# bluecube/minipath

Measured on AMD Instinct MI355X. Metric: Mrays/s, higher is better.
Workload: dtype f32

## Files before the change

minipath_amd/csrc/group_walk.h:

```cpp
#pragma once

#include "wave_common.h"

namespace mp {
namespace {

constexpr int kFcmpOGT = 2, kFcmpOGE = 3, kFcmpOLT = 4, kFcmpOLE = 5;
__device__ __forceinline__ uint64_t mask_gt(float a, float b) { return __builtin_amdgcn_fcmpf(a, b, kFcmpOGT); }
__device__ __forceinline__ uint64_t mask_lt(float a, float b) { return __builtin_amdgcn_fcmpf(a, b, kFcmpOLT); }
__device__ __forceinline__ uint64_t mask_le(float a, float b) { return __builtin_amdgcn_fcmpf(a, b, kFcmpOLE); }
__device__ __forceinline__ uint64_t mask_ge(float a, float b) { return __builtin_amdgcn_fcmpf(a, b, kFcmpOGE); }

enum { kClosest = 0, kBounded = 1, kAnyHit = 2 };
template <bool PATCH_NAN, bool BFE, int QS = 64, int MODE = kClosest>
__device__ __forceinline__ void trace_wave_impl(const DevScene& sc, float* __restrict__ q, uint2* __restrict__ stack_base,
                                                int nrays, float pb = FLT_MAX) {
    static_assert(MODE == kClosest || QS == 64, "ray queries run on the wave's LDS queue");
    constexpr int HB = QS == 64 ? 0 : 9;
    const int lane = static_cast<int>(threadIdx.x) & 63;
    const int g = lane >> 3, li = lane & 7;
    uint2* stack = stack_base + g * sc.stack_cap;
    const uint32_t lanes_below = (1u << li) - 1u;

    int slot = -1, sp = 0, head = 0;
    uint32_t pk = 0, pk_end = 0, seq = 0;
    float ox = 0, oy = 0, oz = 0, dx = 0, dy = 0, dz = 0, ix = 0, iy = 0, iz = 0;
    const float4* __restrict__ nodes4 = reinterpret_cast<const float4*>(PATCH_NAN ? sc.nodes_lit : sc.nodes_aos);
    const uint32_t root = PATCH_NAN ? sc.root_lit : sc.root;
    const float* __restrict__ tris = sc.tris_aos;
    float best_t = FLT_MAX;
    float tl = FLT_MAX, ul = 0, vl = 0;
    uint32_t pkl = kNoPrim, seql = 0;
    float pix = 0.0f, piy = 0.0f, piz = 0.0f;
    if (QS == 64) {
        const float qx = q[3 * 64 + lane], qy = q[4 * 64 + lane], qz = q[5 * 64 + lane];
        pix = (qx == 0.0f) ? INFINITY : 1.0f / qx; piy = (qy == 0.0f) ? INFINITY : 1.0f / qy; piz = (qz == 0.0f) ? INFINITY : 1.0f / qz;
    }

    for (;;) {
        if (MODE == kAnyHit && slot >= 0 && sp == 0 && pk == pk_end) {
            if (li == 0) q[1 * 64 + slot] = as_f(pkl);
            slot = -1;
        }
        if (MODE != kAnyHit && slot >= 0 && sp == 0 && pk == pk_end) {
            float tmin = group_min_t(tl);
            uint32_t key = (pkl != kNoPrim && tl == tmin) ? ((seql << 3) | static_cast<uint32_t>(li)) : 0xFFFFFFFFu;
            uint32_t kmin = group_min_u(key);
            const int wl4 = (((static_cast<int>(threadIdx.x) & 56) | static_cast<int>(kmin & 7u))) << 2;
            const float wu = __int_as_float(__builtin_amdgcn_ds_bpermute(wl4, __float_as_int(ul)));
            const float wv = __int_as_float(__builtin_amdgcn_ds_bpermute(wl4, __float_as_int(vl)));
            const uint32_t wp = static_cast<uint32_t>(__builtin_amdgcn_ds_bpermute(wl4, static_cast<int>(pkl)));
            if (li == 0) {
                bool hit = kmin != 0xFFFFFFFFu;
                q[(HB + 0) * QS + slot] = hit ? tmin : FLT_MAX;
                q[(HB + 1) * QS + slot] = as_f(hit ? (wp * 8u + (kmin & 7u)) : kNoPrim);
                q[(HB + 2) * QS + slot] = wu;
                q[(HB + 3) * QS + slot] = wv;
            }
            slot = -1;
        }
        uint64_t idle = __ballot(slot < 0);
        if (idle != 0) {
            int g_ = g;
            asm volatile("" : "+v"(g_));
            const uint64_t groups_below = (1ull << (g_ * 8)) - 1ull;
            uint64_t gm = idle & 0x0101010101010101ull;
            int mine = head + __popcll(gm & groups_below);
            head += __popcll(gm);
            float fix = 0.0f, fiy = 0.0f, fiz = 0.0f, fb = FLT_MAX;
            if (QS == 64) { fix = __shfl(pix, mine & 63); fiy = __shfl(piy, mine & 63); fiz = __shfl(piz, mine & 63); }
            if (MODE != kClosest) fb = __shfl(pb, mine & 63);
            if (slot < 0 && mine < nrays) {
                slot = mine;
                ox = q[0 * QS + mine]; oy = q[1 * QS + mine]; oz = q[2 * QS + mine];
                dx = q[3 * QS + mine]; dy = q[4 * QS + mine]; dz = q[5 * QS + mine];
                if (QS != 64) { fix = q[6 * QS + mine]; fiy = q[7 * QS + mine]; fiz = q[8 * QS + mine]; }
                ix = fix; iy = fiy; iz = fiz;
                best_t = fb; tl = fb; ul = 0; vl = 0; pkl = kNoPrim; seql = 0; seq = 0;
                pk = pk_end = 0;
                sp = 1;
                if (li == 0) stack[0] = make_uint2(root, as_u(-INFINITY));
            }
            if (__ballot(slot >= 0) == 0) break;
        }
        wave_lds_sync();
        if (slot >= 0 && pk == pk_end) {
            sp--;
            uint2 e = stack[sp];
            float node_t1 = as_f(e.y);
            if (!(node_t1 > best_t)) {
                uint32_t link = e.x;
                if ((link & 63u) == 0u) {
                    const float4* cp = reinterpret_cast<const float4*>(reinterpret_cast<const char*>(nodes4) + ((link << 2) | (static_cast<uint32_t>(li) << 5)));
                    const float4 c0 = cp[0], c1 = cp[1];
                    const uint32_t child = as_u(c1.z);
                    float ax = (c0.x - ox) * ix, ay = (c0.y - oy) * iy, az = (c0.z - oz) * iz;
                    float cx = (c0.w - ox) * ix, cy = (c1.x - oy) * iy, cz = (c1.y - oz) * iz;
                    if (PATCH_NAN) {
                        ax = fmaxf(ax, -INFINITY); ay = fmaxf(ay, -INFINITY); az = fmaxf(az, -INFINITY);
                        cx = fminf(cx, INFINITY); cy = fminf(cy, INFINITY); cz = fminf(cz, INFINITY);
                    }
                    const float t1 = fmaxf(fmaxf(fminf(ax, cx), 0.0f), fmaxf(fminf(ay, cy), fminf(az, cz)));
                    const float t2 = fminf(fminf(fmaxf(ax, cx), best_t), fminf(fmaxf(ay, cy), fmaxf(az, cz)));
                    const uint64_t okm = mask_le(t1, t2) & __builtin_amdgcn_uicmp(child, MP_LINK_NULL, 33);
                    const bool ok = __builtin_amdgcn_inverse_ballot_w64(okm);
                    uint32_t m = static_cast<uint32_t>(okm >> (g * 8)) & 0xFFu;
                    const uint32_t below = BFE ? __builtin_amdgcn_ubfe(m, 0u, static_cast<uint32_t>(li)) : (m & lanes_below);
                    if (ok) stack[sp + __popc(below)] = make_uint2(child, as_u(t1));
                    sp += __popc(m);
                } else {
                    pk = link >> 6;
                    pk_end = pk + (((link & 63u) + 7u) >> 3);
                }
            }
        }
        if (slot >= 0 && pk < pk_end) {
            const uint32_t toff = ((pk * 9u) << 5) + static_cast<uint32_t>(li) * 36u;
            const float* tp = reinterpret_cast<const float*>(reinterpret_cast<const char*>(tris) + toff);
            const float v0x = tp[0], v0y = tp[1], v0z = tp[2], e1x = tp[3], e1y = tp[4], e1z = tp[5], e2x = tp[6], e2y = tp[7], e2z = tp[8];
            float hx = fms(dy, e2z, dz * e2y), hy = fms(dz, e2x, dx * e2z), hz = fms(dx, e2y, dy * e2x);
            float det = fma_dot(e1x, e1y, e1z, hx, hy, hz);
            float inv_det = 1.0f / det;
            float sx = ox - v0x, sy = oy - v0y, sz = oz - v0z;
            float u = inv_det * fma_dot(sx, sy, sz, hx, hy, hz);
            float qx = fms(sy, e1z, sz * e1y), qy = fms(sz, e1x, sx * e1z), qz = fms(sx, e1y, sy * e1x);
            float v = inv_det * fma_dot(dx, dy, dz, qx, qy, qz);
            float t = inv_det * fma_dot(e2x, e2y, e2z, qx, qy, qz);
            bool valid = (u >= 0.0f) & (v >= 0.0f) & ((u + v) <= 1.0f) & (t >= 0.0f) & (t <= best_t);
            if (MODE == kAnyHit) {
                if ((__ballot(valid && t < tl) >> (g * 8)) & 0xFFull) { sp = 0; pk = pk_end; pkl = 0u; }
                else pk++;
                continue;
            }
            if (valid && t < tl) { tl = t; ul = u; vl = v; pkl = pk; seql = seq; }
            seq++;
            pk++;
            if (pk == pk_end) best_t = group_min_t(tl);
        }
    }
    wave_lds_sync();
}

template <bool BFE = false, int MODE = kClosest>
__device__ __forceinline__ void trace_wave(const DevScene& sc, float* __restrict__ q, uint2* __restrict__ stack_base, int nrays,
                                           float pb = FLT_MAX) {
    const int lane = static_cast<int>(threadIdx.x) & 63;
    const float qx = q[3 * 64 + lane], qy = q[4 * 64 + lane], qz = q[5 * 64 + lane];
    const float ix = (qx == 0.0f) ? INFINITY : 1.0f / qx, iy = (qy == 0.0f) ? INFINITY : 1.0f / qy, iz = (qz == 0.0f) ? INFINITY : 1.0f / qz;
    const bool inf = lane < nrays && (fabsf(ix) == INFINITY || fabsf(iy) == INFINITY || fabsf(iz) == INFINITY);
    if (__ballot(inf) != 0) trace_wave_impl<true, BFE, 64, MODE>(sc, q, stack_base, nrays, pb);
    else trace_wave_impl<false, BFE, 64, MODE>(sc, q, stack_base, nrays, pb);
}

template <int QS>
__device__ __forceinline__ void trace_wave_pool(const DevScene& sc, float* __restrict__ q, uint2* __restrict__ stack_base, int nrays) {
    int lane = static_cast<int>(threadIdx.x) & 63;
    asm volatile("" : "+v"(lane));
    bool inf = false;
#pragma unroll
    for (int k = 0; k < QS / 64; k++) {
        const int slot = lane + 64 * k;
        if (slot < nrays)
            inf = inf || fabsf(q[6 * QS + slot]) == INFINITY || fabsf(q[7 * QS + slot]) == INFINITY || fabsf(q[8 * QS + slot]) == INFINITY;
    }
    if (__ballot(inf) != 0) trace_wave_impl<true, true, QS>(sc, q, stack_base, nrays);
    else trace_wave_impl<false, true, QS>(sc, q, stack_base, nrays);
}

__device__ __forceinline__ bool may_hit_scene(const DevScene& sc, const Ray& r) {
    if (!sc.has_pre) return true;
    float ax = (sc.pre_min[0] - r.ox) * r.ix, ay = (sc.pre_min[1] - r.oy) * r.iy, az = (sc.pre_min[2] - r.oz) * r.iz;
    float cx = (sc.pre_max[0] - r.ox) * r.ix, cy = (sc.pre_max[1] - r.oy) * r.iy, cz = (sc.pre_max[2] - r.oz) * r.iz;
    ax = (ax != ax) ? -INFINITY : ax; ay = (ay != ay) ? -INFINITY : ay; az = (az != az) ? -INFINITY : az;
    cx = (cx != cx) ? INFINITY : cx; cy = (cy != cy) ? INFINITY : cy; cz = (cz != cz) ? INFINITY : cz;
    float lox = fminf(ax, cx), loy = fminf(ay, cy), loz = fminf(az, cz);
    float hix = fmaxf(ax, cx), hiy = fmaxf(ay, cy), hiz = fmaxf(az, cz);
    float t1 = fmaxf(fmaxf(lox, 0.0f), fmaxf(loy, loz));
    float t2 = fminf(fminf(hix, FLT_MAX), fminf(hiy, hiz));
    return t1 <= t2;
}

__device__ __forceinline__ uint32_t resolve_normal(const DevScene& sc, uint32_t prim, float u, float v, float n[3]) {
    const float4* sh = reinterpret_cast<const float4*>(sc.shade) + static_cast<size_t>(prim) * 3;
    float4 a = sh[0], b = sh[1], c = sh[2];
    float nx, ny, nz;
    if (as_u(c.y) != 0u) {
        const float* tp = sc.tris_aos + static_cast<size_t>(prim) * kTriDwords;
        float e1x = tp[3], e1y = tp[4], e1z = tp[5], e2x = tp[6], e2y = tp[7], e2z = tp[8];
        nx = e1y * e2z - e1z * e2y;
        ny = e1z * e2x - e1x * e2z;
        nz = e1x * e2y - e1y * e2x;
    } else {
        float w = 1.0f - u - v;
        nx = a.x * w + a.w * u + b.z * v;
        ny = a.y * w + b.x * u + b.w * v;
        nz = a.z * w + b.y * u + c.x * v;
    }
    float len = sqrtf(nx * nx + ny * ny + nz * nz);
    n[0] = nx / len; n[1] = ny / len; n[2] = nz / len;
    return as_u(c.z);
}

__device__ __forceinline__ bool sphere_intersect(const DevScene& sc, const Ray& r, float& t, float n[3]) {
    const float ocx = r.ox - sc.sphere_center[0], ocy = r.oy - sc.sphere_center[1], ocz = r.oz - sc.sphere_center[2];
    const float b = ocx * r.dx + ocy * r.dy + ocz * r.dz;
    const float c = (ocx * ocx + ocy * ocy + ocz * ocz) - sc.sphere_radius * sc.sphere_radius;
    const float disc = b * b - c;
    if (disc < 0.0f) return false;
    const float sq = sqrtf(disc);
    const float t1 = -b - sq, t2 = -b + sq;
    if (t1 > 0.0f) t = t1;
    else if (t2 > 0.0f) t = t2;
    else return false;
    const float px = r.ox + r.dx * t, py = r.oy + r.dy * t, pz = r.oz + r.dz * t;
    const float nx = px - sc.sphere_center[0], ny = py - sc.sphere_center[1], nz = pz - sc.sphere_center[2];
    const float len = sqrtf(nx * nx + ny * ny + nz * nz);
    n[0] = nx / len; n[1] = ny / len; n[2] = nz / len;
    return true;
}

__device__ __forceinline__ void object_scene(const DevScene& sc, uint32_t k, DevScene& sk) {
    sk = sc;
    const DevObject& o = sc.objects[k];
    sk.shade = o.shade; sk.nodes_aos = o.nodes_aos; sk.nodes_lit = o.nodes_lit; sk.tris_aos = o.tris_aos; sk.vidx = o.vidx; sk.vtex = o.vtex;
    sk.root = o.root; sk.root_lit = o.root_lit; sk.has_pre = o.has_pre;
    sk.kind = o.kind; sk.sphere_radius = o.sphere_radius;
    for (int i = 0; i < 3; i++) { sk.pre_min[i] = o.pre_min[i]; sk.pre_max[i] = o.pre_max[i]; sk.sphere_center[i] = o.sphere_center[i]; }
}
__device__ __forceinline__ void quat_rotate(float qi, float qj, float qk, float qw, float vx, float vy, float vz, float& ox,
                                            float& oy, float& oz) {
    const float tx = (qj * vz - qk * vy) * 2.0f, ty = (qk * vx - qi * vz) * 2.0f, tz = (qi * vy - qj * vx) * 2.0f;
    const float cx = qj * tz - qk * ty, cy = qk * tx - qi * tz, cz = qi * ty - qj * tx;
    ox = tx * qw + cx + vx; oy = ty * qw + cy + vy; oz = tz * qw + cz + vz;
}
__device__ __forceinline__ void object_ray(const DevScene& sc, uint32_t k, const Ray& r, Ray& rk) {
    const DevObject& o = sc.objects[k];
    rk = r;
    rk.ox = r.ox - o.t[0]; rk.oy = r.oy - o.t[1]; rk.oz = r.oz - o.t[2];
    if (o.rotated) {
        const float qi = -o.q[0], qj = -o.q[1], qk = -o.q[2], qw = o.q[3];
        const float vx = rk.ox, vy = rk.oy, vz = rk.oz;
        quat_rotate(qi, qj, qk, qw, vx, vy, vz, rk.ox, rk.oy, rk.oz);
        quat_rotate(qi, qj, qk, qw, r.dx, r.dy, r.dz, rk.dx, rk.dy, rk.dz);
        rk.ix = (rk.dx == 0.0f) ? INFINITY : 1.0f / rk.dx;
        rk.iy = (rk.dy == 0.0f) ? INFINITY : 1.0f / rk.dy;
        rk.iz = (rk.dz == 0.0f) ? INFINITY : 1.0f / rk.dz;
    }
}

struct GroupHit {
    float t, u, v;
    uint32_t prim, inst;
};

template <bool OBJ, bool BFE = false, int MODE = kClosest>
__device__ __forceinline__ void trace_objects(const DevScene& sc, const Ray& r, bool act, float* __restrict__ q,
                                              uint2* __restrict__ stack, GroupHit& h, float b = FLT_MAX) {
    h.t = MODE == kClosest ? FLT_MAX : b; h.u = h.v = 0.0f; h.prim = kNoPrim; h.inst = 0u;
    auto pass = [&](const DevScene& sk, const Ray& rk, uint32_t k) {
        const bool open = act && (MODE != kAnyHit || h.prim == kNoPrim);
        if (OBJ && sk.kind == 1u) {
            float ts, nn[3];
            if (open && sphere_intersect(sk, rk, ts, nn) && ts < h.t) { h.t = ts; h.prim = 0u; h.u = h.v = 0.0f; h.inst = k; }
            return;
        }
        const bool queued = open && may_hit_scene(sk, rk);
        const uint64_t am = __ballot(queued);
        const int n = __popcll(am), rank = rank_below(am);
        if (queued) {
            q[0 * 64 + rank] = rk.ox; q[1 * 64 + rank] = rk.oy; q[2 * 64 + rank] = rk.oz;
            q[3 * 64 + rank] = rk.dx; q[4 * 64 + rank] = rk.dy; q[5 * 64 + rank] = rk.dz;
        }
        float pb = FLT_MAX;
        if (MODE != kClosest) {
            const int dst = queued ? rank : n + (static_cast<int>(threadIdx.x & 63) - rank);
            pb = __int_as_float(__builtin_amdgcn_ds_permute(dst << 2, __float_as_int(b)));
        }
        wave_lds_sync();
        trace_wave<BFE, MODE>(sk, q, stack, n, pb);
        if (queued) {
            const uint32_t prim = as_u(q[1 * 64 + rank]);
            if (MODE == kAnyHit) {
                if (prim != kNoPrim) { h.prim = 0u; h.inst = k; }
            } else {
                const float t = q[0 * 64 + rank];
                if (prim != kNoPrim && t < h.t) { h.t = t; h.prim = prim; h.u = q[2 * 64 + rank]; h.v = q[3 * 64 + rank]; h.inst = k; }
            }
        }
        wave_lds_sync();
    };
    if (!OBJ) {
        pass(sc, r, 0u);
    } else {
        for (uint32_t k = 0; k < sc.inst_count; k++) {
            DevScene sk;
            Ray rk;
            object_scene(sc, k, sk);
            object_ray(sc, k, r, rk);
            pass(sk, rk, k);
        }
    }
    if (MODE != kClosest && h.prim == kNoPrim) h.t = FLT_MAX;
}

__device__ __forceinline__ uint32_t object_normal(const DevScene& sc, uint32_t inst, const Ray& r, uint32_t prim, float u, float v,
                                                  float n[3]) {
    DevScene so;
    object_scene(sc, inst, so);
    uint32_t mat = 0u;
    if (so.kind == 1u) {
        Ray rk;
        object_ray(sc, inst, r, rk);
        float t;
        sphere_intersect(so, rk, t, n);
    } else {
        mat = resolve_normal(so, prim, u, v, n);
    }
    const DevObject& o = sc.objects[inst];
    if (o.rotated) quat_rotate(o.q[0], o.q[1], o.q[2], o.q[3], n[0], n[1], n[2], n[0], n[1], n[2]);
    return mat;
}

}
}
```

minipath_amd/csrc/kernels.hip:

```cpp
#include <hip/hip_runtime.h>

#include <algorithm>
#include <cfloat>
#include <cmath>
#include <cstdlib>
#include <type_traits>

#include "launch_plan.h"
#include "mp_internal.h"
#include "family_launch.h"
#include "ray_math.h"

#ifdef MP_PROF_MISSES
namespace mp {
namespace {
__device__ unsigned long long g_prof[8];
}
}
#define MP_PROF_COUNT(i) do { if ((threadIdx.x & 63u) == 0u) atomicAdd(&g_prof[i], 1ull); } while (0)
#endif
#include "mask_cache.h"
#include "group_walk.h"

namespace mp {
namespace {

struct RenderParams {
    DevScene scene;
    RayGen gen;
    const mp_block* tiles;
    uint32_t n_tiles, tile_size;
    float* out;
    uint32_t* counter;
    float inv_spp;
    uint32_t s_begin, s_end;
    uint32_t carry_in;
    uint32_t finalize;
    uint32_t chunked;
    const uint32_t* tile_order;
    unsigned long long* tile_cost;
    uint32_t lds_per_wave;
    uint32_t max_depth;
    unsigned long long* segments;
    float* pool;
    uint32_t pool_stride;
};

constexpr uint32_t kSumChunk = 256;
__device__ __forceinline__ void pixel_state_load(const RenderParams& P, size_t off, bool inpix, bool writer, float& acc, float& cnt) {
    acc = 0.0f;
    cnt = 0.0f;
    if (P.carry_in && inpix) {
        const float4 prev = *reinterpret_cast<const float4*>(P.out + off);
        acc = prev.x;
        cnt = P.chunked ? prev.y : prev.w;
    } else if (P.chunked && inpix && writer) {
        *reinterpret_cast<double*>(P.out + off + 2) = 0.0;
    }
}
__device__ __forceinline__ void chunk_flush(const RenderParams& P, size_t off, bool writer, float& acc) {
    if (writer) {
        double* t = reinterpret_cast<double*>(P.out + off + 2);
        *t = *t + static_cast<double>(acc);
    }
    acc = 0.0f;
}
__device__ __forceinline__ void pixel_state_store(const RenderParams& P, size_t off, float acc, float cnt) {
    if (P.chunked) {
        if (!P.finalize) {
            *reinterpret_cast<float2*>(P.out + off) = make_float2(acc, cnt);
            return;
        }
        double t = *reinterpret_cast<const double*>(P.out + off + 2);
        if ((P.s_end & (kSumChunk - 1u)) != 0u) t = t + static_cast<double>(acc);
        const double inv = 1.0 / static_cast<double>(P.gen.spp);
        const float m = static_cast<float>(t * inv), a = static_cast<float>(static_cast<double>(cnt) * inv);
        *reinterpret_cast<float4*>(P.out + off) = make_float4(m, m, m, a);
        return;
    }
    const float m = P.finalize ? acc * P.inv_spp : acc;
    const float a = P.finalize ? cnt * P.inv_spp : cnt;
    *reinterpret_cast<float4*>(P.out + off) = make_float4(m, m, m, a);
}

typedef const __attribute__((address_space(4))) RenderParams* kparams_t;
__device__ __forceinline__ const RenderParams& params_view(kparams_t kp) { return kernarg_view<RenderParams>(kp); }
#define MP_KERNEL_PARAMS kparams_t KP = (kparams_t)__builtin_amdgcn_kernarg_segment_ptr()

#define MP_NEXT_UNIT(unit)                                                                              \
    uint32_t unit;                                                                                      \
    {                                                                                                   \
        const uint32_t q_ = qstate & 0xFFu;                                                             \
        uint32_t idx_ = 0;                                                                              \
        if (lane == 0) idx_ = atomicAdd(P.counter + q_ * kWorkQueueStride, 1u);                         \
        idx_ = __builtin_amdgcn_readfirstlane(idx_);                                                    \
        unit = idx_ * kWorkQueues + q_;                                                                 \
        if (unit >= total || idx_ >= 0x10000000u) {                                                     \
            if ((qstate >> 8) + 1u == kWorkQueues) break;                                               \
            qstate = ((q_ + 1u) % kWorkQueues) | (((qstate >> 8) + 1u) << 8);                           \
            continue;                                                                                   \
        }                                                                                               \
        qstate = q_;                                                                                    \
    }

template <int S, bool OBJ>
__global__ __launch_bounds__(256) void render_tiles_kernel(RenderParams) {
    extern __shared__ __align__(16) unsigned char smem[];
    MP_KERNEL_PARAMS;
    const RenderParams& P0 = params_view(KP);
    constexpr int BW = (S == 1) ? 8 : (S == 2) ? 8 : (S == 4) ? 4 : 4;
    constexpr int BH = 64 / S / BW;
    const int lane = static_cast<int>(threadIdx.x) & 63, wave = static_cast<int>(threadIdx.x) >> 6;
    float* q = reinterpret_cast<float*>(smem + static_cast<size_t>(wave) * P0.lds_per_wave);
    uint2* stack = reinterpret_cast<uint2*>(q + kQueueFloats);
    const uint32_t ts = P0.tile_size;
    const uint32_t bx = (ts + BW - 1) / BW, by = (ts + BH - 1) / BH, upt = bx * by;
    const uint32_t total = P0.n_tiles * upt;
    const int pix = lane / S, sub = lane % S;

    uint32_t qstate = blockIdx.x % kWorkQueues;
    for (;;) {
        const RenderParams& P = params_view(KP);
        MP_NEXT_UNIT(unit)
        const uint32_t b = unit % upt;
        const uint32_t tile_i = P.tile_order ? P.tile_order[unit / upt] : unit / upt;
        const uint64_t t_unit = P.tile_cost ? __builtin_readcyclecounter() : 0;
        const mp_block T = P.tiles[tile_i];
        const uint32_t px = T.min_x + (b % bx) * BW + static_cast<uint32_t>(pix % BW);
        const uint32_t py = T.min_y + (b / bx) * BH + static_cast<uint32_t>(pix / BW);
        const bool inpix = px < T.max_x && py < T.max_y;
        if (__ballot(inpix) == 0) continue;
        const size_t off = (static_cast<size_t>(tile_i) * ts * ts + static_cast<size_t>(py - T.min_y) * ts + (px - T.min_x)) * 4;
        float acc, cnt;
        pixel_state_load(P, off, inpix, sub == 0, acc, cnt);
        for (uint32_t s0 = P.s_begin & ~static_cast<uint32_t>(S - 1); s0 < P.s_end; s0 += S) {
            const uint32_t s = s0 + static_cast<uint32_t>(sub);
            const bool act = inpix && s >= P.s_begin && s < P.s_end;
            Ray r;
            r.dx = r.dy = r.dz = 0.0f;
            if (act) sample_ray(P.gen, px, py, s, r);
            if (P.scene.kind == 1u) {
                float c = 0.0f, h = 0.0f, ts_, nn[3];
                if (act && sphere_intersect(P.scene, r, ts_, nn)) { c = fabsf(r.dx * nn[0] + r.dy * nn[1] + r.dz * nn[2]); h = 1.0f; }
#pragma unroll
                for (int j = 0; j < S; j++) {
                    acc += __shfl(c, (lane & ~(S - 1)) + j);
                    cnt += __shfl(h, (lane & ~(S - 1)) + j);
                }
                if (P.chunked && ((s0 + S) & (kSumChunk - 1u)) == 0u && s0 + S <= P.s_end) chunk_flush(P, off, inpix && sub == 0, acc);
                continue;
            }
            GroupHit gh;
            trace_objects<OBJ>(P.scene, r, act, q, stack, gh);
            float c = 0.0f, h = 0.0f;
            if (gh.prim != kNoPrim) {
                float nn[3];
                if (OBJ) object_normal(P.scene, gh.inst, r, gh.prim, gh.u, gh.v, nn);
                else resolve_normal(P.scene, gh.prim, gh.u, gh.v, nn);
                c = fabsf(r.dx * nn[0] + r.dy * nn[1] + r.dz * nn[2]);
                h = 1.0f;
            }
#pragma unroll
            for (int j = 0; j < S; j++) {
                acc += __shfl(c, (lane & ~(S - 1)) + j);
                cnt += __shfl(h, (lane & ~(S - 1)) + j);
            }
            if (P.chunked && ((s0 + S) & (kSumChunk - 1u)) == 0u && s0 + S <= P.s_end) chunk_flush(P, off, inpix && sub == 0, acc);
        }
        if (inpix && sub == 0) pixel_state_store(P, off, acc, cnt);
// ... 222 lines not shown
struct RegStack3 {
    int ent, mlo, mhi;
    __device__ __forceinline__ RegStack3() : ent(0), mlo(0), mhi(0) {}
    __device__ __forceinline__ void push(int sp, uint32_t e, uint64_t m) {
        asm volatile("s_mov_b32 m0, %3\n\ts_nop 0\n\t"
                     "v_writelane_b32 %0, %4, m0\n\tv_writelane_b32 %1, %5, m0\n\tv_writelane_b32 %2, %6, m0"
                     : "+v"(ent), "+v"(mlo), "+v"(mhi)
                     : "s"(sp), "s"(e), "s"(static_cast<uint32_t>(m)), "s"(static_cast<uint32_t>(m >> 32))
                     : "m0");
    }
    __device__ __forceinline__ void pop(int sp, uint32_t& e, uint64_t& m) const {
        e = static_cast<uint32_t>(__builtin_amdgcn_readlane(ent, sp));
        m = static_cast<uint32_t>(__builtin_amdgcn_readlane(mlo, sp)) |
            (static_cast<uint64_t>(static_cast<uint32_t>(__builtin_amdgcn_readlane(mhi, sp))) << 32);
    }
};

template <int OCT>
__device__ __noinline__ uint32_t unit_list_slow(const float* __restrict__ nodes_pk, uint32_t* mcache, uint32_t node, uint32_t slots) {
    return unit_list_build(reinterpret_cast<const float4*>(nodes_pk), mcache, node, slots,
                           [](const float* b, const float bmn[3], const float bmx[3]) { return bounds_may_hit<OCT>(b, bmn, bmx); });
}
template <int OCT>
__device__ __forceinline__ bool trace_packet_cached(const DevScene& sc, const Ray& r, bool active, PacketHit& hit, uint32_t* mcache) {
    static_assert(kNullLink == MP_LINK_NULL, "mask_cache.h's copy of the null link");
    kfp nodes = (kfp)(uintptr_t)sc.nodes_pk;
    kfp tris = (kfp)(uintptr_t)sc.tris_aos;
    float best_t = FLT_MAX, bu = 0.0f, bv = 0.0f;
    uint32_t bprim = kNoPrim;
    RegStack3 st;
    int sp = 0;
    mcache[kRootListSlot] = sc.pk_count * sc.pk_mask_bits;
    wave_lds_sync();
    uint32_t cur = (static_cast<uint32_t>(kRootListSlot) << 16) | 1u;
    uint64_t pm = __ballot(active);
    for (;;) {
        if ((cur & 0xFFFFu) == 0u) {
            if (sp == 0) break;
            sp--;
            st.pop(sp, cur, pm);
        }
        cur -= 1u;
        const uint32_t src = __builtin_amdgcn_readfirstlane(mcache[(cur >> 16) + (cur & 0xFFFFu)]);
#ifndef MP_NO_EMPTY_SKIP
        if (static_cast<int32_t>(src) < 0) {
            MP_PROF_COUNT(7);
            continue;
        }
#endif
        const bool pon = __builtin_amdgcn_inverse_ballot_w64(pm);
        const krec8 rec = *reinterpret_cast<const __attribute__((address_space(4))) krec8*>(reinterpret_cast<const __attribute__((address_space(4))) char*>(nodes) + scalar_u(src * 32u));
        float t1, t2;
        slab<false, OCT>(rec[0], rec[1], rec[2], rec[3], rec[4], rec[5], r, pon ? best_t : -1.0f, t1, t2);
        const bool ok = t1 <= t2;
        if (__ballot(ok) == 0) continue;
        const uint32_t link = uniform_u(rec[6]);
        float lim = ok ? best_t : -1.0f;
        if ((link & 63u) == 0u) {
            MP_PROF_COUNT(2);
            const uint32_t node = link >> 6;
            const uint32_t slot = node_slot(node);
            const uint32_t tag = __builtin_amdgcn_readfirstlane(mcache[static_cast<uint32_t>(kMaskCacheHeader) + slot]);
            uint32_t list = __builtin_amdgcn_readfirstlane(mcache[static_cast<uint32_t>(kNodeListBase) + slot]);
            if (__builtin_expect(tag != node, 0)) {
                MP_PROF_COUNT(0);
                if (tag != 0xFFFFFFFFu) MP_PROF_COUNT(4);
                list = __builtin_amdgcn_readfirstlane(unit_list_slow<OCT>(sc.nodes_pk, mcache, node, sc.pk_mask_bits));
                if (list == kListOverflow) {
                    if (sp != 0 || (cur & 0xFFFFu) != 0u) {
                        MP_PROF_COUNT(6);
                        return false;
                    }
                    list = __builtin_amdgcn_readfirstlane(unit_list_slow<OCT>(sc.nodes_pk, mcache, node, sc.pk_mask_bits));
                }
            }
            if ((list & 0xFFFFu) != 0u) {
                if ((cur & 0xFFFFu) != 0u) {
                    st.push(sp, cur, pm);
                    sp++;
                }
                cur = list;
                pm = __ballot(lim >= 0.0f);
            }
        } else {
            const uint32_t first = link >> 6, n_real = link & 63u;
            kfp tp = tris + static_cast<size_t>(first) * (8 * kTriDwords);
            static_assert(kExitTiny == kTiny && kExitHuge == kHuge, "mask_cache.h's copies of the early-out constants");
            const float thr = lim >= 0.0f ? -kTiny : INFINITY;
            auto test = [&](const float v0x, const float v0y, const float v0z, const float e1x, const float e1y, const float e1z,
                            const float e2x, const float e2y, const float e2z, const uint32_t tri) {
                const float hx = fms(r.dy, e2z, r.dz * e2y), hy = fms(r.dz, e2x, r.dx * e2z), hz = fms(r.dx, e2y, r.dy * e2x);
                const float det = fma_dot(e1x, e1y, e1z, hx, hy, hz);
                const float sx = r.ox - v0x, sy = r.oy - v0y, sz = r.oz - v0z;
                const float un = fma_dot(sx, sy, sz, hx, hy, hz);
                const float xu = tri_flipped(det, un);
                if (__ballot(!(tri_exit1_key(det, xu) <= thr)) == 0) return;
                const float qx = fms(sy, e1z, sz * e1y), qy = fms(sz, e1x, sx * e1z), qz = fms(sx, e1y, sy * e1x);
                const float vn = fma_dot(r.dx, r.dy, r.dz, qx, qy, qz);
                const float tn = fma_dot(e2x, e2y, e2z, qx, qy, qz);
                const float xv = tri_flipped(det, vn), xt = tri_flipped(det, tn);
                if (__ballot(!(tri_exit2_key(det, xu, xv, xt) <= thr)) == 0) return;
                constexpr uint32_t kRcpLo = 0x10800000u , kRcpHi = 0x7E000000u ;
                const uint32_t wkey = (as_u(det) << 1) - (kRcpLo << 1);
                const float inv_det = __ballot(wkey > ((kRcpHi - kRcpLo) << 1)) == 0 ? rm::rcp_short(det) : 1.0f / det;
                const float u = inv_det * un, v = inv_det * vn, t = inv_det * tn;
                const bool acc = !(fminf(fminf(u, v), t) < 0.0f) & ((u + v) <= 1.0f) & (t < lim);
                best_t = acc ? t : best_t;
                lim = acc ? t : lim;
                bu = acc ? u : bu;
                bv = acc ? v : bv;
                bprim = acc ? tri : bprim;
            };
            const uint32_t ls = first & static_cast<uint32_t>(kLeafCacheEntries - 1);
            const uint32_t tag = mcache[kLeafTagBase + ls];
            const uint2 tm = reinterpret_cast<const uint2*>(mcache + kLeafMaskBase)[ls];
            uint64_t todo;
            if (__builtin_expect(__builtin_amdgcn_readfirstlane(tag) == first, 1)) {
                todo = __builtin_amdgcn_readfirstlane(tm.x) | (static_cast<uint64_t>(__builtin_amdgcn_readfirstlane(tm.y)) << 32);
            } else {
                MP_PROF_COUNT(1);
                const uint64_t m = leaf_mask_slow(sc.tris_aos, mcache, first, n_real);
                todo = __builtin_amdgcn_readfirstlane(static_cast<uint32_t>(m)) | (static_cast<uint64_t>(__builtin_amdgcn_readfirstlane(static_cast<uint32_t>(m >> 32))) << 32);
            }
#ifndef MP_NO_EMPTY_SKIP
            if (todo == 0 && (cur >> 16) != static_cast<uint32_t>(kRootListSlot)) {
                if ((threadIdx.x & 63u) == 0u) mcache[(cur >> 16) + (cur & 0xFFFFu)] = src | kEmptyLeafBit;
                wave_lds_sync();
            }
#endif
            if (todo != 0) {
                uint32_t c = static_cast<uint32_t>(__builtin_ctzll(todo));
                todo &= ~(1ull << c);
                kfp ta = tri_record(tp, c);
                krec8 ra = *reinterpret_cast<const __attribute__((address_space(4))) krec8*>(ta);
                float a8 = ta[8];
                while (todo != 0) {
                    const uint32_t cn = static_cast<uint32_t>(__builtin_ctzll(todo));
                    todo &= ~(1ull << cn);
                    kfp tb = tri_record(tp, cn);
                    const krec8 rb = *reinterpret_cast<const __attribute__((address_space(4))) krec8*>(tb);
                    const float b8 = tb[8];
                    test(ra[0], ra[1], ra[2], ra[3], ra[4], ra[5], ra[6], ra[7], a8, first * 8u + c);
                    ra = rb; a8 = b8;
                    c = cn;
                }
                test(ra[0], ra[1], ra[2], ra[3], ra[4], ra[5], ra[6], ra[7], a8, first * 8u + c);
            }
        }
    }
    hit.t = best_t; hit.u = bu; hit.v = bv; hit.prim = bprim;
    return true;
}

template <bool OCTANTS, class Stack, bool MC = false>
__device__ __forceinline__ void trace_packet(const DevScene& sc, const Ray& r, bool active, Stack& st, PacketHit& hit,
                                             const MaskCache& mc = MaskCache{nullptr}) {
    if (OCTANTS && MC) {
        if (__ballot(active & !mask_cache_ray_ok(r)) != 0) {
            const bool slow = active && (fabsf(r.ix) == INFINITY || fabsf(r.iy) == INFINITY || fabsf(r.iz) == INFINITY);
            if (__ballot(slow) != 0) trace_packet_impl<2, -1>(sc, r, active, st, hit);
            else trace_packet_impl<1, -1>(sc, r, active, st, hit);
            return;
        }
    } else {
        const bool slow = active && (fabsf(r.ix) == INFINITY || fabsf(r.iy) == INFINITY || fabsf(r.iz) == INFINITY);
        if (__ballot(slow) != 0) {
            trace_packet_impl<2, -1>(sc, r, active, st, hit);
            return;
        }
    }
    if (OCTANTS && sc.boxes_ordered) {
        const uint64_t am = __ballot(active);
        const uint64_t nx = __ballot(active && r.ix < 0.0f), ny = __ballot(active && r.iy < 0.0f), nz = __ballot(active && r.iz < 0.0f);
        if ((nx == 0 || nx == am) && (ny == 0 || ny == am) && (nz == 0 || nz == am)) {
            const uint32_t oct = (nx ? 1u : 0u) | (ny ? 2u : 0u) | (nz ? 4u : 0u);
            if (MC) {
                mask_cache_begin_pass(mc, r, active, oct);
                bool done;
                switch (oct) {
                    case 0: done = trace_packet_cached<0>(sc, r, active, hit, mc.lds); break;
                    case 1: done = trace_packet_cached<1>(sc, r, active, hit, mc.lds); break;
                    case 2: done = trace_packet_cached<2>(sc, r, active, hit, mc.lds); break;
                    case 3: done = trace_packet_cached<3>(sc, r, active, hit, mc.lds); break;
                    case 4: done = trace_packet_cached<4>(sc, r, active, hit, mc.lds); break;
                    case 5: done = trace_packet_cached<5>(sc, r, active, hit, mc.lds); break;
                    case 6: done = trace_packet_cached<6>(sc, r, active, hit, mc.lds); break;
                    default: done = trace_packet_cached<7>(sc, r, active, hit, mc.lds); break;
                }
                if (done) return;
            } else {
                switch (oct) {
                    case 0: trace_packet_impl<1, 0>(sc, r, active, st, hit); return;
                    case 1: trace_packet_impl<1, 1>(sc, r, active, st, hit); return;
                    case 2: trace_packet_impl<1, 2>(sc, r, active, st, hit); return;
                    case 3: trace_packet_impl<1, 3>(sc, r, active, st, hit); return;
                    case 4: trace_packet_impl<1, 4>(sc, r, active, st, hit); return;
                    case 5: trace_packet_impl<1, 5>(sc, r, active, st, hit); return;
                    case 6: trace_packet_impl<1, 6>(sc, r, active, st, hit); return;
                    default: trace_packet_impl<1, 7>(sc, r, active, st, hit); return;
                }
            }
        }
    }
    trace_packet_impl<1, -1>(sc, r, active, st, hit);
}

template <class T>
__device__ __forceinline__ const T* uniform_ptr(const T* p) {
    const uint64_t v = reinterpret_cast<uint64_t>(p);
    const uint32_t lo = __builtin_amdgcn_readfirstlane(static_cast<uint32_t>(v)), hi = __builtin_amdgcn_readfirstlane(static_cast<uint32_t>(v >> 32));
    return reinterpret_cast<const T*>((static_cast<uint64_t>(hi) << 32) | lo);
}

template <bool OCTANTS, class Stack>
__device__ __forceinline__ void trace_packet_objects(const DevScene& sc, const Ray& r, bool act, Stack& st, PacketHit& h, uint32_t& inst) {
    h.t = FLT_MAX; h.u = h.v = 0.0f; h.prim = kNoPrim;
    inst = 0u;
    for (uint32_t k = 0; k < sc.inst_count; k++) {
        DevScene sk;
        Ray rk;
        object_scene(sc, k, sk);
        object_ray(sc, k, r, rk);
        sk.kind = __builtin_amdgcn_readfirstlane(sk.kind);
        sk.root = __builtin_amdgcn_readfirstlane(sk.root);
        sk.root_lit = __builtin_amdgcn_readfirstlane(sk.root_lit);
        sk.nodes_aos = uniform_ptr(sk.nodes_aos);
        sk.nodes_lit = uniform_ptr(sk.nodes_lit);
        sk.tris_aos = uniform_ptr(sk.tris_aos);
        if (sk.kind == 1u) {
            float ts, nn[3];
            if (act && sphere_intersect(sk, rk, ts, nn) && ts < h.t) { h.t = ts; h.prim = 0u; h.u = h.v = 0.0f; inst = k; }
            continue;
        }
        const bool go = act && may_hit_scene(sk, rk);
        if (__ballot(go) == 0) continue;
        PacketHit hk;
        trace_packet<OCTANTS>(sk, rk, go, st, hk);
        if (hk.prim != kNoPrim && hk.t < h.t) { h = hk; inst = k; }
    }
}

struct RegStack2 {
    int link, src, alo, ahi, blo, bhi;
    __device__ __forceinline__ RegStack2() : link(0), src(0), alo(0), ahi(0), blo(0), bhi(0) {}
    __device__ __forceinline__ void push(int sp, uint32_t l, uint32_t s, uint64_t ma, uint64_t mb) {
        asm volatile(
            "s_mov_b32 m0, %6\n\ts_nop 0\n\t"
            "v_writelane_b32 %0, %7, m0\n\tv_writelane_b32 %1, %8, m0\n\tv_writelane_b32 %2, %9, m0\n\tv_writelane_b32 %3, %10, m0\n\t"
            "v_writelane_b32 %4, %11, m0\n\tv_writelane_b32 %5, %12, m0"
            : "+v"(link), "+v"(src), "+v"(alo), "+v"(ahi), "+v"(blo), "+v"(bhi)
            : "s"(sp), "s"(l), "s"(s), "s"(static_cast<uint32_t>(ma)), "s"(static_cast<uint32_t>(ma >> 32)),
              "s"(static_cast<uint32_t>(mb)), "s"(static_cast<uint32_t>(mb >> 32))
            : "m0");
    }
    __device__ __forceinline__ void pop(int sp, uint32_t& l, uint32_t& s, uint64_t& ma, uint64_t& mb) const {
        l = static_cast<uint32_t>(__builtin_amdgcn_readlane(link, sp));
        s = static_cast<uint32_t>(__builtin_amdgcn_readlane(src, sp));
        ma = static_cast<uint32_t>(__builtin_amdgcn_readlane(alo, sp)) |
             (static_cast<uint64_t>(static_cast<uint32_t>(__builtin_amdgcn_readlane(ahi, sp))) << 32);
        mb = static_cast<uint32_t>(__builtin_amdgcn_readlane(blo, sp)) |
             (static_cast<uint64_t>(static_cast<uint32_t>(__builtin_amdgcn_readlane(bhi, sp))) << 32);
    }
};

template <int MODE, int OCT>
__device__ __forceinline__ void trace_packet2_impl(const DevScene& sc, const Ray& ra, const Ray& rb, bool active_a, bool active_b,
                                                   PacketHit& hit_a, PacketHit& hit_b) {
    constexpr bool PATCH_NAN = MODE == 2;
    kfp nodes = (kfp)(uintptr_t)(PATCH_NAN ? sc.nodes_lit : sc.nodes_aos);
    kfp tris = (kfp)(uintptr_t)sc.tris_aos;
    RegStack2 st;
    float best_a = FLT_MAX, ua = 0.0f, va = 0.0f, best_b = FLT_MAX, ub = 0.0f, vb = 0.0f;
    uint32_t prim_a = kNoPrim, prim_b = kNoPrim;
    st.push(0, PATCH_NAN ? sc.root_lit : sc.root, kSrcRoot, __ballot(active_a), __ballot(active_b));
    int sp = 1;
    int stale_top = 0;
    while (sp > 0) {
        sp--;
        uint32_t link, src;
        uint64_t onm_a, onm_b;
        st.pop(sp, link, src, onm_a, onm_b);
        if (sp < stale_top) {
            stale_top = sp;
            kfp bx = nodes + static_cast<size_t>(src) * 8;
            const float b0 = bx[0], b1 = bx[1], b2 = bx[2], b3 = bx[3], b4 = bx[4], b5 = bx[5];
            onm_a &= ~mask_gt(slab_entry<PATCH_NAN, OCT>(b0, b1, b2, b3, b4, b5, ra), best_a);
            onm_b &= ~mask_gt(slab_entry<PATCH_NAN, OCT>(b0, b1, b2, b3, b4, b5, rb), best_b);
        }
        if ((onm_a | onm_b) == 0) continue;
        const bool on_a = __builtin_amdgcn_inverse_ballot_w64(onm_a), on_b = __builtin_amdgcn_inverse_ballot_w64(onm_b);
        float lim_a = on_a ? best_a : -1.0f, lim_b = on_b ? best_b : -1.0f;
        if ((link & 63u) == 0u) {
            const uint32_t node = link >> 6;
            kfp nd = nodes + static_cast<size_t>(node) * 64;
            float a0 = nd[0], a1 = nd[1], a2 = nd[2], a3 = nd[3], a4 = nd[4], a5 = nd[5], a6 = nd[6];
            const uint32_t nchild = uniform_u(nd[7]);
            uint32_t slot = node * 8u;
            auto child = [&](const float b0, const float b1, const float b2, const float b3, const float b4, const float b5,
                             const float blink, const uint32_t cslot) {
                const uint32_t cl = uniform_u(blink);
                if (cl == MP_LINK_NULL) return;
                float t1a, t2a, t1b, t2b;
                slab<PATCH_NAN, OCT>(b0, b1, b2, b3, b4, b5, ra, lim_a, t1a, t2a);
                slab<PATCH_NAN, OCT>(b0, b1, b2, b3, b4, b5, rb, lim_b, t1b, t2b);
                const uint64_t ok_a = __ballot(t1a <= t2a), ok_b = __ballot(t1b <= t2b);
                if ((ok_a | ok_b) != 0) {
                    st.push(sp, cl, cslot, ok_a, ok_b);
                    sp++;
                }
            };
            for (uint32_t p = nchild >> 1; p > 0; p--) {
                const float b0 = nd[8], b1 = nd[9], b2 = nd[10], b3 = nd[11], b4 = nd[12], b5 = nd[13], b6 = nd[14];
                child(a0, a1, a2, a3, a4, a5, a6, slot);
                a0 = nd[16]; a1 = nd[17]; a2 = nd[18]; a3 = nd[19]; a4 = nd[20]; a5 = nd[21]; a6 = nd[22];
                child(b0, b1, b2, b3, b4, b5, b6, slot + 1u);
                slot += 2u;
                nd += 16;
            }
            if (nchild & 1u) child(a0, a1, a2, a3, a4, a5, a6, slot);
        } else {
            const uint32_t first = link >> 6, n_real = link & 63u;
            kfp tp = tris + static_cast<size_t>(first) * (8 * kTriDwords);
            const float thr_a = on_a ? -kTiny : INFINITY, thr_b = on_b ? -kTiny : INFINITY;
            uint64_t changed = 0;
            auto test = [&](const float v0x, const float v0y, const float v0z, const float e1x, const float e1y, const float e1z,
                            const float e2x, const float e2y, const float e2z, const uint32_t tri) {
                const float hxa = fms(ra.dy, e2z, ra.dz * e2y), hya = fms(ra.dz, e2x, ra.dx * e2z), hza = fms(ra.dx, e2y, ra.dy * e2x);
                const float hxb = fms(rb.dy, e2z, rb.dz * e2y), hyb = fms(rb.dz, e2x, rb.dx * e2z), hzb = fms(rb.dx, e2y, rb.dy * e2x);
                const float det_a = fma_dot(e1x, e1y, e1z, hxa, hya, hza), det_b = fma_dot(e1x, e1y, e1z, hxb, hyb, hzb);
                const float sxa = ra.ox - v0x, sya = ra.oy - v0y, sza = ra.oz - v0z;
                const float sxb = rb.ox - v0x, syb = rb.oy - v0y, szb = rb.oz - v0z;
                const float un_a = fma_dot(sxa, sya, sza, hxa, hya, hza), un_b = fma_dot(sxb, syb, szb, hxb, hyb, hzb);
                const uint32_t sg_a = as_u(det_a) & 0x80000000u, sg_b = as_u(det_b) & 0x80000000u;
                const bool ok_a = fabsf(det_a) <= kHuge, ok_b = fabsf(det_b) <= kHuge;
                const float xua = ok_a ? as_f(as_u(un_a) ^ sg_a) : 1.0f, xub = ok_b ? as_f(as_u(un_b) ^ sg_b) : 1.0f;
                if ((__ballot(!(xua <= thr_a)) | __ballot(!(xub <= thr_b))) == 0) return;
                const float qxa = fms(sya, e1z, sza * e1y), qya = fms(sza, e1x, sxa * e1z), qza = fms(sxa, e1y, sya * e1x);
                const float qxb = fms(syb, e1z, szb * e1y), qyb = fms(szb, e1x, sxb * e1z), qzb = fms(sxb, e1y, syb * e1x);
                const float vn_a = fma_dot(ra.dx, ra.dy, ra.dz, qxa, qya, qza), vn_b = fma_dot(rb.dx, rb.dy, rb.dz, qxb, qyb, qzb);
                const float tn_a = fma_dot(e2x, e2y, e2z, qxa, qya, qza), tn_b = fma_dot(e2x, e2y, e2z, qxb, qyb, qzb);
                const float xva = ok_a ? as_f(as_u(vn_a) ^ sg_a) : 1.0f, xta = ok_a ? as_f(as_u(tn_a) ^ sg_a) : 1.0f;
                const float xvb = ok_b ? as_f(as_u(vn_b) ^ sg_b) : 1.0f, xtb = ok_b ? as_f(as_u(tn_b) ^ sg_b) : 1.0f;
                if ((__ballot(!(fminf(fminf(xua, xva), xta) <= thr_a)) | __ballot(!(fminf(fminf(xub, xvb), xtb) <= thr_b))) == 0) return;
                const float inv_a = 1.0f / det_a, inv_b = 1.0f / det_b;
                const float u_a = inv_a * un_a, v_a = inv_a * vn_a, t_a = inv_a * tn_a;
                const float u_b = inv_b * un_b, v_b = inv_b * vn_b, t_b = inv_b * tn_b;
                const bool acc_a = (u_a >= 0.0f) & (v_a >= 0.0f) & ((u_a + v_a) <= 1.0f) & (t_a >= 0.0f) & (t_a < lim_a);
                const bool acc_b = (u_b >= 0.0f) & (v_b >= 0.0f) & ((u_b + v_b) <= 1.0f) & (t_b >= 0.0f) & (t_b < lim_b);
                best_a = acc_a ? t_a : best_a; lim_a = acc_a ? t_a : lim_a; ua = acc_a ? u_a : ua; va = acc_a ? v_a : va; prim_a = acc_a ? tri : prim_a;
                best_b = acc_b ? t_b : best_b; lim_b = acc_b ? t_b : lim_b; ub = acc_b ? u_b : ub; vb = acc_b ? v_b : vb; prim_b = acc_b ? tri : prim_b;
                changed |= __ballot(acc_a) | __ballot(acc_b);
            };
            float a0 = tp[0], a1 = tp[1], a2 = tp[2], a3 = tp[3], a4 = tp[4], a5 = tp[5], a6 = tp[6], a7 = tp[7], a8 = tp[8];
            uint32_t tri = first * 8u;
            for (uint32_t p = n_real >> 1; p > 0; p--) {
                const float b0 = tp[9], b1 = tp[10], b2 = tp[11], b3 = tp[12], b4 = tp[13], b5 = tp[14], b6 = tp[15], b7 = tp[16], b8 = tp[17];
                test(a0, a1, a2, a3, a4, a5, a6, a7, a8, tri);
                a0 = tp[18]; a1 = tp[19]; a2 = tp[20]; a3 = tp[21]; a4 = tp[22]; a5 = tp[23]; a6 = tp[24]; a7 = tp[25]; a8 = tp[26];
                test(b0, b1, b2, b3, b4, b5, b6, b7, b8, tri + 1u);
                tri += 2u;
                tp += 2 * kTriDwords;
            }
            if (n_real & 1u) test(a0, a1, a2, a3, a4, a5, a6, a7, a8, tri);
            if (changed != 0) stale_top = sp;
        }
    }
    hit_a.t = best_a; hit_a.u = ua; hit_a.v = va; hit_a.prim = prim_a;
    hit_b.t = best_b; hit_b.u = ub; hit_b.v = vb; hit_b.prim = prim_b;
}

__device__ __forceinline__ void trace_packet2(const DevScene& sc, const Ray& ra, const Ray& rb, bool act_a, bool act_b, PacketHit& ha,
                                              PacketHit& hb) {
    const bool slow = (act_a && (fabsf(ra.ix) == INFINITY || fabsf(ra.iy) == INFINITY || fabsf(ra.iz) == INFINITY)) ||
                      (act_b && (fabsf(rb.ix) == INFINITY || fabsf(rb.iy) == INFINITY || fabsf(rb.iz) == INFINITY));
    if (__ballot(slow) != 0) {
        trace_packet2_impl<2, -1>(sc, ra, rb, act_a, act_b, ha, hb);
        return;
    }
    if (sc.boxes_ordered) {
        const uint64_t am = __ballot(act_a), bm = __ballot(act_b);
        const uint64_t nxa = __ballot(act_a && ra.ix < 0.0f), nya = __ballot(act_a && ra.iy < 0.0f), nza = __ballot(act_a && ra.iz < 0.0f);
        const uint64_t nxb = __ballot(act_b && rb.ix < 0.0f), nyb = __ballot(act_b && rb.iy < 0.0f), nzb = __ballot(act_b && rb.iz < 0.0f);
        const bool xn = (nxa | nxb) != 0, yn = (nya | nyb) != 0, zn = (nza | nzb) != 0;
        const bool xu = !xn || (nxa == am && nxb == bm), yu = !yn || (nya == am && nyb == bm), zu = !zn || (nza == am && nzb == bm);
        if (xu && yu && zu) {
            switch ((xn ? 1 : 0) | (yn ? 2 : 0) | (zn ? 4 : 0)) {
                case 0: trace_packet2_impl<1, 0>(sc, ra, rb, act_a, act_b, ha, hb); return;
                case 1: trace_packet2_impl<1, 1>(sc, ra, rb, act_a, act_b, ha, hb); return;
                case 2: trace_packet2_impl<1, 2>(sc, ra, rb, act_a, act_b, ha, hb); return;
                case 3: trace_packet2_impl<1, 3>(sc, ra, rb, act_a, act_b, ha, hb); return;
                case 4: trace_packet2_impl<1, 4>(sc, ra, rb, act_a, act_b, ha, hb); return;
                case 5: trace_packet2_impl<1, 5>(sc, ra, rb, act_a, act_b, ha, hb); return;
                case 6: trace_packet2_impl<1, 6>(sc, ra, rb, act_a, act_b, ha, hb); return;
                default: trace_packet2_impl<1, 7>(sc, ra, rb, act_a, act_b, ha, hb); return;
            }
        }
    }
    trace_packet2_impl<1, -1>(sc, ra, rb, act_a, act_b, ha, hb);
}

template <int J, int N>
struct RowSum {
    static __device__ __forceinline__ void run(float& acc, float c) {
        acc += __int_as_float(__builtin_amdgcn_update_dpp(0, __float_as_int(c), 0x150 + J, 0xF, 0xF, false));
        RowSum<J + 1, N>::run(acc, c);
    }
};
template <int N>
struct RowSum<N, N> {
    static __device__ __forceinline__ void run(float&, float) {}
};
template <int S>
__device__ __forceinline__ void add_samples_in_order(float& acc, float c, int lane) {
    if (S == 1) {
        acc += c;
    } else if (S == 16) {
        RowSum<0, 16>::run(acc, c);
    } else if (S == 32) {
        RowSum<0, 16>::run(acc, c);
        acc = __int_as_float(__builtin_amdgcn_update_dpp(__float_as_int(acc), __float_as_int(acc), 0x142, 0xA, 0xF, false));
        RowSum<0, 16>::run(acc, c);
        const float lo = __int_as_float(__builtin_amdgcn_readlane(__float_as_int(acc), 31));
        const float hi = __int_as_float(__builtin_amdgcn_readlane(__float_as_int(acc), 63));
        acc = lane < 32 ? lo : hi;
    } else {
#pragma unroll
        for (int j = 0; j < S; j++) acc += __shfl(c, (lane & ~(S - 1)) + j);
    }
}

template <int S, bool LDS_STACK, int WPE, bool OBJ = false, bool MCACHE = false>
__global__ __launch_bounds__(256) __attribute__((amdgpu_waves_per_eu(WPE, 8))) void render_tiles_packet_kernel(RenderParams) {
    extern __shared__ __align__(16) unsigned char smem[];
    MP_KERNEL_PARAMS;
    constexpr int BW = (S <= 2) ? 8 : (S <= 8) ? 4 : (S <= 32) ? 2 : 1;
    constexpr int BH = 64 / S / BW;
    const int lane = static_cast<int>(threadIdx.x) & 63;
    const int pix = lane / S, sub = lane % S;
    uint32_t qstate = blockIdx.x % kWorkQueues;
    MaskCache mc{nullptr};
    if (MCACHE) mc.lds = reinterpret_cast<uint32_t*>(smem) + static_cast<size_t>(__builtin_amdgcn_readfirstlane(static_cast<int>(threadIdx.x) >> 6)) * kMaskCacheDwords;
    for (;;) {
        const RenderParams& P = params_view(KP);
        const uint32_t ts = P.tile_size;
        const uint32_t bx = (ts + BW - 1) / BW, by = (ts + BH - 1) / BH, upt = bx * by, total = P.n_tiles * upt;
        MP_NEXT_UNIT(unit)
        const uint32_t b = unit % upt;
        const uint32_t tile_i = P.tile_order ? P.tile_order[unit / upt] : unit / upt;
        const uint64_t t_unit = P.tile_cost ? __builtin_readcyclecounter() : 0;
        const mp_block T = P.tiles[tile_i];
        const uint32_t px = T.min_x + (b % bx) * BW + static_cast<uint32_t>(pix % BW);
        const uint32_t py = T.min_y + (b / bx) * BH + static_cast<uint32_t>(pix / BW);
        const bool inpix = px < T.max_x && py < T.max_y;
        if (__ballot(inpix) == 0) continue;
        const size_t off = (static_cast<size_t>(tile_i) * ts * ts + static_cast<size_t>(py - T.min_y) * ts + (px - T.min_x)) * 4;
        float acc, cnt;
        pixel_state_load(P, off, inpix, sub == 0, acc, cnt);
        if (MCACHE) {
            const RenderParams& C = params_view(KP);
            const uint32_t ux = T.min_x + (b % bx) * BW, uy = T.min_y + (b / bx) * BH;
            mask_cache_begin_unit(mc, C.gen.s, C.gen.jitter_scale, ux, min(ux + BW, T.max_x) - 1u, uy, min(uy + BH, T.max_y) - 1u);
        }
        const uint32_t s_begin = P.s_begin, s_end = P.s_end;
        for (uint32_t s0 = s_begin & ~static_cast<uint32_t>(S - 1); s0 < s_end; s0 += S) {
            const uint32_t s = s0 + static_cast<uint32_t>(sub);
            const bool act = inpix && s >= s_begin && s < s_end;
            Ray r;
            r.ox = r.oy = r.oz = r.dx = r.dy = r.dz = r.ix = r.iy = r.iz = 0.0f;
            {
                const RenderParams& G = params_view(KP);
                if (act) sample_ray(G.gen, px, py, s, r);
            }
            PacketHit h;
            h.t = FLT_MAX; h.u = h.v = 0.0f; h.prim = kNoPrim;
            uint32_t hinst = 0u;
            {
                const RenderParams& W = params_view(KP);
                float* lds = reinterpret_cast<float*>(smem + static_cast<size_t>(static_cast<int>(threadIdx.x) >> 6) * W.lds_per_wave);
                if (OBJ) {
                    if (LDS_STACK) {
                        HybridStack st(lds, lane, W.scene.stack_cap, W.scene.packet_stack_regs);
                        trace_packet_objects<false>(W.scene, r, act, st, h, hinst);
                    } else {
                        RegStack st(lds, lane);
                        trace_packet_objects<(S >= 8 && S <= 32)>(W.scene, r, act, st, h, hinst);
                    }
                } else {
#ifdef MP_PROF_NOWALK
                    const bool go = false;
#else
                    const bool go = act && W.scene.kind == 0u && may_hit_scene(W.scene, r);
#endif
                    if (__ballot(go) != 0) {
                        if (LDS_STACK) {
                            HybridStack st(lds, lane, W.scene.stack_cap, W.scene.packet_stack_regs);
                            trace_packet<false>(W.scene, r, go, st, h);
                        } else {
                            RegStack st(lds, lane);
                            trace_packet<((S >= 8 && S <= 32) || MCACHE), RegStack, MCACHE>(W.scene, r, go, st, h, mc);
                        }
                    }
                }
            }
            float c = 0.0f;
            bool hit = h.prim != kNoPrim;
            const RenderParams& H = params_view(KP);
            if (hit) {
#ifdef MP_PROF_NOSHADE
                c = h.u;
#else
                float nn[3];
                if (OBJ) object_normal(H.scene, hinst, r, h.prim, h.u, h.v, nn);
                else resolve_normal(H.scene, h.prim, h.u, h.v, nn);
                c = fabsf(r.dx * nn[0] + r.dy * nn[1] + r.dz * nn[2]);
#endif
            } else if (H.scene.kind == 1u) {
                float ts_, nn[3];
                hit = act && sphere_intersect(H.scene, r, ts_, nn);
                if (hit) c = fabsf(r.dx * nn[0] + r.dy * nn[1] + r.dz * nn[2]);
            }
            {
                int l_ = lane;
                asm volatile("" : "+v"(l_));
                const uint64_t pixel_lanes = (S == 64 ? ~0ull : ((1ull << (S & 63)) - 1ull)) << (l_ & ~(S - 1));
                cnt += static_cast<float>(__popcll(__ballot(hit) & pixel_lanes));
            }
            add_samples_in_order<S>(acc, c, lane);
            if (H.chunked && ((s0 + S) & (kSumChunk - 1u)) == 0u && s0 + S <= s_end) chunk_flush(H, off, inpix && sub == 0, acc);
        }
        const RenderParams& E = params_view(KP);
        if (inpix && sub == 0) pixel_state_store(E, off, acc, cnt);
        if (E.tile_cost && lane == 0) atomicAdd(E.tile_cost + tile_i, static_cast<unsigned long long>(__builtin_readcyclecounter() - t_unit));
    }
}

template <int WPE>
__global__ __launch_bounds__(256) __attribute__((amdgpu_waves_per_eu(WPE, 8))) void render_tiles_packet2_kernel(RenderParams P) {
    constexpr int S = 16;
    const int lane = static_cast<int>(threadIdx.x) & 63;
    const int pix = lane / S, sub = lane % S;
    const uint64_t pixel_lanes = ((1ull << S) - 1ull) << (lane & ~(S - 1));
    const uint32_t ts = P.tile_size;
    const uint32_t bx = (ts + 3) / 4, by = (ts + 1) / 2, upt = bx * by, total = P.n_tiles * upt;
    uint32_t qstate = blockIdx.x % kWorkQueues;
    for (;;) {
        MP_NEXT_UNIT(unit)
        const uint32_t b = unit % upt;
        const uint32_t tile_i = P.tile_order ? P.tile_order[unit / upt] : unit / upt;
        const uint64_t t_unit = P.tile_cost ? __builtin_readcyclecounter() : 0;
        const mp_block T = P.tiles[tile_i];
        const uint32_t px_a = T.min_x + (b % bx) * 4 + static_cast<uint32_t>(pix % 2), px_b = px_a + 2u;
        const uint32_t py = T.min_y + (b / bx) * 2 + static_cast<uint32_t>(pix / 2);
        const bool in_a = px_a < T.max_x && py < T.max_y, in_b = px_b < T.max_x && py < T.max_y;
        if (__ballot(in_a) == 0) continue;
        const size_t off_a = (static_cast<size_t>(tile_i) * ts * ts + static_cast<size_t>(py - T.min_y) * ts + (px_a - T.min_x)) * 4;
        const size_t off_b = off_a + 8;
        float acc_a, cnt_a, acc_b, cnt_b;
        pixel_state_load(P, off_a, in_a, sub == 0, acc_a, cnt_a);
        pixel_state_load(P, off_b, in_b, sub == 0, acc_b, cnt_b);
        for (uint32_t s0 = P.s_begin & ~static_cast<uint32_t>(S - 1); s0 < P.s_end; s0 += S) {
            const uint32_t s = s0 + static_cast<uint32_t>(sub);
            const bool in_pass = s >= P.s_begin && s < P.s_end;
            const bool act_a = in_a && in_pass, act_b = in_b && in_pass;
            Ray ra, rb;
            ra.ox = ra.oy = ra.oz = ra.dx = ra.dy = ra.dz = ra.ix = ra.iy = ra.iz = 0.0f;
            rb = ra;
            if (act_a) sample_ray(P.gen, px_a, py, s, ra);
            if (act_b) sample_ray(P.gen, px_b, py, s, rb);
            const bool go_a = act_a && may_hit_scene(P.scene, ra), go_b = act_b && may_hit_scene(P.scene, rb);
            PacketHit ha, hb;
            ha.t = FLT_MAX; ha.u = ha.v = 0.0f; ha.prim = kNoPrim;
            hb = ha;
            if ((__ballot(go_a) | __ballot(go_b)) != 0) trace_packet2(P.scene, ra, rb, go_a, go_b, ha, hb);
            float c_a = 0.0f, c_b = 0.0f;
            const bool hit_a = ha.prim != kNoPrim, hit_b = hb.prim != kNoPrim;
            if (hit_a) {
                float nn[3];
                resolve_normal(P.scene, ha.prim, ha.u, ha.v, nn);
                c_a = fabsf(ra.dx * nn[0] + ra.dy * nn[1] + ra.dz * nn[2]);
            }
            if (hit_b) {
                float nn[3];
                resolve_normal(P.scene, hb.prim, hb.u, hb.v, nn);
                c_b = fabsf(rb.dx * nn[0] + rb.dy * nn[1] + rb.dz * nn[2]);
            }
            cnt_a += static_cast<float>(__popcll(__ballot(hit_a) & pixel_lanes));
            cnt_b += static_cast<float>(__popcll(__ballot(hit_b) & pixel_lanes));
            add_samples_in_order<S>(acc_a, c_a, lane);
            add_samples_in_order<S>(acc_b, c_b, lane);
            if (P.chunked && ((s0 + S) & (kSumChunk - 1u)) == 0u && s0 + S <= P.s_end) {
                chunk_flush(P, off_a, in_a && sub == 0, acc_a);
                chunk_flush(P, off_b, in_b && sub == 0, acc_b);
            }
        }
        if (sub == 0) {
            if (in_a) pixel_state_store(P, off_a, acc_a, cnt_a);
            if (in_b) pixel_state_store(P, off_b, acc_b, cnt_b);
        }
        if (P.tile_cost && lane == 0) atomicAdd(P.tile_cost + tile_i, static_cast<unsigned long long>(__builtin_readcyclecounter() - t_unit));
    }
}

constexpr float kPathEps = 1e-4f;

__device__ __forceinline__ void hit_tex(const DevScene& so, uint32_t prim, float u, float v, float& tx, float& ty) {
    const uint32_t* vi = so.vidx + static_cast<size_t>(prim) * 3;
    const float *t0 = so.vtex + 3 * static_cast<size_t>(vi[0]), *t1 = so.vtex + 3 * static_cast<size_t>(vi[1]),
                *t2 = so.vtex + 3 * static_cast<size_t>(vi[2]);
    const float w = 1.0f - u - v;
    tx = t0[0] * w + t1[0] * u + t2[0] * v;
    ty = t0[1] * w + t1[1] * u + t2[1] * v;
}

template <bool OBJ, int N>
__device__ __forceinline__ bool path_vertex(const DevScene& sc, const PacketHit& h, uint32_t depth, uint32_t max_depth, Rng& rng,
                                            Ray& r, float (&L)[N], float (&thr)[N], bool& primary_hit, uint32_t inst = 0u) {
    if (h.prim == kNoPrim) {
#pragma unroll
        for (int c = 0; c < N; c++) L[c] = L[c] + thr[c] * sc.sky;
        return false;
    }
    if (depth == 1) primary_hit = true;
    float n[3];
    const uint32_t mat = OBJ ? object_normal(sc, inst, r, h.prim, h.u, h.v, n) : resolve_normal(sc, h.prim, h.u, h.v, n);
    const float* m = sc.materials + static_cast<size_t>(mat) * 12;
#pragma unroll
    for (int c = 0; c < N; c++) L[c] = L[c] + thr[c] * m[3 + c];
    const float dn = r.dx * n[0] + r.dy * n[1] + r.dz * n[2];
    if (dn > 0.0f) { n[0] = -n[0]; n[1] = -n[1]; n[2] = -n[2]; }
    const float* alb = m;
    if (N == 3 && as_u(m[9]) == MP_TEXTURE_CHECKER) {
        float tx = 0.0f, ty = 0.0f;
        if (OBJ) {
            DevScene so;
            object_scene(sc, inst, so);
            if (so.kind == 0u) hit_tex(so, h.prim, h.u, h.v, tx, ty);
        } else {
            hit_tex(sc, h.prim, h.u, h.v, tx, ty);
        }
        const float cell = floorf(tx * m[10]) + floorf(ty * m[10]);
        const float half = cell * 0.5f;
        if (half - floorf(half) != 0.0f) alb = m + 6;
    }
#pragma unroll
    for (int c = 0; c < N; c++) thr[c] = thr[c] * alb[c];
    if (depth == max_depth) return false;
    const float hx = r.ox + r.dx * h.t, hy = r.oy + r.dy * h.t, hz = r.oz + r.dz * h.t;
    float x1, x2;
    unit_disc(rng, x1, x2);
    const float z = sqrtf(1.0f - (x1 * x1 + x2 * x2));
    const float sign = copysignf(1.0f, n[2]);
    const float a = -1.0f / (sign + n[2]);
    const float bb = n[0] * n[1] * a;
    const float t0 = 1.0f + sign * n[0] * n[0] * a, t1 = sign * bb, t2 = -sign * n[0];
    const float b0 = bb, b1 = sign + n[1] * n[1] * a, b2 = -n[1];
    ray_new(hx + n[0] * kPathEps, hy + n[1] * kPathEps, hz + n[2] * kPathEps, t0 * x1 + b0 * x2 + n[0] * z,
            t1 * x1 + b1 * x2 + n[1] * z, t2 * x1 + b2 * x2 + n[2] * z, r);
    return true;
}

__device__ __forceinline__ void pixel_state_load3(const RenderParams& P, size_t off, bool inpix, float (&acc)[3], float& cnt) {
    acc[0] = acc[1] = acc[2] = 0.0f;
    cnt = 0.0f;
    if (P.carry_in && inpix) {
        const float4 prev = *reinterpret_cast<const float4*>(P.out + off);
        acc[0] = prev.x; acc[1] = prev.y; acc[2] = prev.z;
        cnt = prev.w;
    }
}
__device__ __forceinline__ void pixel_state_store3(const RenderParams& P, size_t off, const float (&acc)[3], float cnt) {
    const float s = P.finalize ? P.inv_spp : 1.0f;
    *reinterpret_cast<float4*>(P.out + off) = make_float4(acc[0] * s, acc[1] * s, acc[2] * s, cnt * s);
}

struct AovParams {
    RenderParams r;
    float* shade;
    float* normal;
    float* albedo;
    uint32_t* ids;
    float* position;
    float* shade_sq;
    uint32_t park_pixel;
};

template <bool OBJ>
__device__ __forceinline__ void hit_albedo(const DevScene& sc, uint32_t inst, uint32_t mat, uint32_t prim, float u, float v, float (&a)[3]) {
    if (sc.materials == nullptr) { a[0] = a[1] = a[2] = 0.75f; return; }
    const float* m = sc.materials + static_cast<size_t>(mat) * 12;
    const float* alb = m;
    if (as_u(m[9]) == MP_TEXTURE_CHECKER) {
        float tx = 0.0f, ty = 0.0f;
        if (OBJ) {
            DevScene so;
            object_scene(sc, inst, so);
            if (so.kind == 0u) hit_tex(so, prim, u, v, tx, ty);
        } else {
            hit_tex(sc, prim, u, v, tx, ty);
        }
        const float cell = floorf(tx * m[10]) + floorf(ty * m[10]);
        const float half = cell * 0.5f;
        if (half - floorf(half) != 0.0f) alb = m + 6;
    }
    a[0] = alb[0]; a[1] = alb[1]; a[2] = alb[2];
}

template <int S, bool LDS_STACK, int WPE, bool OBJ = false, bool MCACHE = false>
__global__ __launch_bounds__(256) __attribute__((amdgpu_waves_per_eu(WPE, 8))) void render_aov_packet_kernel(AovParams) {
    extern __shared__ __align__(16) unsigned char smem[];
    typedef const __attribute__((address_space(4))) AovParams* kaov_t;
    kaov_t KP = (kaov_t)__builtin_amdgcn_kernarg_segment_ptr();
    constexpr int BW = (S <= 2) ? 8 : (S <= 8) ? 4 : (S <= 32) ? 2 : 1;
    constexpr int BH = 64 / S / BW;
    constexpr uint32_t kParkPixels = 64 / S;
    const int lane = static_cast<int>(threadIdx.x) & 63;
    const int pix = lane / S, sub = lane % S;
    uint32_t qstate = blockIdx.x % kWorkQueues;
    MaskCache mc{nullptr};
    if (MCACHE) mc.lds = reinterpret_cast<uint32_t*>(smem + 4 * kParkPixels * kernarg_view<AovParams>(KP).park_pixel) + static_cast<size_t>(__builtin_amdgcn_readfirstlane(static_cast<int>(threadIdx.x) >> 6)) * kMaskCacheDwords;
    for (;;) {
        const RenderParams& P = kernarg_view<AovParams>(KP).r;
        const uint32_t ts = P.tile_size;
        const uint32_t bx = (ts + BW - 1) / BW, by = (ts + BH - 1) / BH, upt = bx * by, total = P.n_tiles * upt;
        MP_NEXT_UNIT(unit)
        const uint32_t b = unit % upt;
        const uint32_t tile_i = P.tile_order ? P.tile_order[unit / upt] : unit / upt;
        const uint64_t t_unit = P.tile_cost ? __builtin_readcyclecounter() : 0;
        const mp_block T = P.tiles[tile_i];
        const uint32_t px = T.min_x + (b % bx) * BW + static_cast<uint32_t>(pix % BW);
        const uint32_t py = T.min_y + (b / bx) * BH + static_cast<uint32_t>(pix / BW);
        const bool inpix = px < T.max_x && py < T.max_y;
        if (__ballot(inpix) == 0) continue;
        const size_t off = (static_cast<size_t>(tile_i) * ts * ts + static_cast<size_t>(py - T.min_y) * ts + (px - T.min_x)) * 4;
        float cnt = 0.0f;
        {
            const AovParams& U = kernarg_view<AovParams>(KP);
            float4* park = reinterpret_cast<float4*>(smem + (static_cast<size_t>(static_cast<int>(threadIdx.x) >> 6) * kParkPixels + pix) * U.park_pixel);
            if (sub == 0) {
                float4 a0 = make_float4(0.0f, 0.0f, 0.0f, 0.0f), a1 = a0, a2 = a0;
                if (U.r.carry_in && inpix) {
                    if (U.shade_sq) { const float4 v = *reinterpret_cast<const float4*>(U.shade_sq + off); a2.w = v.x; cnt = v.w; }
                    if (U.position) { const float4 v = *reinterpret_cast<const float4*>(U.position + off); a2.x = v.x; a2.y = v.y; a2.z = v.z; cnt = v.w; }
                    if (U.albedo) { const float4 v = *reinterpret_cast<const float4*>(U.albedo + off); a1.y = v.x; a1.z = v.y; a1.w = v.z; cnt = v.w; }
                    if (U.normal) { const float4 v = *reinterpret_cast<const float4*>(U.normal + off); a0.y = v.x; a0.z = v.y; a0.w = v.z; a1.x = v.w; }
                    if (U.shade) { const float4 v = *reinterpret_cast<const float4*>(U.shade + off); a0.x = v.x; cnt = v.w; }
                }
                park[0] = a0; park[1] = a1;
                if (U.park_pixel > 32u) park[2] = a2;
            }
            if (MCACHE && lane == 0) mc.lds[kHdrState] = 0xFFFFFFFFu;
            wave_lds_sync();
        }
        const uint32_t s_end = P.s_end;
        for (uint32_t s0 = P.s_begin & ~static_cast<uint32_t>(S - 1); s0 < s_end; s0 += S) {
            const uint32_t s = s0 + static_cast<uint32_t>(sub);
            bool act;
            Ray r;
            r.ox = r.oy = r.oz = r.dx = r.dy = r.dz = r.ix = r.iy = r.iz = 0.0f;
            {
                const RenderParams& G = kernarg_view<AovParams>(KP).r;
                act = inpix && s >= G.s_begin && s < s_end;
                if (act) sample_ray(G.gen, px, py, s, r);
            }
            PacketHit h;
            h.t = FLT_MAX; h.u = h.v = 0.0f; h.prim = kNoPrim;
            uint32_t hinst = 0u;
            {
                const AovParams& WA = kernarg_view<AovParams>(KP);
                const RenderParams& W = WA.r;
                float* lds = reinterpret_cast<float*>(smem + 4 * kParkPixels * WA.park_pixel + static_cast<size_t>(static_cast<int>(threadIdx.x) >> 6) * W.lds_per_wave);
                if (OBJ) {
                    if (LDS_STACK) {
                        HybridStack st(lds, lane, W.scene.stack_cap, W.scene.packet_stack_regs);
                        trace_packet_objects<false>(W.scene, r, act, st, h, hinst);
                    } else {
                        RegStack st(lds, lane);
                        trace_packet_objects<(S == 16)>(W.scene, r, act, st, h, hinst);
                    }
                } else {
                    const bool go = act && W.scene.kind == 0u && may_hit_scene(W.scene, r);
                    if (__ballot(go) != 0) {
                        if (LDS_STACK) {
                            HybridStack st(lds, lane, W.scene.stack_cap, W.scene.packet_stack_regs);
                            trace_packet<false>(W.scene, r, go, st, h);
                        } else {
                            RegStack st(lds, lane);
                            trace_packet<(S == 16 || MCACHE), RegStack, MCACHE>(W.scene, r, go, st, h, mc);
                        }
                    }
                }
            }
            const AovParams& H = kernarg_view<AovParams>(KP);
            bool hit = h.prim != kNoPrim;
            float nn[3] = {0.0f, 0.0f, 0.0f};
            uint32_t mat = 0u;
            if (hit) {
                mat = OBJ ? object_normal(H.r.scene, hinst, r, h.prim, h.u, h.v, nn) : resolve_normal(H.r.scene, h.prim, h.u, h.v, nn);
            } else if (H.r.scene.kind == 1u) {
                hit = act && sphere_intersect(H.r.scene, r, h.t, nn);
                if (hit) h.prim = 0u;
            }
            if (H.ids && act && s == 0u)
                *reinterpret_cast<uint4*>(H.ids + off) = hit ? make_uint4(h.prim, hinst, mat, 1u) : make_uint4(kNoPrim, 0u, 0u, 0u);
            int l_ = lane;
            asm volatile("" : "+v"(l_));
            const uint64_t pixel_lanes = (S == 64 ? ~0ull : ((1ull << (S & 63)) - 1ull)) << (l_ & ~(S - 1));
            cnt += static_cast<float>(__popcll(__ballot(hit) & pixel_lanes));
            float4* park = reinterpret_cast<float4*>(smem + (static_cast<size_t>(static_cast<int>(threadIdx.x) >> 6) * kParkPixels + (l_ / S)) * H.park_pixel);
            float4 a0 = park[0], a1 = park[1];
            float c = 0.0f;
            if (H.shade || H.shade_sq) c = hit ? fabsf(r.dx * nn[0] + r.dy * nn[1] + r.dz * nn[2]) : 0.0f;
            if (H.shade) add_samples_in_order<S>(a0.x, c, lane);
            if (H.normal) {
                add_samples_in_order<S>(a0.y, hit ? nn[0] : 0.0f, lane);
                add_samples_in_order<S>(a0.z, hit ? nn[1] : 0.0f, lane);
                add_samples_in_order<S>(a0.w, hit ? nn[2] : 0.0f, lane);
                add_samples_in_order<S>(a1.x, hit ? h.t : 0.0f, lane);
            }
            if (H.albedo) {
                float al[3] = {0.0f, 0.0f, 0.0f};
                if (hit) hit_albedo<OBJ>(H.r.scene, hinst, mat, h.prim, h.u, h.v, al);
                add_samples_in_order<S>(a1.y, al[0], lane);
                add_samples_in_order<S>(a1.z, al[1], lane);
                add_samples_in_order<S>(a1.w, al[2], lane);
            }
            float4 a2 = make_float4(0.0f, 0.0f, 0.0f, 0.0f);
            if (H.park_pixel > 32u) {
                a2 = park[2];
                if (H.position) {
                    add_samples_in_order<S>(a2.x, hit ? r.ox + r.dx * h.t : 0.0f, lane);
                    add_samples_in_order<S>(a2.y, hit ? r.oy + r.dy * h.t : 0.0f, lane);
                    add_samples_in_order<S>(a2.z, hit ? r.oz + r.dz * h.t : 0.0f, lane);
                }
                if (H.shade_sq) add_samples_in_order<S>(a2.w, c * c, lane);
            }
            wave_lds_sync();
            if ((l_ & (S - 1)) == 0) {
                park[0] = a0; park[1] = a1;
                if (H.park_pixel > 32u) park[2] = a2;
            }
            wave_lds_sync();
        }
        const AovParams& E = kernarg_view<AovParams>(KP);
        if (inpix && sub == 0) {
            const float4* park = reinterpret_cast<const float4*>(smem + (static_cast<size_t>(static_cast<int>(threadIdx.x) >> 6) * kParkPixels + pix) * E.park_pixel);
            const float4 a0 = park[0], a1 = park[1];
            const float inv = E.r.finalize ? E.r.inv_spp : 1.0f, a = cnt * inv;
            if (E.shade) { const float m = a0.x * inv; *reinterpret_cast<float4*>(E.shade + off) = make_float4(m, m, m, a); }
            if (E.normal) *reinterpret_cast<float4*>(E.normal + off) = make_float4(a0.y * inv, a0.z * inv, a0.w * inv, a1.x * inv);
            if (E.albedo) *reinterpret_cast<float4*>(E.albedo + off) = make_float4(a1.y * inv, a1.z * inv, a1.w * inv, a);
            if (E.park_pixel > 32u) {
                const float4 a2 = park[2];
                if (E.position) *reinterpret_cast<float4*>(E.position + off) = make_float4(a2.x * inv, a2.y * inv, a2.z * inv, a);
                if (E.shade_sq) { const float m = a2.w * inv; *reinterpret_cast<float4*>(E.shade_sq + off) = make_float4(m, m, m, a); }
            }
        }
        if (E.r.tile_cost && lane == 0) atomicAdd(E.r.tile_cost + tile_i, static_cast<unsigned long long>(__builtin_readcyclecounter() - t_unit));
    }
}

#ifndef MP_PATHS_WPE
#define MP_PATHS_WPE 6
#endif
template <int S, bool OBJ, bool RGB, bool MCACHE = false>
__global__ __launch_bounds__(256) __attribute__((amdgpu_waves_per_eu(MP_PATHS_WPE, 8))) void render_paths_kernel(RenderParams) {
    constexpr int N = RGB ? 3 : 1;
    extern __shared__ __align__(16) unsigned char smem[];
    MP_KERNEL_PARAMS;
    MaskCache mc{nullptr};
    if (MCACHE) {
        const RenderParams& P0 = params_view(KP);
        mc.lds = reinterpret_cast<uint32_t*>(smem + static_cast<size_t>(__builtin_amdgcn_readfirstlane(static_cast<int>(threadIdx.x) >> 6) + 1) * P0.lds_per_wave) - kMaskCacheDwords;
    }
    constexpr int BW = (S <= 2) ? 8 : (S <= 8) ? 4 : 2;
    constexpr int BH = 64 / S / BW;
    const int lane = static_cast<int>(threadIdx.x) & 63, wave = static_cast<int>(threadIdx.x) >> 6;
    const int pix = lane / S, sub = lane % S;
    unsigned long long segs = 0;
    uint32_t qstate = blockIdx.x % kWorkQueues;
    for (;;) {
        const RenderParams& P = params_view(KP);
        const uint32_t ts = P.tile_size;
        const uint32_t bx = (ts + BW - 1) / BW, by = (ts + BH - 1) / BH, upt = bx * by, total = P.n_tiles * upt;
        MP_NEXT_UNIT(unit)
        const uint32_t b = unit % upt;
        const uint32_t tile_i = P.tile_order ? P.tile_order[unit / upt] : unit / upt;
        const uint64_t t_unit = P.tile_cost ? __builtin_readcyclecounter() : 0;
        const mp_block T = P.tiles[tile_i];
        const uint32_t px = T.min_x + (b % bx) * BW + static_cast<uint32_t>(pix % BW);
        const uint32_t py = T.min_y + (b / bx) * BH + static_cast<uint32_t>(pix / BW);
        const bool inpix = px < T.max_x && py < T.max_y;
        if (__ballot(inpix) == 0) continue;
        const size_t off = (static_cast<size_t>(tile_i) * ts * ts + static_cast<size_t>(py - T.min_y) * ts + (px - T.min_x)) * 4;
        float acc[N], cnt;
        if (RGB) pixel_state_load3(P, off, inpix, reinterpret_cast<float (&)[3]>(acc[0]), cnt);
        else pixel_state_load(P, off, inpix, sub == 0, acc[0], cnt);
        if (MCACHE) {
            if (lane == 0) mc.lds[kHdrState] = 0xFFFFFFFFu;
            wave_lds_sync();
        }
        const uint32_t s_begin = P.s_begin, s_end = P.s_end, max_depth = P.max_depth;
        for (uint32_t s0 = s_begin & ~static_cast<uint32_t>(S - 1); s0 < s_end; s0 += S) {
            const uint32_t s = s0 + static_cast<uint32_t>(sub);
            const bool act = inpix && s >= s_begin && s < s_end;
            Rng rng;
            rng_zero(rng);
            Ray r;
            r.ox = r.oy = r.oz = r.dx = r.dy = r.dz = r.ix = r.iy = r.iz = 0.0f;
            {
                const RenderParams& G = params_view(KP);
                if (act) {
                    rng_seed(rng, sample_key(G.gen, px, py, s));
                    sample_ray_rng(G.gen, px, py, rng, r);
                }
            }
            float L[N], thr[N];
#pragma unroll
            for (int c = 0; c < N; c++) { L[c] = 0.0f; thr[c] = 1.0f; }
            bool alive = act, primary_hit = false;
            PacketHit h;
            for (uint32_t depth = 1; depth <= max_depth; depth++) {
                const uint64_t alive_m = __ballot(alive);
                if (alive_m == 0) break;
                segs += static_cast<unsigned long long>(__popcll(alive_m));
                h.t = FLT_MAX; h.u = h.v = 0.0f; h.prim = kNoPrim;
                uint32_t hinst = 0u;
                {
                    const RenderParams& W = params_view(KP);
                    float* q = reinterpret_cast<float*>(smem + static_cast<size_t>(wave) * W.lds_per_wave);
                    uint2* stack = reinterpret_cast<uint2*>(q + kQueueFloats);
                    if (depth == 1 && OBJ) {
                        RegStack rst(nullptr, lane);
                        HybridStack hst(reinterpret_cast<float*>(stack), lane, W.scene.stack_cap, W.scene.packet_stack_regs);
                        if (W.scene.stack_cap > W.scene.packet_stack_regs) trace_packet_objects<false>(W.scene, r, alive, hst, h, hinst);
                        else trace_packet_objects<(S >= 8)>(W.scene, r, alive, rst, h, hinst);
                    } else if (depth == 1) {
                        const bool go = alive && may_hit_scene(W.scene, r);
                        if (__ballot(go) != 0) {
                            RegStack rst(nullptr, lane);
                            HybridStack hst(reinterpret_cast<float*>(stack), lane, W.scene.stack_cap, W.scene.packet_stack_regs);
                            if (W.scene.stack_cap > W.scene.packet_stack_regs) trace_packet<false>(W.scene, r, go, hst, h);
                            else trace_packet<(S >= 8), RegStack, MCACHE>(W.scene, r, go, rst, h, mc);
                        }
                    } else {
                        GroupHit gh;
                        trace_objects<OBJ>(W.scene, r, alive, q, stack, gh);
                        h.t = gh.t; h.u = gh.u; h.v = gh.v; h.prim = gh.prim;
                        hinst = gh.inst;
                    }
                }
                const RenderParams& V = params_view(KP);
                if (alive) alive = path_vertex<OBJ, N>(V.scene, h, depth, max_depth, rng, r, L, thr, primary_hit, hinst);
            }
            {
                int l_ = lane;
                asm volatile("" : "+v"(l_));
                const uint64_t pixel_lanes = (S == 64 ? ~0ull : ((1ull << (S & 63)) - 1ull)) << (l_ & ~(S - 1));
                cnt += static_cast<float>(__popcll(__ballot(primary_hit) & pixel_lanes));
            }
#pragma unroll
            for (int c = 0; c < N; c++) add_samples_in_order<S>(acc[c], L[c], lane);
            const RenderParams& A = params_view(KP);
            if (!RGB && A.chunked && ((s0 + S) & (kSumChunk - 1u)) == 0u && s0 + S <= s_end) chunk_flush(A, off, inpix && sub == 0, acc[0]);
        }
        const RenderParams& E = params_view(KP);
        if (inpix && sub == 0) {
            if (RGB) pixel_state_store3(E, off, reinterpret_cast<const float (&)[3]>(acc[0]), cnt);
            else pixel_state_store(E, off, acc[0], cnt);
        }
        if (E.tile_cost && lane == 0) atomicAdd(E.tile_cost + tile_i, static_cast<unsigned long long>(__builtin_readcyclecounter() - t_unit));
    }
    const RenderParams& Z = params_view(KP);
    if (lane == 0 && Z.segments && segs) atomicAdd(Z.segments, segs);
}

#ifndef MP_POOL_WPE
#define MP_POOL_WPE 8
#endif
constexpr int kPoolQueueRows = 13, kPoolStateRows = 11;
__host__ __device__ constexpr uint32_t pool_floats_per_wave(int nsub) { return static_cast<uint32_t>((kPoolQueueRows + kPoolStateRows) * 64 * nsub); }
constexpr uint32_t kPoolAlive = 1u, kPoolPrimary = 2u, kPoolQueued = 4u;

template <int NSUB>
__global__ __launch_bounds__(256) __attribute__((amdgpu_waves_per_eu(MP_POOL_WPE, 8))) void render_paths_pooled_kernel(RenderParams) {
    extern __shared__ __align__(16) unsigned char smem[];
    MP_KERNEL_PARAMS;
    constexpr int S = 8, BW = 4, BH = 2, QN = 64 * NSUB;
    const int lane = static_cast<int>(threadIdx.x) & 63;
    const int wave = __builtin_amdgcn_readfirstlane(static_cast<int>(threadIdx.x) >> 6);
    const int pix = lane / S, sub = lane % S;
    unsigned long long segs = 0;
    uint32_t qstate = blockIdx.x % kWorkQueues;
    float* q;
    uint32_t* park;
    uint2* stack;
    {
        const RenderParams& P0 = params_view(KP);
        q = P0.pool + static_cast<size_t>(blockIdx.x * 4u + static_cast<uint32_t>(wave)) * P0.pool_stride;
        park = reinterpret_cast<uint32_t*>(q + kPoolQueueRows * QN);
        stack = reinterpret_cast<uint2*>(smem + static_cast<size_t>(wave) * P0.lds_per_wave);
    }
    auto park_store = [&](int j, const Rng& rng, float L, float thr, uint32_t flags) {
        uint32_t* p = park + j * 64 + lane;
        __builtin_nontemporal_store(rng.s0.lo, p + 0 * QN); __builtin_nontemporal_store(rng.s0.hi, p + 1 * QN);
        __builtin_nontemporal_store(rng.s1.lo, p + 2 * QN); __builtin_nontemporal_store(rng.s1.hi, p + 3 * QN);
        __builtin_nontemporal_store(rng.s2.lo, p + 4 * QN); __builtin_nontemporal_store(rng.s2.hi, p + 5 * QN);
        __builtin_nontemporal_store(rng.s3.lo, p + 6 * QN); __builtin_nontemporal_store(rng.s3.hi, p + 7 * QN);
        __builtin_nontemporal_store(as_u(L), p + 8 * QN); __builtin_nontemporal_store(as_u(thr), p + 9 * QN); __builtin_nontemporal_store(flags, p + 10 * QN);
    };
    auto push_ray = [&](const DevScene& sc, const Ray& r, bool alive, uint32_t& nq, uint32_t& flags) {
        const bool queued = alive && may_hit_scene(sc, r);
        const uint64_t am = __ballot(queued);
        const uint32_t slot = nq + static_cast<uint32_t>(rank_below(am));
        if (queued) {
            q[0 * QN + slot] = r.ox; q[1 * QN + slot] = r.oy; q[2 * QN + slot] = r.oz;
            q[3 * QN + slot] = r.dx; q[4 * QN + slot] = r.dy; q[5 * QN + slot] = r.dz;
            q[6 * QN + slot] = r.ix; q[7 * QN + slot] = r.iy; q[8 * QN + slot] = r.iz;
            flags |= kPoolQueued | (slot << 8);
        }
        nq += static_cast<uint32_t>(__popcll(am));
    };
    for (;;) {
        const RenderParams& P = params_view(KP);
        const uint32_t ts = P.tile_size;
        const uint32_t bx = (ts + BW - 1) / BW, by = (ts + BH - 1) / BH, upt = bx * by, total = P.n_tiles * upt;
        MP_NEXT_UNIT(unit)
        const uint32_t b = unit % upt;
        const uint32_t tile_i = P.tile_order ? P.tile_order[unit / upt] : unit / upt;
        const uint64_t t_unit = P.tile_cost ? __builtin_readcyclecounter() : 0;
        const mp_block T = P.tiles[tile_i];
        const uint32_t px = T.min_x + (b % bx) * BW + static_cast<uint32_t>(pix % BW);
        const uint32_t py = T.min_y + (b / bx) * BH + static_cast<uint32_t>(pix / BW);
        const bool inpix = px < T.max_x && py < T.max_y;
        if (__ballot(inpix) == 0) continue;
        const size_t off = (static_cast<size_t>(tile_i) * ts * ts + static_cast<size_t>(py - T.min_y) * ts + (px - T.min_x)) * 4;
        float acc, cnt;
        pixel_state_load(P, off, inpix, sub == 0, acc, cnt);
        const uint32_t s_begin = P.s_begin, s_end = P.s_end, max_depth = P.max_depth;
        for (uint32_t s0 = s_begin & ~static_cast<uint32_t>(S * NSUB - 1); s0 < s_end; s0 += S * NSUB) {
            uint32_t nq = 0, na = 0;
#pragma nounroll
            for (int j = 0; j < NSUB; j++) {
                const uint32_t s = s0 + static_cast<uint32_t>(j * S + sub);
                const bool act = inpix && s >= s_begin && s < s_end;
                Rng rng;
                rng_zero(rng);
                Ray r;
                r.ox = r.oy = r.oz = r.dx = r.dy = r.dz = r.ix = r.iy = r.iz = 0.0f;
                {
                    const RenderParams& G = params_view(KP);
                    if (act) {
                        rng_seed(rng, sample_key(G.gen, px, py, s));
                        sample_ray_rng(G.gen, px, py, rng, r);
                    }
                }
                segs += static_cast<unsigned long long>(__popcll(__ballot(act)));
                PacketHit h;
                h.t = FLT_MAX; h.u = h.v = 0.0f; h.prim = kNoPrim;
                {
                    const RenderParams& W = params_view(KP);
                    const bool go = act && may_hit_scene(W.scene, r);
                    if (__ballot(go) != 0) {
                        RegStack rst(nullptr, lane);
                        HybridStack hst(reinterpret_cast<float*>(stack), lane, W.scene.stack_cap, W.scene.packet_stack_regs);
                        if (W.scene.stack_cap > W.scene.packet_stack_regs) trace_packet<false>(W.scene, r, go, hst, h);
                        else trace_packet<true>(W.scene, r, go, rst, h);
                    }
                }
                const RenderParams& V = params_view(KP);
                float L[1] = {0.0f}, thr[1] = {1.0f};
                bool alive = act, primary_hit = false;
                if (alive) alive = path_vertex<false, 1>(V.scene, h, 1u, max_depth, rng, r, L, thr, primary_hit);
                uint32_t flags = (alive ? kPoolAlive : 0u) | (primary_hit ? kPoolPrimary : 0u);
                push_ray(V.scene, r, alive, nq, flags);
                na += static_cast<uint32_t>(__popcll(__ballot(alive)));
                park_store(j, rng, L[0], thr[0], flags);
            }
            for (uint32_t depth = 2; depth <= max_depth && na != 0u; depth++) {
                segs += na;
                wave_mem_sync();
                if (nq != 0u) {
                    const RenderParams& W = params_view(KP);
                    trace_wave_pool<QN>(W.scene, q, stack, static_cast<int>(nq));
                }
                wave_mem_sync();
                nq = 0;
                na = 0;
    #pragma nounroll
            for (int j = 0; j < NSUB; j++) {
                    const uint32_t* p = park + j * 64 + lane;
                    uint32_t flags = __builtin_nontemporal_load(p + 10 * QN);
                    bool alive = (flags & kPoolAlive) != 0u;
                    if (__ballot(alive) == 0) continue;
                    Rng rng;
                    auto ld = [&](int row) { return static_cast<uint64_t>(__builtin_nontemporal_load(p + row * QN)); };
// ... 511 lines not shown
    rc = launch(plan.kernel, plan.grid, 256, plan.lds, st, err, P);
    if (P.pool) (void)hipFreeAsync(P.pool, st);
    return rc;
}

int launch_render_aov(const RenderLaunch& L, const mp_aov_planes_ex& planes, void* stream, std::string& err) {
    hipStream_t st = static_cast<hipStream_t>(stream);
    if (L.n_tiles == 0) return MP_OK;
    const LaunchPlan plan = plan_render_aov(L);
    if (plan.rc) return refused(plan, err);
    AovParams A;
    RenderParams& P = A.r;
    fill_render(P, L, plan);
    P.out = nullptr;
    P.chunked = 0u;
    P.max_depth = 0;
    P.segments = nullptr;
    A.shade = planes.d_shade;
    A.normal = planes.d_normal;
    A.albedo = planes.d_albedo;
    A.ids = planes.d_ids;
    A.position = planes.d_position;
    A.shade_sq = planes.d_shade_sq;
    A.park_pixel = plan.park_pixel;
    const int rc = zero_work_queues(L, st, err);
    if (rc) return rc;
    return launch(plan.kernel, plan.grid, 256, plan.lds, st, err, A);
}

int launch_render_paths_wavefront(const RenderLaunch& L, void* stream, std::string& err) {
    hipStream_t st = static_cast<hipStream_t>(stream);
    if (L.n_tiles == 0) return MP_OK;
    const WavefrontPlan plan = plan_render_paths_wavefront(L);
    if (plan.rc) return refused(plan, err);
    WfParams P;
    fill_common(P, L);
    P.lds_per_wave = plan.cam_lds_per_wave;
    P.st.nchan = plan.nchan;
    const size_t n64 = plan.n64, bin_bytes = (static_cast<size_t>(plan.nbins) + 64) * 4;
    unsigned char* ws = nullptr;
    int rc = check(hipMallocAsync(reinterpret_cast<void**>(&ws), plan.ws_bytes, st), "hipMallocAsync(path state)", err);
    if (rc) return rc;
    unsigned char* w = ws;
    auto take = [&](size_t b) { unsigned char* r = w; w += b; return r; };
    P.st.rng = reinterpret_cast<uint64_t*>(take(n64 * 32));
    P.st.ray = reinterpret_cast<float*>(take(n64 * 24));
    P.st.thr = reinterpret_cast<float*>(take(n64 * 4 * plan.nchan));
    P.st.L = reinterpret_cast<float*>(take(n64 * 4 * plan.nchan));
    P.st.hit_t = reinterpret_cast<float*>(take(n64 * 4));
    P.st.hit_prim = reinterpret_cast<uint32_t*>(take(n64 * 4));
    P.st.hit_u = reinterpret_cast<float*>(take(n64 * 4));
    P.st.hit_v = reinterpret_cast<float*>(take(n64 * 4));
    P.st.hit_inst = reinterpret_cast<uint32_t*>(take(n64 * 4));
    P.st.flags = reinterpret_cast<uint32_t*>(take(n64 * 4));
    P.st.key = reinterpret_cast<uint32_t*>(take(n64 * 4));
    P.st.idx = reinterpret_cast<uint32_t*>(take(n64 * 4));
    P.st.hist = reinterpret_cast<uint32_t*>(take(bin_bytes));
    P.st.offs = reinterpret_cast<uint32_t*>(take(bin_bytes));
    P.st.cursor = reinterpret_cast<uint32_t*>(take(bin_bytes));
    for (uint32_t tile_base = 0; tile_base < L.n_tiles && !rc; tile_base += plan.tb) {
        const uint32_t ntb = std::min(plan.tb, L.n_tiles - tile_base);
        const WavefrontBatch B = plan.batch(ntb);
        P.tiles = L.d_tiles + tile_base;
        P.n_tiles = ntb;
        P.tile_base = tile_base;
        for (uint32_t s0 = L.pass_begin; s0 < L.pass_end && !rc; s0 += plan.sc) {
            P.s0 = s0;
            P.sc = plan.sc;
            P.s_end = L.pass_end;
            P.st.n = B.n;
            P.st.nbins = B.nbins;
            P.carry_in = (L.carry_in || s0 > L.pass_begin) ? 1u : 0u;
            P.finalize = (L.finalize && s0 + plan.sc >= L.pass_end) ? 1u : 0u;
            rc = check(hipMemsetAsync(P.st.hist, 0, (static_cast<size_t>(P.st.nbins) + 1) * 4, st), "hipMemsetAsync(histogram)", err);
            if (rc) break;
            rc = check(hipMemsetAsync(P.st.flags, 0, static_cast<size_t>(P.st.n) * 4, st), "hipMemsetAsync(path flags)", err);
            if (rc) break;
            rc = launch(plan.camera, B.cam_grid, 256, plan.cam_lds, st, err, P);
            WfParams G = P;
            G.lds_per_wave = plan.trace_lds_per_wave;
            for (uint32_t depth = 1; depth <= L.max_depth && !rc; depth++) {
                P.depth = depth;
                rc = launch(plan.vertex, B.flat_grid, 256, 0, st, err, P);
                if (rc || depth == L.max_depth) break;
                rc = launch(K_WF_SCAN, 1, 1024, 0, st, err, P);
                if (!rc) rc = launch(K_WF_SCATTER, B.flat_grid, 256, 0, st, err, P);
                if (!rc) rc = launch(plan.trace, plan.trace_grid, 256, plan.trace_lds, st, err, G);
            }
            if (!rc) rc = launch(K_WF_ACCUMULATE, B.px_grid, 256, 0, st, err, P);
        }
    }
    (void)hipFreeAsync(ws, st);
    return rc;
}

int launch_trace_rays(const DevScene& sc, const float* ox, const float* oy, const float* oz, const float* dx,
                      const float* dy, const float* dz, uint64_t n, const mp_hits_soa& hits, int cu_count, void* stream,
                      std::string& err) {
    return launch_rays(kQueryClosest, sc, ox, oy, oz, dx, dy, dz, nullptr, n, &hits, nullptr, cu_count, stream, err);
}

int launch_query_rays(const DevScene& sc, const float* ox, const float* oy, const float* oz, const float* dx, const float* dy,
                      const float* dz, const float* tmax, uint64_t n, const mp_hits_soa* hits, uint8_t* occluded, int cu_count,
                      void* stream, std::string& err) {
    return launch_rays(occluded ? kQueryAnyHit : kQueryBounded, sc, ox, oy, oz, dx, dy, dz, tmax, n, hits, occluded, cu_count, stream, err);
}

int launch_set_u64(unsigned long long* d_ptr, unsigned long long value, void* stream, std::string& err) {
    return launch(K_SET_U64, 1, 1, 0, static_cast<hipStream_t>(stream), err, d_ptr, value);
}

int launch_generate_rays(const mp_camera_sampler& s, uint32_t width, uint32_t spp, uint64_t seed, mp_block block,
                         uint32_t sample, float* ox, float* oy, float* oz, float* dx, float* dy, float* dz, void* stream,
                         std::string& err) {
    const uint64_t n = static_cast<uint64_t>(block.max_x - block.min_x) * (block.max_y - block.min_y);
    if (n == 0) return MP_OK;
    RayGen G;
    fill_raygen(G, s, width, spp, seed);
    const uint32_t grid = static_cast<uint32_t>(std::min<uint64_t>((n + 255) / 256, 8192));
    return launch(K_GENERATE_RAYS, grid, 256, 0, static_cast<hipStream_t>(stream), err, G, block, sample, ox, oy, oz, dx, dy, dz);
}

int launch_untile(uint32_t width, uint32_t height, uint32_t tile_size, const mp_block* d_tiles, uint32_t n_tiles,
                  const float* d_tiles_f32, float* d_image_f32, uint8_t* d_image_u8, void* stream, std::string& err,
                  uint32_t preview_mode, uint32_t preview_samples) {
    const uint64_t n = static_cast<uint64_t>(tile_size) * tile_size * n_tiles;
    if (n == 0) return MP_OK;
    const uint32_t grid = static_cast<uint32_t>(std::min<uint64_t>((n + 255) / 256, 8192));
    const uint32_t k = std::max<uint32_t>(preview_samples, 1u);
    return launch(K_UNTILE, grid, 256, 0, static_cast<hipStream_t>(stream), err, width, height, tile_size, d_tiles, n_tiles, d_tiles_f32,
                  d_image_f32, d_image_u8, preview_mode, 1.0f / static_cast<float>(k), 1.0 / static_cast<double>(k));
}

int launch_quantise(const float* d_rgba_f32, uint8_t* d_rgba_u8, uint64_t n_pixels, void* stream, std::string& err) {
    if (n_pixels == 0) return MP_OK;
    const uint32_t grid = static_cast<uint32_t>(std::min<uint64_t>((n_pixels + 255) / 256, 8192));
    return launch(K_QUANTISE, grid, 256, 0, static_cast<hipStream_t>(stream), err, d_rgba_f32, d_rgba_u8, n_pixels);
}

}

#ifdef MP_PROF_MISSES
extern "C" int mp_prof_read8(unsigned long long* out, int reset) {
    if (hipMemcpyFromSymbol(out, HIP_SYMBOL(mp::g_prof), sizeof(unsigned long long) * 8) != hipSuccess) return 1;
    if (reset) { unsigned long long z[8] = {0, 0, 0, 0, 0, 0, 0, 0}; if (hipMemcpyToSymbol(HIP_SYMBOL(mp::g_prof), z, sizeof(z)) != hipSuccess) return 1; }
    return 0;
}
extern "C" int mp_prof_read(unsigned long long* out, int reset) {
    unsigned long long all[8];
    if (mp_prof_read8(all, reset) != 0) return 1;
    for (int i = 0; i < 4; i++) out[i] = all[i];
    return 0;
}
#endif
```

minipath_amd/csrc/mask_cache.h:

```cpp
#pragma once

#include <hip/hip_runtime.h>

#include <cfloat>
#include <cmath>
#include <cstdint>

#include "camera_rays.h"

#ifndef MP_PROF_COUNT
#define MP_PROF_COUNT(i) do { } while (0)
#endif

namespace mp {
namespace mc {
__device__ __forceinline__ float as_f(uint32_t u) { return __uint_as_float(u); }
__device__ __forceinline__ uint32_t as_u(float f) { return __float_as_uint(f); }

__device__ __forceinline__ void wave_lds_sync() {
    __builtin_amdgcn_fence(__ATOMIC_RELEASE, "wavefront");
    __builtin_amdgcn_wave_barrier();
    __builtin_amdgcn_fence(__ATOMIC_ACQUIRE, "wavefront");
}

struct Ray {
    float ox, oy, oz, dx, dy, dz, ix, iy, iz;
};

__device__ __forceinline__ float fma_dot(float ax, float ay, float az, float bx, float by, float bz) {
    return __builtin_fmaf(az, bz, __builtin_fmaf(ay, by, ax * bx));
}
__device__ __forceinline__ float fms(float a, float b, float c) { return __builtin_fmaf(a, b, -c); }

template <bool PATCH_NAN, int OCT>
__device__ __forceinline__ void slab(float bnx, float bny, float bnz, float bxx, float bxy, float bxz, const Ray& r,
                                     float limit, float& t1, float& t2) {
    float ax = (bnx - r.ox) * r.ix, ay = (bny - r.oy) * r.iy, az = (bnz - r.oz) * r.iz;
    float cx = (bxx - r.ox) * r.ix, cy = (bxy - r.oy) * r.iy, cz = (bxz - r.oz) * r.iz;
    if (PATCH_NAN) {
        ax = fmaxf(ax, -INFINITY); ay = fmaxf(ay, -INFINITY); az = fmaxf(az, -INFINITY);
        cx = fminf(cx, INFINITY); cy = fminf(cy, INFINITY); cz = fminf(cz, INFINITY);
    }
    float lox, loy, loz, hix, hiy, hiz;
    if (OCT >= 0) {
        lox = (OCT & 1) ? cx : ax; hix = (OCT & 1) ? ax : cx;
        loy = (OCT & 2) ? cy : ay; hiy = (OCT & 2) ? ay : cy;
        loz = (OCT & 4) ? cz : az; hiz = (OCT & 4) ? az : cz;
    } else {
        lox = fminf(ax, cx); loy = fminf(ay, cy); loz = fminf(az, cz);
        hix = fmaxf(ax, cx); hiy = fmaxf(ay, cy); hiz = fmaxf(az, cz);
    }
    t1 = fmaxf(fmaxf(lox, 0.0f), fmaxf(loy, loz));
    t2 = fminf(fminf(hix, limit), fminf(hiy, hiz));
}

#ifndef MP_MCACHE_PAD
#define MP_MCACHE_PAD 0.25f
#endif
#ifndef MP_NODE_ENTRIES
#define MP_NODE_ENTRIES 64
#endif
#ifndef MP_LEAF_ENTRIES
#define MP_LEAF_ENTRIES 128
#endif
#ifndef MP_ARENA_ENTRIES
#define MP_ARENA_ENTRIES 384
#endif
#ifndef MP_ARENA_ROOM
#define MP_ARENA_ROOM 384
#endif
#ifndef MP_NODE_SLOT_MASK
#define MP_NODE_SLOT_MASK 0xFFFFFFFFu
#endif
constexpr int kMaskCacheEntries = MP_NODE_ENTRIES;
constexpr int kMaskCacheHeader = 32;
constexpr int kLeafCacheEntries = MP_LEAF_ENTRIES;
constexpr int kLeafTagBase = kMaskCacheHeader + kMaskCacheEntries;
constexpr int kLeafMaskBase = kLeafTagBase + kLeafCacheEntries;
constexpr int kNodeListBase = kLeafMaskBase + 2 * kLeafCacheEntries;
constexpr int kArenaBase = kNodeListBase + kMaskCacheEntries;
constexpr int kArenaRoom = MP_ARENA_ROOM;
constexpr int kArenaEntries = MP_ARENA_ENTRIES;
constexpr int kMaskCacheDwords = kArenaBase + kArenaRoom;
constexpr int kArenaTopSlot = kMaskCacheHeader + kMaskCacheEntries - 1;
constexpr int kRootListSlot = kNodeListBase + kMaskCacheEntries - 1;
static_assert((kMaskCacheEntries & (kMaskCacheEntries - 1)) == 0 && kMaskCacheEntries >= 4, "the node table's slot mask");
static_assert(kArenaEntries >= 16 && kArenaEntries <= kArenaRoom, "an unexpanded list (at most 16 entries) fits the empty arena");
static_assert((kLeafMaskBase % 2) == 0 && (kMaskCacheDwords % 4) == 0, "LDS alignment of the leaf masks / of the next wave's header");
constexpr float kCoordCap = 1073741824.0f;
struct MaskCache {
    uint32_t* lds;
};
#define MP_DPP_STEP6(CTRL)                                                                                              \
    "v_min_f32_dpp %0, %0, %0 " CTRL "\n\tv_min_f32_dpp %1, %1, %1 " CTRL "\n\tv_min_f32_dpp %2, %2, %2 " CTRL "\n\t"         \
    "v_max_f32_dpp %3, %3, %3 " CTRL "\n\tv_max_f32_dpp %4, %4, %4 " CTRL "\n\tv_max_f32_dpp %5, %5, %5 " CTRL "\n\t"
__device__ __forceinline__ void wave_min3_max3(float (&mn)[3], float (&mx)[3]) {
    asm volatile("s_nop 1\n\t"
                 MP_DPP_STEP6("quad_perm:[1,0,3,2] row_mask:0xf bank_mask:0xf")
                 MP_DPP_STEP6("quad_perm:[2,3,0,1] row_mask:0xf bank_mask:0xf")
                 MP_DPP_STEP6("row_half_mirror row_mask:0xf bank_mask:0xf")
                 MP_DPP_STEP6("row_mirror row_mask:0xf bank_mask:0xf")
                 MP_DPP_STEP6("row_bcast:15 row_mask:0xa bank_mask:0xf")
                 MP_DPP_STEP6("row_bcast:31 row_mask:0xc bank_mask:0xf")
                 : "+v"(mn[0]), "+v"(mn[1]), "+v"(mn[2]), "+v"(mx[0]), "+v"(mx[1]), "+v"(mx[2]));
}
__device__ __forceinline__ bool mask_cache_ray_ok(const Ray& r) {
    constexpr uint32_t kMag = 0x7FFFFFFFu;
    const uint32_t mo = max(max(as_u(r.ox) & kMag, as_u(r.oy) & kMag), as_u(r.oz) & kMag);
    const uint32_t mi = max(max(as_u(r.ix) & kMag, as_u(r.iy) & kMag), as_u(r.iz) & kMag);
    const uint32_t md = max(max(as_u(r.dx) & kMag, as_u(r.dy) & kMag), as_u(r.dz) & kMag);
    constexpr uint32_t kCapO = 0x4E800000u , kCapI = 0x7F7FFFFFu , kCapD = 0x40000000u ;
    static_assert(kCoordCap == 1073741824.0f, "kCapO is kCoordCap's bit pattern");
    return static_cast<int32_t>((mo - (kCapO + 1u)) & (mi - (kCapI + 1u)) & (md - (kCapD + 1u))) < 0;
}
constexpr int kHdrState = 12;
constexpr int hdr_lo(int g) { return g == 2 ? kHdrState + 1 : g * 6; }
__device__ __forceinline__ float bounds_deviation(float v, float lo, float hi) {
    return fabsf(v - __builtin_amdgcn_fmed3f(v, lo, hi));
}
__device__ __forceinline__ void mask_cache_begin_pass(const MaskCache& mc, const Ray& r, bool active, uint32_t oct) {
    const int lane = static_cast<int>(threadIdx.x) & 63;
    float* hdr = reinterpret_cast<float*>(mc.lds);
    float h[20];
#pragma unroll
    for (int i = 0; i < 5; i++) {
        const float4 q = reinterpret_cast<const float4*>(mc.lds)[i];
        h[4 * i] = q.x; h[4 * i + 1] = q.y; h[4 * i + 2] = q.z; h[4 * i + 3] = q.w;
    }
    const uint32_t state = __builtin_amdgcn_readfirstlane(as_u(h[kHdrState]));
    const bool same = state == (oct | 0x100u);
    const float val[3][3] = {{r.ox, r.oy, r.oz}, {r.ix, r.iy, r.iz}, {r.dx, r.dy, r.dz}};
    float dev = 0.0f;
#pragma unroll
    for (int g = 0; g < 3; g++) {
#pragma unroll
        for (int k = 0; k < 3; k++) dev = fmaxf(dev, bounds_deviation(val[g][k], h[hdr_lo(g) + k], h[hdr_lo(g) + 3 + k]));
    }
    if (__ballot(active && (!same || dev != 0.0f)) != 0) {
        float pmin[3][3], pmax[3][3];
#pragma unroll
        for (int g = 0; g < 3; g++) {
#pragma unroll
            for (int k = 0; k < 3; k++) {
                pmin[g][k] = active ? val[g][k] : INFINITY;
                pmax[g][k] = active ? val[g][k] : -INFINITY;
            }
            wave_min3_max3(pmin[g], pmax[g]);
        }
#pragma unroll
        for (int g = 0; g < 3; g++) {
#pragma unroll
            for (int k = 0; k < 3; k++) {
                float lo = pmin[g][k], hi = pmax[g][k];
                if (same) { lo = fminf(lo, h[hdr_lo(g) + k]); hi = fmaxf(hi, h[hdr_lo(g) + 3 + k]); }
                const float pad = (hi - lo) * MP_MCACHE_PAD;
                float wlo = lo - pad, whi = hi + pad;
                if (g == 1) {
                    if ((wlo < 0.0f) != (lo < 0.0f) || wlo == 0.0f) wlo = lo;
                    if ((whi < 0.0f) != (hi < 0.0f) || whi == 0.0f) whi = hi;
                    if (!(fabsf(wlo) < INFINITY)) wlo = lo;
                    if (!(fabsf(whi) < INFINITY)) whi = hi;
                } else {
                    const float cap = g == 0 ? 2.0f * kCoordCap : 2.0f;
                    wlo = fmaxf(wlo, -cap); whi = fminf(whi, cap);
                }
                pmin[g][k] = wlo; pmax[g][k] = whi;
            }
        }
        MP_PROF_COUNT(3);
        wave_lds_sync();
        if (lane == 63) {
#pragma unroll
            for (int g = 0; g < 3; g++) {
#pragma unroll
                for (int k = 0; k < 3; k++) { hdr[hdr_lo(g) + k] = pmin[g][k]; hdr[hdr_lo(g) + 3 + k] = pmax[g][k]; }
            }
            mc.lds[kHdrState] = oct | 0x100u;
        }
        int l_ = lane;
        asm volatile("" : "+v"(l_));
#pragma unroll
        for (int i = 0; i < (kMaskCacheEntries + kLeafCacheEntries) / 64; i++) mc.lds[kMaskCacheHeader + i * 64 + l_] = 0xFFFFFFFFu;
        wave_lds_sync();
    }
}
#ifndef MP_MCACHE_MARGIN
#define MP_MCACHE_MARGIN 0.015625f
#endif
__device__ __forceinline__ void mask_cache_begin_unit(const MaskCache& mc, const mp_camera_sampler& s, float jitter_scale, uint32_t x0,
                                                      uint32_t x1, uint32_t y0, uint32_t y1) {
    const int lane = static_cast<int>(threadIdx.x) & 63;
    Ray r;
    float f[3];
    camera_film(s, (lane & 1) ? static_cast<float>(x1) + (jitter_scale + (-0.5f)) : static_cast<float>(x0) + (-0.5f),
                (lane & 2) ? static_cast<float>(y1) + (jitter_scale + (-0.5f)) : static_cast<float>(y0) + (-0.5f), f);
    camera_lens_ray(s, f, (lane & 4) ? 1.0f : -1.0f, (lane & 8) ? 1.0f : -1.0f, r);
    const uint64_t nx = __ballot(r.ix < 0.0f), ny = __ballot(r.iy < 0.0f), nz = __ballot(r.iz < 0.0f);
    const bool adopt = __ballot(!mask_cache_ray_ok(r)) == 0 && (nx == 0 || ~nx == 0) && (ny == 0 || ~ny == 0) && (nz == 0 || ~nz == 0);
    if (!adopt) {
        if (lane == 0) mc.lds[kHdrState] = 0xFFFFFFFFu;
        wave_lds_sync();
        return;
    }
    const uint32_t oct = (nx ? 1u : 0u) | (ny ? 2u : 0u) | (nz ? 4u : 0u);
    float pmin[3][3] = {{r.ox, r.oy, r.oz}, {r.ix, r.iy, r.iz}, {r.dx, r.dy, r.dz}}, pmax[3][3];
#pragma unroll
    for (int g = 0; g < 3; g++) {
#pragma unroll
        for (int k = 0; k < 3; k++) pmax[g][k] = pmin[g][k];
        wave_min3_max3(pmin[g], pmax[g]);
    }
    float* hdr = reinterpret_cast<float*>(mc.lds);
    if (lane == 63) {
#pragma unroll
        for (int g = 0; g < 3; g++) {
#pragma unroll
            for (int k = 0; k < 3; k++) {
                const float lo = pmin[g][k], hi = pmax[g][k];
                const float pad = (hi - lo) * MP_MCACHE_MARGIN;
                float wlo = lo - pad, whi = hi + pad;
                if (g == 1) {
                    if ((wlo < 0.0f) != (lo < 0.0f) || wlo == 0.0f) wlo = lo;
                    if ((whi < 0.0f) != (hi < 0.0f) || whi == 0.0f) whi = hi;
                    if (!(fabsf(wlo) < INFINITY)) wlo = lo;
                    if (!(fabsf(whi) < INFINITY)) whi = hi;
                } else {
                    const float cap = g == 0 ? 2.0f * kCoordCap : 2.0f;
                    wlo = fmaxf(wlo, -cap); whi = fminf(whi, cap);
                }
                hdr[hdr_lo(g) + k] = wlo; hdr[hdr_lo(g) + 3 + k] = whi;
            }
        }
        mc.lds[kHdrState] = oct | 0x100u;
    }
    MP_PROF_COUNT(3);
#pragma unroll
    for (int i = 0; i < (kMaskCacheEntries + kLeafCacheEntries) / 64; i++) mc.lds[kMaskCacheHeader + i * 64 + lane] = 0xFFFFFFFFu;
    wave_lds_sync();
}
template <int OCT>
__device__ __forceinline__ bool bounds_may_hit(const float* b, const float bmn[3], const float bmx[3]) {
    float L[3], U[3];
#pragma unroll
    for (int k = 0; k < 3; k++) {
        const float y = bmn[k] - b[3 + k], z = bmx[k] - b[k];
        const float lo_src = ((OCT >> k) & 1) ? z : y, hi_src = ((OCT >> k) & 1) ? y : z;
        L[k] = fminf(lo_src * b[6 + k], lo_src * b[9 + k]);
        U[k] = fmaxf(hi_src * b[6 + k], hi_src * b[9 + k]);
    }
    const float t1 = fmaxf(fmaxf(L[0], 0.0f), fmaxf(L[1], L[2])), t2 = fminf(U[0], fminf(U[1], U[2]));
    return !(t1 > t2);
}

constexpr uint32_t kNullLink = 0xFFFFFFF8u;
constexpr uint32_t kListOverflow = 0xFFFFFFFFu;
constexpr uint32_t kEmptyLeafBit = 0x80000000u;
constexpr int kListDepth = 64;
__device__ __forceinline__ uint32_t node_slot(uint32_t node) {
    return min(node & static_cast<uint32_t>(kMaskCacheEntries - 1) & MP_NODE_SLOT_MASK, static_cast<uint32_t>(kMaskCacheEntries - 2));
}
template <class Kept>
__device__ __forceinline__ uint32_t unit_list_build(const float4* __restrict__ recs, uint32_t* mcache, uint32_t node, uint32_t slots, Kept kept) {
    const uint32_t lane = threadIdx.x & 63u;
    const float* b = reinterpret_cast<const float*>(mcache);
    node = __builtin_amdgcn_readfirstlane(node);
    slots = __builtin_amdgcn_readfirstlane(slots);
    auto kept_of = [&](uint32_t n, float4& c0, float4& c1) -> uint32_t {
        bool keep = false;
        c0 = make_float4(0.0f, 0.0f, 0.0f, 0.0f); c1 = c0;
        if (lane < slots) {
            const float4* r = recs + (static_cast<size_t>(n) * slots + lane) * 2;
            c0 = r[0]; c1 = r[1];
            const float bmn[3] = {c0.x, c0.y, c0.z}, bmx[3] = {c0.w, c1.x, c1.y};
            keep = as_u(c1.z) != kNullLink && kept(b, bmn, bmx);
        }
        return __builtin_amdgcn_readfirstlane(static_cast<uint32_t>(__ballot(keep)));
    };
    float4 c0, c1;
    uint32_t mask = kept_of(node, c0, c1);
    const uint32_t top = ~__builtin_amdgcn_readfirstlane(mcache[kArenaTopSlot]);
    if (top > static_cast<uint32_t>(kArenaEntries) || top + static_cast<uint32_t>(__popc(mask)) > static_cast<uint32_t>(kArenaEntries)) {
        MP_PROF_COUNT(5);
        wave_lds_sync();
#pragma unroll
        for (int i = 0; i < (kMaskCacheEntries + 63) / 64; i++)
            if (i * 64 + static_cast<int>(lane) < kMaskCacheEntries) mcache[kMaskCacheHeader + i * 64 + static_cast<int>(lane)] = 0xFFFFFFFFu;
        wave_lds_sync();
        return kListOverflow;
    }
    const uint32_t room = static_cast<uint32_t>(kArenaEntries) - top;
    uint32_t used = 0u, pend = static_cast<uint32_t>(__popc(mask)), cur = node;
    int st_node = 0, st_mask = 0, depth = 0;
    for (;;) {
        if (mask == 0u) {
            while (mask == 0u && depth > 0) {
                depth--;
                cur = static_cast<uint32_t>(__builtin_amdgcn_readlane(st_node, depth));
                mask = static_cast<uint32_t>(__builtin_amdgcn_readlane(st_mask, depth));
            }
            if (mask == 0u) break;
            if (lane < slots) {
                const float4* r = recs + (static_cast<size_t>(cur) * slots + lane) * 2;
                c0 = r[0]; c1 = r[1];
            }
        }
        const uint32_t j = static_cast<uint32_t>(__builtin_ctz(mask));
        mask &= mask - 1u;
        pend--;
        const uint32_t rec = cur * slots + j;
        auto from_lane = [&](float v) { return as_f(static_cast<uint32_t>(__builtin_amdgcn_readlane(static_cast<int>(as_u(v)), static_cast<int>(j)))); };
        const float4 p0 = make_float4(from_lane(c0.x), from_lane(c0.y), from_lane(c0.z), from_lane(c0.w));
        const float4 p1 = make_float4(from_lane(c1.x), from_lane(c1.y), from_lane(c1.z), 0.0f);
        const uint32_t link = as_u(p1.z);
        bool emit = true;
        if ((link & 63u) == 0u) {
            const uint32_t m = link >> 6;
            float4 g0, g1;
            const uint32_t km = kept_of(m, g0, g1);
            const bool sticks_out = ((km >> lane) & 1u) != 0u && lane < slots &&
                                    !(p0.x <= g0.x && p0.y <= g0.y && p0.z <= g0.z && g0.w <= p0.w && g1.x <= p1.x && g1.y <= p1.y);
            if (km == 0u) {
                emit = false;
            } else if (__ballot(sticks_out) == 0 && depth < kListDepth && used + pend + static_cast<uint32_t>(__popc(km)) <= room) {
                if (mask != 0u) {
                    asm volatile("s_mov_b32 m0, %2\n\ts_nop 0\n\tv_writelane_b32 %0, %3, m0\n\tv_writelane_b32 %1, %4, m0"
                                 : "+v"(st_node), "+v"(st_mask) : "s"(depth), "s"(__builtin_amdgcn_readfirstlane(cur)), "s"(__builtin_amdgcn_readfirstlane(mask)) : "m0");
                    depth++;
                }
                cur = m; mask = km; pend += static_cast<uint32_t>(__popc(km));
                c0 = g0; c1 = g1;
                emit = false;
            }
        }
        if (emit) {
            if (lane == 0u) mcache[static_cast<uint32_t>(kArenaBase) + top + used] = rec;
            used++;
        }
    }
    const uint32_t val = ((static_cast<uint32_t>(kArenaBase) + top) << 16) | used;
    if (lane == 0u) {
        const uint32_t slot = node_slot(node);
        mcache[static_cast<uint32_t>(kMaskCacheHeader) + slot] = node;
        mcache[static_cast<uint32_t>(kNodeListBase) + slot] = val;
        mcache[kArenaTopSlot] = ~(top + used);
    }
    wave_lds_sync();
    return val;
}

struct Iv {
    float lo, hi;
};
__device__ __forceinline__ Iv iv_neg(const Iv a) { return Iv{-a.hi, -a.lo}; }
__device__ __forceinline__ Iv iv_mul_c(const Iv a, const float c) {
    const float p = a.lo * c, q = a.hi * c;
    return Iv{fminf(p, q), fmaxf(p, q)};
}
__device__ __forceinline__ Iv iv_mul(const Iv a, const Iv b) {
    const float p1 = a.lo * b.lo, p2 = a.lo * b.hi, p3 = a.hi * b.lo, p4 = a.hi * b.hi;
    return Iv{fminf(fminf(p1, p2), fminf(p3, p4)), fmaxf(fmaxf(p1, p2), fmaxf(p3, p4))};
}
__device__ __forceinline__ Iv iv_fma_c(const Iv a, const float c, const Iv z) {
    return Iv{fminf(__builtin_fmaf(a.lo, c, z.lo), __builtin_fmaf(a.hi, c, z.lo)), fmaxf(__builtin_fmaf(a.lo, c, z.hi), __builtin_fmaf(a.hi, c, z.hi))};
}
__device__ __forceinline__ Iv iv_fma(const Iv a, const Iv b, const Iv z) {
    const float l1 = __builtin_fmaf(a.lo, b.lo, z.lo), l2 = __builtin_fmaf(a.lo, b.hi, z.lo), l3 = __builtin_fmaf(a.hi, b.lo, z.lo), l4 = __builtin_fmaf(a.hi, b.hi, z.lo);
    const float h1 = __builtin_fmaf(a.lo, b.lo, z.hi), h2 = __builtin_fmaf(a.lo, b.hi, z.hi), h3 = __builtin_fmaf(a.hi, b.lo, z.hi), h4 = __builtin_fmaf(a.hi, b.hi, z.hi);
    return Iv{fminf(fminf(l1, l2), fminf(l3, l4)), fmaxf(fmaxf(h1, h2), fmaxf(h3, h4))};
}
__device__ __forceinline__ bool tri_may_hit(const float* b, const float (&v0)[3], const float (&e1)[3], const float (&e2)[3]) {
    const Iv d[3] = {Iv{b[13], b[16]}, Iv{b[14], b[17]}, Iv{b[15], b[18]}};
    const Iv h[3] = {iv_fma_c(d[1], e2[2], iv_neg(iv_mul_c(d[2], e2[1]))), iv_fma_c(d[2], e2[0], iv_neg(iv_mul_c(d[0], e2[2]))),
                     iv_fma_c(d[0], e2[1], iv_neg(iv_mul_c(d[1], e2[0])))};
    const Iv det = iv_fma_c(h[2], e1[2], iv_fma_c(h[1], e1[1], iv_mul_c(h[0], e1[0])));
    if (!(det.lo > 0.0f || det.hi < 0.0f)) return true;
    const Iv inv = Iv{1.0f / det.hi, 1.0f / det.lo};
    if (!(fabsf(inv.lo) < INFINITY && fabsf(inv.hi) < INFINITY)) return true;
    const Iv s[3] = {Iv{b[0] - v0[0], b[3] - v0[0]}, Iv{b[1] - v0[1], b[4] - v0[1]}, Iv{b[2] - v0[2], b[5] - v0[2]}};
    const Iv u = iv_mul(inv, iv_fma(s[2], h[2], iv_fma(s[1], h[1], iv_mul(s[0], h[0]))));
    const Iv q[3] = {iv_fma_c(s[1], e1[2], iv_neg(iv_mul_c(s[2], e1[1]))), iv_fma_c(s[2], e1[0], iv_neg(iv_mul_c(s[0], e1[2]))),
                     iv_fma_c(s[0], e1[1], iv_neg(iv_mul_c(s[1], e1[0])))};
    const Iv v = iv_mul(inv, iv_fma(d[2], q[2], iv_fma(d[1], q[1], iv_mul(d[0], q[0]))));
    const Iv t = iv_mul(inv, iv_fma_c(q[2], e2[2], iv_fma_c(q[1], e2[1], iv_mul_c(q[0], e2[0]))));
    const bool miss = u.hi < 0.0f || v.hi < 0.0f || (u.lo + v.lo) > 1.0f || t.hi < 0.0f;
    return !miss;
}
// ... 27 lines not shown
```

minipath_amd/csrc/mask_probe.hip:

```cpp
#include <hip/hip_runtime.h>

#include <cfloat>
#include <cstdint>

#include "mask_cache.h"

namespace {

using namespace mp::mc;

constexpr int kCounters = 8;
constexpr float kOrgCap = 2.0f * kCoordCap;

__device__ __forceinline__ uint64_t mix64(uint64_t z) {
    z = (z ^ (z >> 30)) * 0xbf58476d1ce4e5b9ull;
    z = (z ^ (z >> 27)) * 0x94d049bb133111ebull;
    return z ^ (z >> 31);
}
__device__ __forceinline__ uint64_t hsh(uint64_t seed, uint64_t c, uint32_t k) { return mix64(seed ^ mix64(c * 0x10000ull + k)); }
__device__ __forceinline__ float unit(uint64_t h) { return static_cast<float>(static_cast<uint32_t>(h >> 40)) * 0x1p-24f; }

__device__ __forceinline__ void record_case(unsigned long long* out, bool bad, uint64_t idx, bool hit, bool rejected, bool edge_only) {
    if ((threadIdx.x & 63) != 0) return;
    atomicAdd(out + 1, 1ull);
// ... 345 lines not shown
        float t1, t2;
        slab<false, OCT>(bmn[0], bmn[1], bmn[2], bmx[0], bmx[1], bmx[2], r, FLT_MAX, t1, t2);
        const bool pass = t1 <= t2;
        if (s < 2) edge |= pass; else inner |= pass;
        if (rec) {
            uint32_t* rr = rec + kDumpHead + j * kDumpRay;
            for (int k = 0; k < 6; k++) rr[k] = as_u(x[k]);
            rr[6] = as_u(t1); rr[7] = as_u(t2); rr[8] = 0u; rr[9] = pass ? 1u : 0u;
        }
    }
    const bool any_edge = __ballot(edge) != 0, any_inner = __ballot(inner) != 0, any = any_edge || any_inner;
    if (rec && lane < 20u) rec[lane] = as_u(b[lane]);
    if (rec && lane == 20u) {
        for (int k = 0; k < 3; k++) { rec[20 + k] = as_u(bmn[k]); rec[23 + k] = as_u(bmx[k]); }
        rec[26] = OCT;
        rec[35] = keep ? 1u : 0u;
    }
    record_case(out, !keep && any, c, any, !keep, any_edge && !any_inner);
}

__global__ void box_kernel(uint64_t seed, uint64_t base, uint64_t ncases, unsigned long long* out, uint32_t* dump) {
    const uint64_t c = base + (static_cast<uint64_t>(blockIdx.x) * blockDim.x + threadIdx.x) / 64u;
    if (c >= ncases) return;
    switch (static_cast<int>(c & 7u)) {
        case 0: box_case<0>(seed, c, out, dump); break;
        case 1: box_case<1>(seed, c, out, dump); break;
        case 2: box_case<2>(seed, c, out, dump); break;
        case 3: box_case<3>(seed, c, out, dump); break;
        case 4: box_case<4>(seed, c, out, dump); break;
        case 5: box_case<5>(seed, c, out, dump); break;
        case 6: box_case<6>(seed, c, out, dump); break;
        default: box_case<7>(seed, c, out, dump); break;
    }
}

__constant__ uint32_t kOther[32] = {
    0x00000000u, 0x80000000u, 0x3F800000u, 0xBF000000u, 0x00000001u, 0x807FFFFFu, 0x00800000u, 0x3FFFFFFFu,
    0x40000000u, 0xC0000000u, 0x40000001u, 0xC0000001u, 0x4E800000u, 0xCE800000u, 0x4E7FFFFFu, 0x4E800001u,
    0xCE800001u, 0x7F7FFFFFu, 0xFF7FFFFFu, 0x7F800000u, 0xFF800000u, 0x7FC00000u, 0xFFC00000u, 0x7F800001u,
    0xFFFFFFFFu, 0x4F000000u, 0x1F800000u, 0x40400000u, 0x3F7FFFFFu, 0xBE800000u, 0x00400000u, 0x7FFFFFFFu};
__device__ __forceinline__ bool ray_ok_plain(const float (&x)[9]) {
    bool ok = true;
    for (int k = 0; k < 3; k++) ok = ok && fabsf(x[k]) <= kCoordCap;
    for (int k = 3; k < 6; k++) ok = ok && fabsf(x[k]) <= FLT_MAX;
    for (int k = 6; k < 9; k++) ok = ok && fabsf(x[k]) <= 2.0f;
    return ok;
}
constexpr uint32_t kOkPerThread = 16;
__global__ void ray_ok_kernel(uint64_t seed, int comp, uint64_t base, unsigned long long* out) {
    const uint64_t tid = base + static_cast<uint64_t>(blockIdx.x) * blockDim.x + threadIdx.x;
    bool bad = false;
    uint64_t first = ~0ull;
    for (uint32_t i = 0; i < kOkPerThread; i++) {
        const uint64_t idx = tid * kOkPerThread + i;
        const uint64_t h = mix64(seed ^ (idx * 0x9E3779B97F4A7C15ull) ^ static_cast<uint64_t>(comp));
        float x[9];
#pragma unroll
        for (int k = 0; k < 9; k++) {
            const uint32_t sel = static_cast<uint32_t>(h >> (6 * k)) & 63u;
            x[k] = as_f(kOther[(sel & 0x30u) ? (sel & 7u) : (sel & 31u)]);
        }
#pragma unroll
        for (int k = 0; k < 9; k++) if (k == comp) x[k] = as_f(static_cast<uint32_t>(idx));
        Ray r;
        r.ox = x[0]; r.oy = x[1]; r.oz = x[2]; r.ix = x[3]; r.iy = x[4]; r.iz = x[5]; r.dx = x[6]; r.dy = x[7]; r.dz = x[8];
        if (mask_cache_ray_ok(r) != ray_ok_plain(x) && !bad) { bad = true; first = idx; }
    }
    const uint64_t m = __ballot(bad);
    if (bad) { atomicAdd(out + 0, 1ull); atomicMin(out + 2, static_cast<unsigned long long>(first)); }
    if ((threadIdx.x & 63u) == 0u) atomicAdd(out + 1, 64ull * kOkPerThread);
    (void)m;
}

__global__ void dev_kernel(uint64_t seed, int mode, uint64_t base, uint32_t n, const float* set, unsigned long long* out) {
    const uint64_t idx = base + static_cast<uint64_t>(blockIdx.x) * blockDim.x + threadIdx.x;
    float v, lo, hi;
    if (mode == 0) {
        if (idx >= static_cast<uint64_t>(n) * n * n) return;
        v = set[idx % n]; lo = set[(idx / n) % n]; hi = set[idx / (static_cast<uint64_t>(n) * n)];
    } else {
        const uint64_t h = mix64(seed ^ mix64(idx)), h2 = mix64(h ^ 0x5555u), h3 = mix64(h2 ^ 0xAAAAu);
        const float a = pick(h, 0, 254), bb = (h & 0x30000u) == 0u ? pick(h2, 0, 254) : a + pick(h2, 0, 254);
        lo = fminf(a, bb); hi = fmaxf(a, bb);
        const uint32_t k = static_cast<uint32_t>(h3 & 7u);
        v = k == 0u ? lo : k == 1u ? hi : k == 2u ? step(lo, false) : k == 3u ? step(hi, true) : k == 4u ? step(lo, true)
          : k == 5u ? step(hi, false) : k == 6u ? lerp_in(lo, hi, unit(h3)) : pick(h3, 0, 254);
    }
    const bool valid = fabsf(v) <= FLT_MAX && fabsf(lo) <= FLT_MAX && fabsf(hi) <= FLT_MAX && lo <= hi;
    const bool bad = valid && ((bounds_deviation(v, lo, hi) != 0.0f) != (v < lo || v > hi));
    if (bad) { atomicAdd(out + 0, 1ull); atomicMin(out + 2, static_cast<unsigned long long>(idx)); }
    const uint64_t nv = __popcll(__ballot(valid));
    if ((threadIdx.x & 63u) == __ffsll(static_cast<unsigned long long>(__ballot(true))) - 1 && nv) atomicAdd(out + 1, nv);
}

constexpr int kPasses = 64;
constexpr int kEntryDwords = kMaskCacheDwords - kMaskCacheHeader;
static_assert(kEntryDwords % 64 == 0 && (kLeafMaskBase - kMaskCacheHeader) % 64 == 0, "entries: whole dwords per lane");
__device__ __forceinline__ uint32_t entry_val(uint64_t seed, uint64_t c, int i, uint32_t lane) {
    return static_cast<uint32_t>(hsh(seed, c, 5000u + static_cast<uint32_t>(i) * 64u + lane));
}
__device__ __forceinline__ bool same_or_zero(float a, float b) { return as_u(a) == as_u(b) || (a == 0.0f && b == 0.0f); }

__global__ void __launch_bounds__(256) pass_kernel(uint64_t seed, unsigned long long* out) {
    __shared__ __align__(16) uint32_t lds[4 * kMaskCacheDwords];
    __shared__ float rays[4][9][64];
    const uint32_t w = threadIdx.x >> 6, lane = threadIdx.x & 63u;
    const uint64_t wave = static_cast<uint64_t>(blockIdx.x) * 4u + w;
    uint32_t* const base = lds + w * kMaskCacheDwords;
    const MaskCache mc{base};
    if (lane < static_cast<uint32_t>(kMaskCacheHeader)) base[lane] = static_cast<uint32_t>(hsh(seed, wave, 100u + lane));
    if (lane == 0u) base[kHdrState] = 0xFFFFFFFFu;
    wave_lds_sync();
    uint32_t oct = static_cast<uint32_t>(hsh(seed, wave, 99)) & 7u;
    for (int pass = 0; pass < kPasses; pass++) {
        const uint64_t c = wave * kPasses + static_cast<uint64_t>(pass);
        const uint64_t hp = hsh(seed, c, 0);
        if ((hp & 7u) == 0u) oct = static_cast<uint32_t>(hp >> 8) & 7u;
        for (int i = 0; i < kEntryDwords / 64; i++) base[kMaskCacheHeader + i * 64 + static_cast<int>(lane)] = entry_val(seed, c, i, lane);
        wave_lds_sync();
        float oh[32];
        for (int i = 0; i < 32; i++) oh[i] = as_f(base[i]);
        const bool valid = as_u(oh[kHdrState]) == (oct | 0x100u);
        const uint32_t ak = static_cast<uint32_t>(hp >> 16) % 7u;
        const uint64_t rnd = hsh(seed, c, 1);
        const uint64_t am = ak == 0u ? ~0ull : ak == 1u ? 0ull : ak == 2u ? 1ull << ((hp >> 24) & 63u) : ak == 3u ? ~0ull >> 1
                          : ak == 4u ? ((hp >> 30) & 1u ? 0xAAAAAAAAAAAAAAAAull : 0x5555555555555555ull) : ak == 5u ? rnd : rnd | ~0ull << 60;
        const bool active = (am >> lane) & 1u;
        const bool may_leave = ((hp >> 40) & 1u) != 0u;
        float val[9];
        for (int g = 0; g < 3; g++) {
            for (int k = 0; k < 3; k++) {
                const uint64_t h = hsh(seed, c, 10u + lane * 9u + static_cast<uint32_t>(g * 3 + k));
                const uint32_t pos = static_cast<uint32_t>(h & 7u);
                const float lo = oh[hdr_lo(g) + k], hi = oh[hdr_lo(g) + 3 + k];
                float x;
                if (valid && lo <= hi && pos < 3u) x = lerp_in(lo, hi, unit(h));
                else if (valid && lo <= hi && pos < 5u) x = pos == 3u ? lo : hi;
                else if (valid && lo <= hi && pos == 5u && may_leave) x = (h >> 8) & 1u ? step(lo, false) : step(hi, true);
                else if (valid && lo <= hi && !may_leave) x = lo;
                else x = g == 2 ? pick(h, 127 - 20, 127 + 1) : pick(h, 127 - 20, g == 0 ? 127 + 30 : 127 + 20);
                if (g == 0) x = clampf(x, -kCoordCap, kCoordCap);
                if (g == 2) x = clampf(x, -2.0f, 2.0f);
                if (g == 1) {
                    x = clampf(fabsf(x), 0x1p-149f, FLT_MAX);
                    if ((oct >> k) & 1u) x = -x;
                }
                val[g * 3 + k] = active ? x : as_f(static_cast<uint32_t>(h >> 32) | ((h & 0x30u) ? 0x7F800000u : 0u));
            }
        }
        for (int i = 0; i < 9; i++) rays[w][i][lane] = val[i];
        Ray r;
        r.ox = val[0]; r.oy = val[1]; r.oz = val[2]; r.ix = val[3]; r.iy = val[4]; r.iz = val[5]; r.dx = val[6]; r.dy = val[7]; r.dz = val[8];
        wave_lds_sync();
        mask_cache_begin_pass(mc, r, active, oct);
        wave_lds_sync();
        bool outside = false;
        for (int g = 0; g < 3; g++)
            for (int k = 0; k < 3; k++) outside = outside || val[g * 3 + k] < oh[hdr_lo(g) + k] || val[g * 3 + k] > oh[hdr_lo(g) + 3 + k];
        const bool rewrite = __ballot(active && (!valid || outside)) != 0;
        float nh[32];
        for (int i = 0; i < 32; i++) nh[i] = as_f(base[i]);
        bool bad = false;
        if (rewrite) {
            for (int g = 0; g < 3; g++) {
                for (int k = 0; k < 3; k++) {
                    float lo = INFINITY, hi = -INFINITY;
                    for (int l = 0; l < 64; l++) {
                        if (!((am >> l) & 1u)) continue;
                        const float x = rays[w][g * 3 + k][l];
                        if (x < lo) lo = x;
                        if (x > hi) hi = x;
                    }
                    if (valid) { lo = oh[hdr_lo(g) + k] < lo ? oh[hdr_lo(g) + k] : lo; hi = oh[hdr_lo(g) + 3 + k] > hi ? oh[hdr_lo(g) + 3 + k] : hi; }
                    const float pad = (hi - lo) * MP_MCACHE_PAD;
                    float wlo = lo - pad, whi = hi + pad;
                    if (g == 1) {
                        const bool neg = ((oct >> k) & 1u) != 0u;
                        if (!(neg ? (wlo < 0.0f && wlo > -INFINITY) : (wlo > 0.0f && wlo < INFINITY))) wlo = lo;
                        if (!(neg ? (whi < 0.0f && whi > -INFINITY) : (whi > 0.0f && whi < INFINITY))) whi = hi;
                    } else {
                        const float cap = g == 0 ? kOrgCap : 2.0f;
                        if (wlo < -cap) wlo = -cap;
                        if (whi > cap) whi = cap;
                    }
                    bad = bad || !same_or_zero(nh[hdr_lo(g) + k], wlo) || !same_or_zero(nh[hdr_lo(g) + 3 + k], whi);
                }
            }
            bad = bad || as_u(nh[kHdrState]) != (oct | 0x100u);
        } else {
            for (int i = 0; i < 19; i++) bad = bad || as_u(nh[i]) != as_u(oh[i]);
        }
        for (int i = 19; i < 32; i++) bad = bad || as_u(nh[i]) != as_u(oh[i]);
        if (as_u(nh[kHdrState]) == (oct | 0x100u)) {
            for (int k = 0; k < 3; k++) {
                const bool neg = ((oct >> k) & 1u) != 0u;
                const float ilo = nh[6 + k], ihi = nh[9 + k];
                bad = bad || !(ilo <= ihi) || !(fabsf(ilo) <= FLT_MAX) || !(fabsf(ihi) <= FLT_MAX);
                bad = bad || (neg ? !(ihi < 0.0f) : !(ilo > 0.0f));
                bad = bad || !(nh[k] >= -kOrgCap && nh[k] <= nh[3 + k] && nh[3 + k] <= kOrgCap);
                bad = bad || !(nh[13 + k] >= -2.0f && nh[13 + k] <= nh[16 + k] && nh[16 + k] <= 2.0f);
            }
        }
        bool lane_bad = false;
        for (int g = 0; g < 3; g++)
            for (int k = 0; k < 3; k++) lane_bad = lane_bad || (active && !(val[g * 3 + k] >= nh[hdr_lo(g) + k] && val[g * 3 + k] <= nh[hdr_lo(g) + 3 + k]));
        for (int i = 0; i < kEntryDwords / 64; i++) {
            const uint32_t e = base[kMaskCacheHeader + i * 64 + static_cast<int>(lane)];
            const bool cleared = rewrite && i < (kLeafMaskBase - kMaskCacheHeader) / 64;
            lane_bad = lane_bad || e != (cleared ? 0xFFFFFFFFu : entry_val(seed, c, i, lane));
        }
        bad = bad || __ballot(lane_bad) != 0;
        if (lane == 0u) {
            atomicAdd(out + 1, 1ull);
            if (rewrite) atomicAdd(out + 6, 1ull);
            if (bad) { atomicAdd(out + 0, 1ull); atomicMin(out + 2, static_cast<unsigned long long>(c)); }
        }
        wave_lds_sync();
    }
}

constexpr int kUnitOut = 20;
struct SamplerArg {
    mp_camera_sampler s;
};
__global__ void __launch_bounds__(256) unit_kernel(SamplerArg cam, float jitter_scale, const uint32_t* blocks, uint32_t n, uint32_t* out) {
    __shared__ __align__(16) uint32_t lds[4 * kMaskCacheDwords];
    const uint32_t w = threadIdx.x >> 6, lane = threadIdx.x & 63u;
    const uint32_t unit = blockIdx.x * 4u + w;
    if (unit >= n) return;
    uint32_t* const base = lds + w * kMaskCacheDwords;
    if (lane < static_cast<uint32_t>(kMaskCacheHeader)) base[lane] = static_cast<uint32_t>(hsh(0x0E17ull, unit, lane));
    constexpr int kTags = kLeafMaskBase - kMaskCacheHeader;
    for (int i = 0; i < kTags / 64; i++) base[kMaskCacheHeader + i * 64 + static_cast<int>(lane)] = static_cast<uint32_t>(i * 64) + lane;
    wave_lds_sync();
    mask_cache_begin_unit(MaskCache{base}, cam.s, jitter_scale, blocks[4 * unit], blocks[4 * unit + 1], blocks[4 * unit + 2], blocks[4 * unit + 3]);
    wave_lds_sync();
    uint32_t cleared = 0u;
    for (int i = 0; i < kTags / 64; i++) cleared += static_cast<uint32_t>(__popcll(__ballot(base[kMaskCacheHeader + i * 64 + static_cast<int>(lane)] == 0xFFFFFFFFu)));
    if (lane < 19u) out[kUnitOut * unit + lane] = base[lane];
    if (lane == 19u) out[kUnitOut * unit + 19u] = cleared;
}

constexpr int kListOut = 4 + kArenaRoom;
template <int OCT>
__device__ __noinline__ uint32_t list_slow(const float4* __restrict__ recs, uint32_t* mcache, uint32_t node, uint32_t slots) {
    return unit_list_build(recs, mcache, node, slots,
                           [](const float* b, const float bmn[3], const float bmx[3]) { return bounds_may_hit<OCT>(b, bmn, bmx); });
}
__global__ void __launch_bounds__(256) list_kernel(const float4* recs, uint32_t slots, const uint32_t* headers, const uint32_t* cases, uint32_t n,
                                                   uint32_t* out) {
    __shared__ __align__(16) uint32_t lds[4 * kMaskCacheDwords];
    const uint32_t w = threadIdx.x >> 6, lane = threadIdx.x & 63u;
    const uint32_t c = blockIdx.x * 4u + w;
    if (c >= n) return;
    uint32_t* const base = lds + w * kMaskCacheDwords;
    for (uint32_t i = lane; i < static_cast<uint32_t>(kMaskCacheDwords); i += 64u)
        base[i] = i < static_cast<uint32_t>(kMaskCacheHeader) ? headers[32u * c + i] : i < static_cast<uint32_t>(kLeafMaskBase) ? 0xFFFFFFFFu : 0xDEAD0000u + i;
    wave_lds_sync();
    const uint32_t node = cases[2u * c], top0 = cases[2u * c + 1u];
    if (lane == 0u) base[kArenaTopSlot] = ~top0;
    wave_lds_sync();
    uint32_t val;
    switch (__builtin_amdgcn_readfirstlane(base[kHdrState]) & 7u) {
        case 0: val = list_slow<0>(recs, base, node, slots); break;
        case 1: val = list_slow<1>(recs, base, node, slots); break;
        case 2: val = list_slow<2>(recs, base, node, slots); break;
        case 3: val = list_slow<3>(recs, base, node, slots); break;
        case 4: val = list_slow<4>(recs, base, node, slots); break;
        case 5: val = list_slow<5>(recs, base, node, slots); break;
        case 6: val = list_slow<6>(recs, base, node, slots); break;
        default: val = list_slow<7>(recs, base, node, slots); break;
    }
    wave_lds_sync();
    uint32_t* const o = out + static_cast<size_t>(c) * kListOut;
    if (lane == 0u) {
        const uint32_t slot = node_slot(node);
        o[0] = val; o[1] = ~base[kArenaTopSlot]; o[2] = base[static_cast<uint32_t>(kMaskCacheHeader) + slot]; o[3] = base[static_cast<uint32_t>(kNodeListBase) + slot];
    }
    for (uint32_t i = lane; i < static_cast<uint32_t>(kArenaRoom); i += 64u) o[4u + i] = base[static_cast<uint32_t>(kArenaBase) + i];
}

template <class F>
int run(F launch, unsigned long long* host) {
    (void)hipGetLastError();
    unsigned long long* dev = nullptr;
    unsigned long long init[kCounters] = {0ull, 0ull, ~0ull, 0ull, 0ull, 0ull, 0ull, 0ull};
    hipError_t e = hipMalloc(&dev, sizeof(init));
    if (e != hipSuccess) return static_cast<int>(e);
    e = hipMemcpy(dev, init, sizeof(init), hipMemcpyHostToDevice);
    if (e == hipSuccess) {
        launch(dev);
        e = hipGetLastError();
        if (e == hipSuccess) e = hipDeviceSynchronize();
        if (e == hipSuccess) e = hipMemcpy(host, dev, sizeof(init), hipMemcpyDeviceToHost);
    }
    const hipError_t ef = hipFree(dev);
    return static_cast<int>(e != hipSuccess ? e : ef);
}
void merge(unsigned long long* acc, const unsigned long long* r) {
    for (int i = 0; i < kCounters; i++) if (i != 2) acc[i] += r[i];
    if (r[2] < acc[2]) acc[2] = r[2];
}
void reset(unsigned long long* acc) {
    for (int i = 0; i < kCounters; i++) acc[i] = 0ull;
    acc[2] = ~0ull;
}
constexpr uint64_t kCasesPerLaunch = 1ull << 20;

template <class K>
int run_cases(K kernel, uint64_t seed, uint64_t ncases, uint32_t* dump_dev, unsigned long long* out) {
    unsigned long long acc[kCounters];
    reset(acc);
    for (uint64_t c0 = 0; c0 < ncases; c0 += kCasesPerLaunch) {
        const uint64_t n = ncases - c0 < kCasesPerLaunch ? ncases - c0 : kCasesPerLaunch;
        unsigned long long r[kCounters];
        if (int rc = run([&](unsigned long long* d) {
                hipLaunchKernelGGL(kernel, dim3(static_cast<uint32_t>((n + 3) / 4)), dim3(256), 0, 0, seed, c0, c0 + n, d, dump_dev);
            }, r))
            return rc;
        merge(acc, r);
    }
    for (int i = 0; i < kCounters; i++) out[i] = acc[i];
    return 0;
}

}

extern "C" {
int mp_mask_probe_tri(uint64_t seed, uint64_t ncases, unsigned long long* out) { return run_cases(tri_kernel, seed, ncases, nullptr, out); }
int mp_mask_probe_exits(uint64_t seed, uint64_t ncases, unsigned long long* out) { return run_cases(exit_kernel, seed, ncases, nullptr, out); }
int mp_mask_probe_box(uint64_t seed, uint64_t ncases, unsigned long long* out) { return run_cases(box_kernel, seed, ncases, nullptr, out); }
int mp_mask_probe_dump_dwords() { return kDumpCase; }
int mp_mask_probe_dump(int kind, uint64_t seed, uint64_t ncases, uint32_t* host, unsigned long long* out) {
    (void)hipGetLastError();
    uint32_t* dev = nullptr;
    const size_t bytes = static_cast<size_t>(ncases) * kDumpCase * sizeof(uint32_t);
    hipError_t e = hipMalloc(&dev, bytes);
    if (e != hipSuccess) return static_cast<int>(e);
    e = hipMemset(dev, 0, bytes);
    int rc = static_cast<int>(e);
    if (e == hipSuccess) rc = kind == 0 ? run_cases(tri_kernel, seed, ncases, dev, out) : run_cases(box_kernel, seed, ncases, dev, out);
    if (rc == 0) rc = static_cast<int>(hipMemcpy(host, dev, bytes, hipMemcpyDeviceToHost));
    const hipError_t ef = hipFree(dev);
    return rc != 0 ? rc : static_cast<int>(ef);
}
int mp_mask_probe_ray_ok(uint64_t seed, unsigned long long* out) {
    unsigned long long acc[kCounters];
    reset(acc);
    constexpr uint64_t kThreads = (1ull << 32) / kOkPerThread, kBlocks = kThreads / 256;
    for (int comp = 0; comp < 9; comp++) {
        unsigned long long r[kCounters];
        if (int rc = run([&](unsigned long long* d) {
                hipLaunchKernelGGL(ray_ok_kernel, dim3(static_cast<uint32_t>(kBlocks)), dim3(256), 0, 0, seed, comp, 0ull, d);
            }, r))
            return rc;
        if (r[2] != ~0ull) r[2] += static_cast<unsigned long long>(comp) << 32;
        merge(acc, r);
    }
    for (int i = 0; i < kCounters; i++) out[i] = acc[i];
    return 0;
}
int mp_mask_probe_dev(uint64_t seed, const float* set, uint32_t n, uint64_t nrandom, unsigned long long* out) {
    (void)hipGetLastError();
    float* dset = nullptr;
    hipError_t e = hipMalloc(&dset, sizeof(float) * (n ? n : 1u));
    if (e != hipSuccess) return static_cast<int>(e);
    e = hipMemcpy(dset, set, sizeof(float) * n, hipMemcpyHostToDevice);
    int rc = static_cast<int>(e);
    unsigned long long acc[kCounters];
    reset(acc);
    const uint64_t ntrip = static_cast<uint64_t>(n) * n * n;
    if (rc == 0 && ntrip) {
        unsigned long long r[kCounters];
        rc = run([&](unsigned long long* d) {
            hipLaunchKernelGGL(dev_kernel, dim3(static_cast<uint32_t>((ntrip + 255) / 256)), dim3(256), 0, 0, seed, 0, 0ull, n, dset, d);
        }, r);
        if (rc == 0) merge(acc, r);
    }
    if (rc == 0 && nrandom) {
        unsigned long long r[kCounters];
        rc = run([&](unsigned long long* d) {
            hipLaunchKernelGGL(dev_kernel, dim3(static_cast<uint32_t>((nrandom + 255) / 256)), dim3(256), 0, 0, seed, 1, 0ull, n, dset, d);
        }, r);
        if (rc == 0) { if (r[2] != ~0ull) r[2] += 1ull << 40; merge(acc, r); }
    }
    const hipError_t ef = hipFree(dset);
    if (rc != 0) return rc;
    for (int i = 0; i < kCounters; i++) out[i] = acc[i];
    return static_cast<int>(ef);
}
int mp_mask_probe_unit(const float* sampler, float jitter_scale, const uint32_t* blocks, uint32_t n, uint32_t* out, uint32_t* ntags,
                       float* margin) {
    (void)hipGetLastError();
    *ntags = static_cast<uint32_t>(kLeafMaskBase - kMaskCacheHeader);
    *margin = MP_MCACHE_MARGIN;
    if (n == 0u) return 0;
    SamplerArg cam;
    const float* p = sampler;
    for (int k = 0; k < 3; k++) { cam.s.center[k] = p[k]; cam.s.up[k] = p[3 + k]; cam.s.right[k] = p[6 + k]; cam.s.film_origin_offset[k] = p[9 + k]; }
    cam.s.pixel_scale = p[12]; cam.s.lens_radius = p[13]; cam.s.lens_weight = p[14];
    uint32_t *dblocks = nullptr, *dout = nullptr;
    hipError_t e = hipMalloc(&dblocks, sizeof(uint32_t) * 4u * n);
    if (e == hipSuccess) e = hipMalloc(&dout, sizeof(uint32_t) * kUnitOut * n);
    if (e == hipSuccess) e = hipMemcpy(dblocks, blocks, sizeof(uint32_t) * 4u * n, hipMemcpyHostToDevice);
    if (e == hipSuccess) {
        hipLaunchKernelGGL(unit_kernel, dim3((n + 3u) / 4u), dim3(256), 0, 0, cam, jitter_scale, dblocks, n, dout);
        e = hipGetLastError();
        if (e == hipSuccess) e = hipDeviceSynchronize();
        if (e == hipSuccess) e = hipMemcpy(out, dout, sizeof(uint32_t) * kUnitOut * n, hipMemcpyDeviceToHost);
    }
    (void)hipFree(dblocks);
    (void)hipFree(dout);
    return static_cast<int>(e);
}
int mp_mask_probe_pass(uint64_t seed, uint64_t nwaves, unsigned long long* out) {
    return run([&](unsigned long long* d) {
        hipLaunchKernelGGL(pass_kernel, dim3(static_cast<uint32_t>(nwaves / 4)), dim3(256), 0, 0, seed, d);
    }, out);
}
int mp_mask_probe_list_dwords() { return kListOut; }
int mp_mask_probe_list(const uint32_t* recs, uint32_t n_nodes, uint32_t slots, const uint32_t* headers, const uint32_t* cases, uint32_t ncases,
                       uint32_t* out, uint32_t* info) {
    (void)hipGetLastError();
    if (info) { info[0] = static_cast<uint32_t>(kArenaEntries); info[1] = static_cast<uint32_t>(kMaskCacheEntries); info[2] = static_cast<uint32_t>(kArenaBase); }
    if (slots != 8u && slots != 16u) return -1;
    for (uint32_t c = 0; c < ncases; c++)
        if (cases[2u * c] >= n_nodes || cases[2u * c + 1u] > static_cast<uint32_t>(kArenaEntries)) return -1;
    for (size_t i = 0; i < static_cast<size_t>(n_nodes) * slots; i++) {
        const uint32_t link = recs[i * 8u + 6u];
        if (link != kNullLink && (link & 63u) == 0u && (link >> 6) >= n_nodes) return -1;
    }
    if (ncases == 0u) return 0;
    uint32_t *drecs = nullptr, *dhdr = nullptr, *dcases = nullptr, *dout = nullptr;
    const size_t rec_bytes = sizeof(uint32_t) * 8u * slots * n_nodes, out_bytes = sizeof(uint32_t) * kListOut * static_cast<size_t>(ncases);
    hipError_t e = hipMalloc(&drecs, rec_bytes);
    if (e == hipSuccess) e = hipMalloc(&dhdr, sizeof(uint32_t) * 32u * ncases);
    if (e == hipSuccess) e = hipMalloc(&dcases, sizeof(uint32_t) * 2u * ncases);
    if (e == hipSuccess) e = hipMalloc(&dout, out_bytes);
    if (e == hipSuccess) e = hipMemcpy(drecs, recs, rec_bytes, hipMemcpyHostToDevice);
    if (e == hipSuccess) e = hipMemcpy(dhdr, headers, sizeof(uint32_t) * 32u * ncases, hipMemcpyHostToDevice);
    if (e == hipSuccess) e = hipMemcpy(dcases, cases, sizeof(uint32_t) * 2u * ncases, hipMemcpyHostToDevice);
    if (e == hipSuccess) {
        hipLaunchKernelGGL(list_kernel, dim3((ncases + 3u) / 4u), dim3(256), 0, 0, reinterpret_cast<const float4*>(drecs), slots, dhdr, dcases, ncases, dout);
        e = hipGetLastError();
        if (e == hipSuccess) e = hipDeviceSynchronize();
        if (e == hipSuccess) e = hipMemcpy(out, dout, out_bytes, hipMemcpyDeviceToHost);
    }
    (void)hipFree(drecs); (void)hipFree(dhdr); (void)hipFree(dcases); (void)hipFree(dout);
    return static_cast<int>(e);
}
}
```

Before: 37760.

## Add short-circuit pass entry reusing cached wave verdict for mask-cache walk

Adds a cached verdict word to the mask-cache LDS header recording whether the pass bounds are strict and lie inside the scene pre-box. A new trace_pass_cached entry first tries a short path that reuses this verdict to skip the per-ray pre-box test, NaN/inf ballots and octant ballots, and falls back to the full classification otherwise. The aim is to cut per-pass ballot and scene-culling overhead in the mask-cache render kernels. In exchange it adds header state that has to be reset per unit, plus a verification probe kernel, and the short path could pick the wrong walk if the verdict goes stale.

```diff
diff --git a/minipath_amd/csrc/group_walk.h b/minipath_amd/csrc/group_walk.h
--- a/minipath_amd/csrc/group_walk.h
+++ b/minipath_amd/csrc/group_walk.h
@@ -167,18 +167,8 @@
     else trace_wave_impl<false, true, QS>(sc, q, stack_base, nrays);
 }
 
-__device__ __forceinline__ bool may_hit_scene(const DevScene& sc, const Ray& r) {
-    if (!sc.has_pre) return true;
-    float ax = (sc.pre_min[0] - r.ox) * r.ix, ay = (sc.pre_min[1] - r.oy) * r.iy, az = (sc.pre_min[2] - r.oz) * r.iz;
-    float cx = (sc.pre_max[0] - r.ox) * r.ix, cy = (sc.pre_max[1] - r.oy) * r.iy, cz = (sc.pre_max[2] - r.oz) * r.iz;
-    ax = (ax != ax) ? -INFINITY : ax; ay = (ay != ay) ? -INFINITY : ay; az = (az != az) ? -INFINITY : az;
-    cx = (cx != cx) ? INFINITY : cx; cy = (cy != cy) ? INFINITY : cy; cz = (cz != cz) ? INFINITY : cz;
-    float lox = fminf(ax, cx), loy = fminf(ay, cy), loz = fminf(az, cz);
-    float hix = fmaxf(ax, cx), hiy = fmaxf(ay, cy), hiz = fmaxf(az, cz);
-    float t1 = fmaxf(fmaxf(lox, 0.0f), fmaxf(loy, loz));
-    float t2 = fminf(fminf(hix, FLT_MAX), fminf(hiy, hiz));
-    return t1 <= t2;
-}
+__device__ __forceinline__ PreBox scene_pre_box(const DevScene& sc) { return PreBox{sc.has_pre, sc.pre_min, sc.pre_max}; }
+__device__ __forceinline__ bool may_hit_scene(const DevScene& sc, const Ray& r) { return pre_box_may_hit(scene_pre_box(sc), r); }
 
 __device__ __forceinline__ uint32_t resolve_normal(const DevScene& sc, uint32_t prim, float u, float v, float n[3]) {
     const float4* sh = reinterpret_cast<const float4*>(sc.shade) + static_cast<size_t>(prim) * 3;
diff --git a/minipath_amd/csrc/kernels.hip b/minipath_amd/csrc/kernels.hip
--- a/minipath_amd/csrc/kernels.hip
+++ b/minipath_amd/csrc/kernels.hip
@@ -14,7 +14,7 @@
 #ifdef MP_PROF_MISSES
 namespace mp {
 namespace {
-__device__ unsigned long long g_prof[8];
+__device__ unsigned long long g_prof[9];
 }
 }
 #define MP_PROF_COUNT(i) do { if ((threadIdx.x & 63u) == 0u) atomicAdd(&g_prof[i], 1ull); } while (0)
@@ -543,57 +543,76 @@
     return true;
 }
 
-template <bool OCTANTS, class Stack, bool MC = false>
-__device__ __forceinline__ void trace_packet(const DevScene& sc, const Ray& r, bool active, Stack& st, PacketHit& hit,
-                                             const MaskCache& mc = MaskCache{nullptr}) {
-    if (OCTANTS && MC) {
-        if (__ballot(active & !mask_cache_ray_ok(r)) != 0) {
-            const bool slow = active && (fabsf(r.ix) == INFINITY || fabsf(r.iy) == INFINITY || fabsf(r.iz) == INFINITY);
-            if (__ballot(slow) != 0) trace_packet_impl<2, -1>(sc, r, active, st, hit);
-            else trace_packet_impl<1, -1>(sc, r, active, st, hit);
-            return;
-        }
-    } else {
-        const bool slow = active && (fabsf(r.ix) == INFINITY || fabsf(r.iy) == INFINITY || fabsf(r.iz) == INFINITY);
-        if (__ballot(slow) != 0) {
-            trace_packet_impl<2, -1>(sc, r, active, st, hit);
-            return;
-        }
+template <bool OCTANTS, class Stack>
+__device__ __forceinline__ void trace_packet(const DevScene& sc, const Ray& r, bool active, Stack& st, PacketHit& hit) {
+    const bool slow = active && (fabsf(r.ix) == INFINITY || fabsf(r.iy) == INFINITY || fabsf(r.iz) == INFINITY);
+    if (__ballot(slow) != 0) {
+        trace_packet_impl<2, -1>(sc, r, active, st, hit);
+        return;
     }
     if (OCTANTS && sc.boxes_ordered) {
         const uint64_t am = __ballot(active);
         const uint64_t nx = __ballot(active && r.ix < 0.0f), ny = __ballot(active && r.iy < 0.0f), nz = __ballot(active && r.iz < 0.0f);
         if ((nx == 0 || nx == am) && (ny == 0 || ny == am) && (nz == 0 || nz == am)) {
             const uint32_t oct = (nx ? 1u : 0u) | (ny ? 2u : 0u) | (nz ? 4u : 0u);
-            if (MC) {
-                mask_cache_begin_pass(mc, r, active, oct);
-                bool done;
-                switch (oct) {
-                    case 0: done = trace_packet_cached<0>(sc, r, active, hit, mc.lds); break;
-                    case 1: done = trace_packet_cached<1>(sc, r, active, hit, mc.lds); break;
-                    case 2: done = trace_packet_cached<2>(sc, r, active, hit, mc.lds); break;
-                    case 3: done = trace_packet_cached<3>(sc, r, active, hit, mc.lds); break;
-                    case 4: done = trace_packet_cached<4>(sc, r, active, hit, mc.lds); break;
-                    case 5: done = trace_packet_cached<5>(sc, r, active, hit, mc.lds); break;
-                    case 6: done = trace_packet_cached<6>(sc, r, active, hit, mc.lds); break;
-                    default: done = trace_packet_cached<7>(sc, r, active, hit, mc.lds); break;
-                }
-                if (done) return;
-            } else {
-                switch (oct) {
-                    case 0: trace_packet_impl<1, 0>(sc, r, active, st, hit); return;
-                    case 1: trace_packet_impl<1, 1>(sc, r, active, st, hit); return;
-                    case 2: trace_packet_impl<1, 2>(sc, r, active, st, hit); return;
-                    case 3: trace_packet_impl<1, 3>(sc, r, active, st, hit); return;
-                    case 4: trace_packet_impl<1, 4>(sc, r, active, st, hit); return;
-                    case 5: trace_packet_impl<1, 5>(sc, r, active, st, hit); return;
-                    case 6: trace_packet_impl<1, 6>(sc, r, active, st, hit); return;
-                    default: trace_packet_impl<1, 7>(sc, r, active, st, hit); return;
-                }
+            switch (oct) {
+                case 0: trace_packet_impl<1, 0>(sc, r, active, st, hit); return;
+                case 1: trace_packet_impl<1, 1>(sc, r, active, st, hit); return;
+                case 2: trace_packet_impl<1, 2>(sc, r, active, st, hit); return;
+                case 3: trace_packet_impl<1, 3>(sc, r, active, st, hit); return;
+                case 4: trace_packet_impl<1, 4>(sc, r, active, st, hit); return;
+                case 5: trace_packet_impl<1, 5>(sc, r, active, st, hit); return;
+                case 6: trace_packet_impl<1, 6>(sc, r, active, st, hit); return;
+                default: trace_packet_impl<1, 7>(sc, r, active, st, hit); return;
             }
         }
     }
     trace_packet_impl<1, -1>(sc, r, active, st, hit);
+}
+template <bool KIND0, class Stack>
+__device__ __forceinline__ void trace_pass_cached(const DevScene& sc, const Ray& r, bool act, Stack& st, PacketHit& hit, const MaskCache& mc) {
+    bool go = act;
+#ifdef MP_PROF_NOWALK
+    uint32_t walk = kWalkNone;
+#else
+#ifdef MP_NO_SHORT_ENTRY
+    uint32_t walk = kWalkNone;
+#else
+    uint32_t walk = pass_entry_short(mc, r, act, !KIND0 || sc.kind == 0u, sc.boxes_ordered != 0u);
+#endif
+    if (walk == kWalkNone) {
+        go = act && (!KIND0 || sc.kind == 0u) && may_hit_scene(sc, r);
+        if (__ballot(go) == 0) return;
+        walk = kWalkGeneric;
+        if (__ballot(go & !mask_cache_ray_ok(r)) != 0) {
+            const bool slow = go && (fabsf(r.ix) == INFINITY || fabsf(r.iy) == INFINITY || fabsf(r.iz) == INFINITY);
+            if (__ballot(slow) != 0) walk = kWalkLiteral;
+        } else if (sc.boxes_ordered) {
+            const uint64_t am = __ballot(go);
+            const uint64_t nx = __ballot(go && r.ix < 0.0f), ny = __ballot(go && r.iy < 0.0f), nz = __ballot(go && r.iz < 0.0f);
+            if ((nx == 0 || nx == am) && (ny == 0 || ny == am) && (nz == 0 || nz == am)) {
+                walk = (nx ? 1u : 0u) | (ny ? 2u : 0u) | (nz ? 4u : 0u);
+                mask_cache_begin_pass(mc, r, go, walk, scene_pre_box(sc));
+            }
+        }
+    }
+#endif
+    bool done = false;
+    switch (walk) {
+        case 0: done = trace_packet_cached<0>(sc, r, go, hit, mc.lds); break;
+        case 1: done = trace_packet_cached<1>(sc, r, go, hit, mc.lds); break;
+        case 2: done = trace_packet_cached<2>(sc, r, go, hit, mc.lds); break;
+        case 3: done = trace_packet_cached<3>(sc, r, go, hit, mc.lds); break;
+        case 4: done = trace_packet_cached<4>(sc, r, go, hit, mc.lds); break;
+        case 5: done = trace_packet_cached<5>(sc, r, go, hit, mc.lds); break;
+        case 6: done = trace_packet_cached<6>(sc, r, go, hit, mc.lds); break;
+        case 7: done = trace_packet_cached<7>(sc, r, go, hit, mc.lds); break;
+        case kWalkNone: return;
+        default: break;
+    }
+    if (done) return;
+    if (walk == kWalkLiteral) trace_packet_impl<2, -1>(sc, r, go, st, hit);
+    else trace_packet_impl<1, -1>(sc, r, go, st, hit);
 }
 
 template <class T>
@@ -850,7 +869,7 @@
         if (MCACHE) {
             const RenderParams& C = params_view(KP);
             const uint32_t ux = T.min_x + (b % bx) * BW, uy = T.min_y + (b / bx) * BH;
-            mask_cache_begin_unit(mc, C.gen.s, C.gen.jitter_scale, ux, min(ux + BW, T.max_x) - 1u, uy, min(uy + BH, T.max_y) - 1u);
+            mask_cache_begin_unit(mc, C.gen.s, C.gen.jitter_scale, ux, min(ux + BW, T.max_x) - 1u, uy, min(uy + BH, T.max_y) - 1u, scene_pre_box(C.scene));
         }
         const uint32_t s_begin = P.s_begin, s_end = P.s_end;
         for (uint32_t s0 = s_begin & ~static_cast<uint32_t>(S - 1); s0 < s_end; s0 += S) {
@@ -876,6 +895,10 @@
                         RegStack st(lds, lane);
                         trace_packet_objects<(S >= 8 && S <= 32)>(W.scene, r, act, st, h, hinst);
                     }
+                } else if constexpr (MCACHE) {
+                    static_assert(!(MCACHE && LDS_STACK), "the cached walk keeps its frames in registers");
+                    RegStack st(lds, lane);
+                    trace_pass_cached<true>(W.scene, r, act, st, h, mc);
                 } else {
 #ifdef MP_PROF_NOWALK
                     const bool go = false;
@@ -888,7 +911,7 @@
                             trace_packet<false>(W.scene, r, go, st, h);
                         } else {
                             RegStack st(lds, lane);
-                            trace_packet<((S >= 8 && S <= 32) || MCACHE), RegStack, MCACHE>(W.scene, r, go, st, h, mc);
+                            trace_packet<(S >= 8 && S <= 32)>(W.scene, r, go, st, h);
                         }
                     }
                 }
@@ -1139,7 +1162,7 @@
                 park[0] = a0; park[1] = a1;
                 if (U.park_pixel > 32u) park[2] = a2;
             }
-            if (MCACHE && lane == 0) mc.lds[kHdrState] = 0xFFFFFFFFu;
+            if (MCACHE && lane == 0) { mc.lds[kHdrState] = 0xFFFFFFFFu; mc.lds[kHdrVerdict] = 0u; }
             wave_lds_sync();
         }
         const uint32_t s_end = P.s_end;
@@ -1168,6 +1191,10 @@
                         RegStack st(lds, lane);
                         trace_packet_objects<(S == 16)>(W.scene, r, act, st, h, hinst);
                     }
+                } else if constexpr (MCACHE) {
+                    static_assert(!(MCACHE && LDS_STACK), "the cached walk keeps its frames in registers");
+                    RegStack st(lds, lane);
+                    trace_pass_cached<true>(W.scene, r, act, st, h, mc);
                 } else {
                     const bool go = act && W.scene.kind == 0u && may_hit_scene(W.scene, r);
                     if (__ballot(go) != 0) {
@@ -1176,7 +1203,7 @@
                             trace_packet<false>(W.scene, r, go, st, h);
                         } else {
                             RegStack st(lds, lane);
-                            trace_packet<(S == 16 || MCACHE), RegStack, MCACHE>(W.scene, r, go, st, h, mc);
+                            trace_packet<(S == 16)>(W.scene, r, go, st, h);
                         }
                     }
                 }
@@ -1287,7 +1314,7 @@
         if (RGB) pixel_state_load3(P, off, inpix, reinterpret_cast<float (&)[3]>(acc[0]), cnt);
         else pixel_state_load(P, off, inpix, sub == 0, acc[0], cnt);
         if (MCACHE) {
-            if (lane == 0) mc.lds[kHdrState] = 0xFFFFFFFFu;
+            if (lane == 0) { mc.lds[kHdrState] = 0xFFFFFFFFu; mc.lds[kHdrVerdict] = 0u; }
             wave_lds_sync();
         }
         const uint32_t s_begin = P.s_begin, s_end = P.s_end, max_depth = P.max_depth;
@@ -1325,13 +1352,16 @@
                         HybridStack hst(reinterpret_cast<float*>(stack), lane, W.scene.stack_cap, W.scene.packet_stack_regs);
                         if (W.scene.stack_cap > W.scene.packet_stack_regs) trace_packet_objects<false>(W.scene, r, alive, hst, h, hinst);
                         else trace_packet_objects<(S >= 8)>(W.scene, r, alive, rst, h, hinst);
+                    } else if (depth == 1 && MCACHE && W.scene.stack_cap <= W.scene.packet_stack_regs) {
+                        RegStack rst(nullptr, lane);
+                        trace_pass_cached<false>(W.scene, r, alive, rst, h, mc);
                     } else if (depth == 1) {
                         const bool go = alive && may_hit_scene(W.scene, r);
                         if (__ballot(go) != 0) {
                             RegStack rst(nullptr, lane);
                             HybridStack hst(reinterpret_cast<float*>(stack), lane, W.scene.stack_cap, W.scene.packet_stack_regs);
                             if (W.scene.stack_cap > W.scene.packet_stack_regs) trace_packet<false>(W.scene, r, go, hst, h);
-                            else trace_packet<(S >= 8), RegStack, MCACHE>(W.scene, r, go, rst, h, mc);
+                            else trace_packet<(S >= 8)>(W.scene, r, go, rst, h);
                         }
                     } else {
                         GroupHit gh;
@@ -2149,4 +2179,9 @@
     for (int i = 0; i < 4; i++) out[i] = all[i];
     return 0;
 }
+extern "C" int mp_prof_read9(unsigned long long* out, int reset) {
+    if (hipMemcpyFromSymbol(out + 8, HIP_SYMBOL(mp::g_prof), sizeof(unsigned long long), sizeof(unsigned long long) * 8) != hipSuccess) return 1;
+    if (reset) { unsigned long long z = 0; if (hipMemcpyToSymbol(HIP_SYMBOL(mp::g_prof), &z, sizeof(z), sizeof(unsigned long long) * 8) != hipSuccess) return 1; }
+    return mp_prof_read8(out, reset);
+}
 #endif
diff --git a/minipath_amd/csrc/mask_cache.h b/minipath_amd/csrc/mask_cache.h
--- a/minipath_amd/csrc/mask_cache.h
+++ b/minipath_amd/csrc/mask_cache.h
@@ -118,7 +118,39 @@
 __device__ __forceinline__ float bounds_deviation(float v, float lo, float hi) {
     return fabsf(v - __builtin_amdgcn_fmed3f(v, lo, hi));
 }
-__device__ __forceinline__ void mask_cache_begin_pass(const MaskCache& mc, const Ray& r, bool active, uint32_t oct) {
+constexpr int kHdrVerdict = 19;
+constexpr uint32_t kVerdictStrict = 1u, kVerdictInsidePre = 2u;
+struct PreBox {
+    uint32_t has;
+    const float* mn;
+    const float* mx;
+};
+__device__ __forceinline__ void verdict_fold(uint32_t& verdict, int g, int k, uint32_t oct, float lo, float hi, const PreBox& pre) {
+    bool strict, inside = true;
+    if (g == 0) {
+        strict = fabsf(lo) <= kCoordCap && fabsf(hi) <= kCoordCap;
+        if (pre.has) inside = pre.mn[k] <= lo && hi <= pre.mx[k] && fabsf(pre.mn[k]) < INFINITY && fabsf(pre.mx[k]) < INFINITY;
+    } else if (g == 1) {
+        strict = ((oct >> k) & 1u) ? (lo > -INFINITY && hi < 0.0f) : (lo > 0.0f && hi < INFINITY);
+    } else {
+        strict = fabsf(lo) <= 2.0f && fabsf(hi) <= 2.0f;
+    }
+    if (!strict) verdict &= ~kVerdictStrict;
+    if (!inside) verdict &= ~kVerdictInsidePre;
+}
+__device__ __forceinline__ bool pre_box_may_hit(const PreBox& pre, const Ray& r) {
+    if (!pre.has) return true;
+    float ax = (pre.mn[0] - r.ox) * r.ix, ay = (pre.mn[1] - r.oy) * r.iy, az = (pre.mn[2] - r.oz) * r.iz;
+    float cx = (pre.mx[0] - r.ox) * r.ix, cy = (pre.mx[1] - r.oy) * r.iy, cz = (pre.mx[2] - r.oz) * r.iz;
+    ax = (ax != ax) ? -INFINITY : ax; ay = (ay != ay) ? -INFINITY : ay; az = (az != az) ? -INFINITY : az;
+    cx = (cx != cx) ? INFINITY : cx; cy = (cy != cy) ? INFINITY : cy; cz = (cz != cz) ? INFINITY : cz;
+    float lox = fminf(ax, cx), loy = fminf(ay, cy), loz = fminf(az, cz);
+    float hix = fmaxf(ax, cx), hiy = fmaxf(ay, cy), hiz = fmaxf(az, cz);
+    float t1 = fmaxf(fmaxf(lox, 0.0f), fmaxf(loy, loz));
+    float t2 = fminf(fminf(hix, FLT_MAX), fminf(hiy, hiz));
+    return t1 <= t2;
+}
+__device__ __forceinline__ void mask_cache_begin_pass(const MaskCache& mc, const Ray& r, bool active, uint32_t oct, const PreBox& pre) {
     const int lane = static_cast<int>(threadIdx.x) & 63;
     float* hdr = reinterpret_cast<float*>(mc.lds);
     float h[20];
@@ -147,6 +179,7 @@
             }
             wave_min3_max3(pmin[g], pmax[g]);
         }
+        uint32_t verdict = kVerdictStrict | kVerdictInsidePre;
 #pragma unroll
         for (int g = 0; g < 3; g++) {
 #pragma unroll
@@ -165,6 +198,7 @@
                     wlo = fmaxf(wlo, -cap); whi = fminf(whi, cap);
                 }
                 pmin[g][k] = wlo; pmax[g][k] = whi;
+                verdict_fold(verdict, g, k, oct, wlo, whi, pre);
             }
         }
         MP_PROF_COUNT(3);
@@ -176,6 +210,7 @@
                 for (int k = 0; k < 3; k++) { hdr[hdr_lo(g) + k] = pmin[g][k]; hdr[hdr_lo(g) + 3 + k] = pmax[g][k]; }
             }
             mc.lds[kHdrState] = oct | 0x100u;
+            mc.lds[kHdrVerdict] = verdict;
         }
         int l_ = lane;
         asm volatile("" : "+v"(l_));
@@ -184,11 +219,35 @@
         wave_lds_sync();
     }
 }
+constexpr uint32_t kWalkGeneric = 8u, kWalkLiteral = 9u, kWalkNone = 10u;
+__device__ __forceinline__ uint32_t pass_entry_short(const MaskCache& mc, const Ray& r, bool act, bool kind_ok, bool boxes_ordered) {
+    if (!(kind_ok && boxes_ordered)) return kWalkNone;
+    float h[20];
+#pragma unroll
+    for (int i = 0; i < 5; i++) {
+        const float4 q = reinterpret_cast<const float4*>(mc.lds)[i];
+        h[4 * i] = q.x; h[4 * i + 1] = q.y; h[4 * i + 2] = q.z; h[4 * i + 3] = q.w;
+    }
+    const uint32_t state = __builtin_amdgcn_readfirstlane(as_u(h[kHdrState]));
+    const uint32_t verdict = __builtin_amdgcn_readfirstlane(as_u(h[kHdrVerdict]));
+    if ((state & ~7u) != 0x100u || verdict != (kVerdictStrict | kVerdictInsidePre)) return kWalkNone;
+    const float val[3][3] = {{r.ox, r.oy, r.oz}, {r.ix, r.iy, r.iz}, {r.dx, r.dy, r.dz}};
+    bool in = true;
+#pragma unroll
+    for (int g = 0; g < 3; g++) {
+#pragma unroll
+        for (int k = 0; k < 3; k++) in = in && val[g][k] >= h[hdr_lo(g) + k] && val[g][k] <= h[hdr_lo(g) + 3 + k];
+    }
+    if (__ballot(act) == 0 || __ballot(act && !in) != 0) return kWalkNone;
+    MP_PROF_COUNT(8);
+    return state & 7u;
+}
+
 #ifndef MP_MCACHE_MARGIN
 #define MP_MCACHE_MARGIN 0.015625f
 #endif
 __device__ __forceinline__ void mask_cache_begin_unit(const MaskCache& mc, const mp_camera_sampler& s, float jitter_scale, uint32_t x0,
-                                                      uint32_t x1, uint32_t y0, uint32_t y1) {
+                                                      uint32_t x1, uint32_t y0, uint32_t y1, const PreBox& pre) {
     const int lane = static_cast<int>(threadIdx.x) & 63;
     Ray r;
     float f[3];
@@ -198,7 +257,7 @@
     const uint64_t nx = __ballot(r.ix < 0.0f), ny = __ballot(r.iy < 0.0f), nz = __ballot(r.iz < 0.0f);
     const bool adopt = __ballot(!mask_cache_ray_ok(r)) == 0 && (nx == 0 || ~nx == 0) && (ny == 0 || ~ny == 0) && (nz == 0 || ~nz == 0);
     if (!adopt) {
-        if (lane == 0) mc.lds[kHdrState] = 0xFFFFFFFFu;
+        if (lane == 0) { mc.lds[kHdrState] = 0xFFFFFFFFu; mc.lds[kHdrVerdict] = 0u; }
         wave_lds_sync();
         return;
     }
@@ -212,6 +271,7 @@
     }
     float* hdr = reinterpret_cast<float*>(mc.lds);
     if (lane == 63) {
+        uint32_t verdict = kVerdictStrict | kVerdictInsidePre;
 #pragma unroll
         for (int g = 0; g < 3; g++) {
 #pragma unroll
@@ -229,9 +289,11 @@
                     wlo = fmaxf(wlo, -cap); whi = fminf(whi, cap);
                 }
                 hdr[hdr_lo(g) + k] = wlo; hdr[hdr_lo(g) + 3 + k] = whi;
+                verdict_fold(verdict, g, k, oct, wlo, whi, pre);
             }
         }
         mc.lds[kHdrState] = oct | 0x100u;
+        mc.lds[kHdrVerdict] = verdict;
     }
     MP_PROF_COUNT(3);
 #pragma unroll
diff --git a/minipath_amd/csrc/mask_probe.hip b/minipath_amd/csrc/mask_probe.hip
--- a/minipath_amd/csrc/mask_probe.hip
+++ b/minipath_amd/csrc/mask_probe.hip
@@ -521,7 +521,7 @@
         Ray r;
         r.ox = val[0]; r.oy = val[1]; r.oz = val[2]; r.ix = val[3]; r.iy = val[4]; r.iz = val[5]; r.dx = val[6]; r.dy = val[7]; r.dz = val[8];
         wave_lds_sync();
-        mask_cache_begin_pass(mc, r, active, oct);
+        mask_cache_begin_pass(mc, r, active, oct, PreBox{0u, nullptr, nullptr});
         wave_lds_sync();
         bool outside = false;
         for (int g = 0; g < 3; g++)
@@ -559,7 +559,18 @@
         } else {
             for (int i = 0; i < 19; i++) bad = bad || as_u(nh[i]) != as_u(oh[i]);
         }
-        for (int i = 19; i < 32; i++) bad = bad || as_u(nh[i]) != as_u(oh[i]);
+        for (int i = 20; i < 32; i++) bad = bad || as_u(nh[i]) != as_u(oh[i]);
+        if (rewrite) {
+            bool strict = true;
+            for (int k = 0; k < 3; k++) {
+                const bool neg = ((oct >> k) & 1u) != 0u;
+                strict = strict && fabsf(nh[k]) <= kCoordCap && fabsf(nh[3 + k]) <= kCoordCap && fabsf(nh[13 + k]) <= 2.0f && fabsf(nh[16 + k]) <= 2.0f;
+                strict = strict && (neg ? (nh[6 + k] > -INFINITY && nh[9 + k] < 0.0f) : (nh[6 + k] > 0.0f && nh[9 + k] < INFINITY));
+            }
+            bad = bad || as_u(nh[kHdrVerdict]) != ((strict ? kVerdictStrict : 0u) | kVerdictInsidePre);
+        } else {
+            bad = bad || as_u(nh[kHdrVerdict]) != as_u(oh[kHdrVerdict]);
+        }
         if (as_u(nh[kHdrState]) == (oct | 0x100u)) {
             for (int k = 0; k < 3; k++) {
                 const bool neg = ((oct >> k) & 1u) != 0u;
@@ -585,6 +596,164 @@
             if (bad) { atomicAdd(out + 0, 1ull); atomicMin(out + 2, static_cast<unsigned long long>(c)); }
         }
         wave_lds_sync();
+    }
+}
+
+constexpr int kEntryHead = 32, kEntryDump = kEntryHead + 9 * 64;
+__device__ __forceinline__ uint32_t pass_entry_full(const MaskCache& mc, const Ray& r, bool act, bool kind_ok, bool boxes_ordered, const PreBox& pre,
+                                                    bool& go) {
+    go = act && kind_ok && pre_box_may_hit(pre, r);
+    if (__ballot(go) == 0) return kWalkNone;
+    if (__ballot(go & !mask_cache_ray_ok(r)) != 0) {
+        const bool slow = go && (fabsf(r.ix) == INFINITY || fabsf(r.iy) == INFINITY || fabsf(r.iz) == INFINITY);
+        return __ballot(slow) != 0 ? kWalkLiteral : kWalkGeneric;
+    }
+    if (!boxes_ordered) return kWalkGeneric;
+    const uint64_t am = __ballot(go);
+    const uint64_t nx = __ballot(go && r.ix < 0.0f), ny = __ballot(go && r.iy < 0.0f), nz = __ballot(go && r.iz < 0.0f);
+    if (!((nx == 0 || nx == am) && (ny == 0 || ny == am) && (nz == 0 || nz == am))) return kWalkGeneric;
+    const uint32_t oct = (nx ? 1u : 0u) | (ny ? 2u : 0u) | (nz ? 4u : 0u);
+    mask_cache_begin_pass(mc, r, go, oct, pre);
+    return oct;
+}
+__device__ __forceinline__ uint32_t pass_entry(const MaskCache& mc, const Ray& r, bool act, bool kind_ok, bool boxes_ordered, const PreBox& pre,
+                                               bool& go) {
+    const uint32_t oct = pass_entry_short(mc, r, act, kind_ok, boxes_ordered);
+    if (oct != kWalkNone) {
+        go = act;
+        return oct;
+    }
+    return pass_entry_full(mc, r, act, kind_ok, boxes_ordered, pre, go);
+}
+__global__ void __launch_bounds__(256) entry_kernel(uint64_t seed, uint64_t base_case, uint64_t ncases, unsigned long long* out, uint32_t* dump) {
+    __shared__ __align__(16) uint32_t lds[8 * kMaskCacheDwords];
+    const uint32_t w = threadIdx.x >> 6, lane = threadIdx.x & 63u;
+    const uint64_t c = base_case + static_cast<uint64_t>(blockIdx.x) * 4u + w;
+    if (c >= ncases) return;
+    uint32_t* const ca = lds + (2u * w) * kMaskCacheDwords;
+    uint32_t* const cb = ca + kMaskCacheDwords;
+    const uint32_t cls = static_cast<uint32_t>(c & 7u);
+    const uint64_t hc = hsh(seed, c, 0);
+    const uint32_t oct = static_cast<uint32_t>(hc >> 8) & 7u;
+    float b[20];
+    float olo[3], ohi[3];
+    gen_origin_bounds(seed, c, olo, ohi);
+#pragma unroll
+    for (int k = 0; k < 3; k++) {
+        if (cls != 5u || k != static_cast<int>((hc >> 12) % 3u)) { olo[k] = clampf(olo[k], -kCoordCap, kCoordCap); ohi[k] = clampf(ohi[k], -kCoordCap, kCoordCap); }
+        else { ohi[k] = (hc >> 16) & 1u ? kOrgCap : step(kCoordCap, true); olo[k] = fminf(olo[k], ohi[k]); }
+        const uint64_t h = hsh(seed, c, 60 + k), h2 = hsh(seed, c, 63 + k);
+        const bool wide = (h & 0x300u) == 0u;
+        const float m1 = wide ? pick_pos(h, 0, 254) : pick_pos(h, 127 - 2, 127 + 12);
+        float m2 = (h2 & 7u) == 0u ? m1 : wide ? pick_pos(h2, 0, 254) : pick_pos(h2, 127 - 2, 127 + 12);
+        if ((h2 & 0x7F00u) == 0u) m2 = FLT_MAX;
+        const float mlo = fmaxf(fminf(m1, m2), 0x1p-149f), mhi = fmaxf(fmaxf(m1, m2), 0x1p-149f);
+        const bool neg = ((oct >> k) & 1u) != 0u;
+        b[k] = olo[k]; b[3 + k] = ohi[k];
+        b[6 + k] = neg ? -mhi : mlo;
+        b[9 + k] = neg ? -mlo : mhi;
+        const uint64_t h3 = hsh(seed, c, 66 + k), h4 = hsh(seed, c, 69 + k);
+        const float d1 = clampf(pick(h3, 127 - 30, 127 + 1), -2.0f, 2.0f), d2 = (h4 & 7u) == 0u ? ((h4 & 8u) ? 0.0f : -0.0f) : clampf(pick(h4, 127 - 30, 127 + 1), -2.0f, 2.0f);
+        b[13 + k] = fminf(d1, d2); b[16 + k] = fmaxf(d1, d2);
+    }
+    b[12] = as_f(oct | 0x100u);
+    if (cls == 7u) b[12] = as_f((hc >> 20) & 1u ? 0xFFFFFFFFu : (hc >> 21) & 1u ? oct : (oct | 0x200u));
+    float pmn[3], pmx[3];
+    const bool has_pre = cls == 6u || (hc >> 24 & 3u) != 0u;
+#pragma unroll
+    for (int k = 0; k < 3; k++) {
+        const uint64_t h = hsh(seed, c, 80 + k);
+        const uint32_t f = static_cast<uint32_t>(h & 7u);
+        const float g1 = pick_pos(h, 127 - 20, 127 + 32), g2 = pick_pos(hsh(seed, c, 83 + k), 127 - 20, 127 + 32);
+        pmn[k] = (f & 1u) ? b[k] : clampf(b[k] - g1, -FLT_MAX, b[k]);
+        pmx[k] = (f & 2u) ? b[3 + k] : clampf(b[3 + k] + g2, b[3 + k], FLT_MAX);
+        if (cls == 6u && (hc >> 28 & 1u) && k == static_cast<int>((hc >> 29) % 3u)) {
+            if (f & 4u) pmn[k] = b[k] < b[3 + k] ? lerp_in(step(b[k], true), b[3 + k], unit(h)) : step(b[k], true);
+            else pmx[k] = b[k] < b[3 + k] ? lerp_in(b[k], step(b[3 + k], false), unit(h)) : step(b[3 + k], false);
+        }
+    }
+    const PreBox pre{has_pre ? 1u : 0u, pmn, pmx};
+    uint32_t verdict = kVerdictStrict | kVerdictInsidePre;
+#pragma unroll
+    for (int g = 0; g < 3; g++) {
+#pragma unroll
+        for (int k = 0; k < 3; k++) verdict_fold(verdict, g, k, oct, b[hdr_lo(g) + k], b[hdr_lo(g) + 3 + k], pre);
+    }
+    b[kHdrVerdict] = as_f(as_u(b[12]) == 0xFFFFFFFFu ? 0u : verdict);
+    const bool kind_ok = (hc >> 32 & 15u) != 0u, ordered = (hc >> 36 & 15u) != 0u;
+    const uint64_t rnd = hsh(seed, c, 1);
+    const uint32_t ak = static_cast<uint32_t>(hc >> 40) % 5u;
+    uint64_t am = ak == 0u ? ~0ull : ak == 1u ? ~0ull >> 1 : ak == 2u ? rnd | 1ull : ak == 3u ? 1ull << (rnd & 63u) : rnd | ~0ull << 60;
+    if (cls == 4u) am &= ~(1ull << ((rnd >> 8) & 63u)) & ~(1ull << ((rnd >> 16) & 63u));
+    if (cls != 4u && (hc >> 44 & 63u) == 0u) am = 0ull;
+    uint32_t special = 64u;
+    if (cls >= 1u && cls <= 3u && am != 0ull) {
+        special = static_cast<uint32_t>(rnd >> 24) & 63u;
+        if (!((am >> special) & 1u)) special = static_cast<uint32_t>(__builtin_ctzll(am));
+    }
+    const bool active = (am >> lane) & 1u;
+    float val[9];
+#pragma unroll
+    for (int g = 0; g < 3; g++) {
+#pragma unroll
+        for (int k = 0; k < 3; k++) {
+            const uint64_t h = hsh(seed, c, 100u + lane * 9u + static_cast<uint32_t>(g * 3 + k));
+            const uint32_t pos = static_cast<uint32_t>(h & 7u);
+            const float lo = b[hdr_lo(g) + k], hi = b[hdr_lo(g) + 3 + k];
+            float x = pos < 4u ? lerp_in(lo, hi, unit(h)) : pos < 6u ? lo : hi;
+            if (x == 0.0f && (h >> 8 & 1u)) x = -x;
+            if (!active && cls == 4u) x = as_f(static_cast<uint32_t>(h >> 32) | ((h & 0x30u) ? 0x7F800000u : 0u));
+            val[g * 3 + k] = x;
+        }
+    }
+    if (lane == special) {
+        const uint32_t comp = static_cast<uint32_t>(c >> 3) % 9u;
+        const bool up = ((c >> 3) / 9u & 1u) != 0u;
+#pragma unroll
+        for (int i = 0; i < 9; i++) {
+            const float lo = b[hdr_lo(i / 3) + i % 3], hi = b[hdr_lo(i / 3) + 3 + i % 3];
+            if (cls == 1u && i == static_cast<int>(comp)) val[i] = up ? step(hi, true) : step(lo, false);
+            if (cls == 2u && i == static_cast<int>(comp)) val[i] = as_f(up ? 0x7FC00000u : 0xFF800001u);
+            if (cls == 3u && i >= 3 && i < 6 && i % 3 == static_cast<int>(comp % 3u)) val[i] = up ? INFINITY : -INFINITY;
+        }
+    }
+    for (uint32_t i = lane; i < static_cast<uint32_t>(kMaskCacheDwords); i += 64u) {
+        const uint32_t v = static_cast<uint32_t>(hsh(seed, c, 5000u + i)) & 0x7FFFFFFFu;
+        ca[i] = v; cb[i] = v;
+    }
+    wave_lds_sync();
+    if (lane == 0u) {
+#pragma unroll
+        for (int i = 0; i < 20; i++) { ca[i] = as_u(b[i]); cb[i] = as_u(b[i]); }
+    }
+    wave_lds_sync();
+    Ray r;
+    r.ox = val[0]; r.oy = val[1]; r.oz = val[2]; r.ix = val[3]; r.iy = val[4]; r.iz = val[5]; r.dx = val[6]; r.dy = val[7]; r.dz = val[8];
+    bool go_a = false, go_b = false;
+    const uint32_t walk_a = __builtin_amdgcn_readfirstlane(pass_entry_full(MaskCache{ca}, r, active, kind_ok, ordered, pre, go_a));
+    wave_lds_sync();
+    const bool took_short = __builtin_amdgcn_readfirstlane(pass_entry_short(MaskCache{cb}, r, active, kind_ok, ordered)) != kWalkNone;
+    const uint32_t walk_b = __builtin_amdgcn_readfirstlane(pass_entry(MaskCache{cb}, r, active, kind_ok, ordered, pre, go_b));
+    wave_lds_sync();
+    bool lane_bad = false;
+    for (uint32_t i = lane; i < static_cast<uint32_t>(kLeafMaskBase); i += 64u) lane_bad = lane_bad || ((i < 20u || i >= static_cast<uint32_t>(kMaskCacheHeader)) && ca[i] != cb[i]);
+    const bool bad = walk_a != walk_b || __ballot(go_a) != __ballot(go_b) || __ballot(lane_bad) != 0;
+    record_case(out, bad, c, took_short, walk_a < 8u, false);
+    if (dump) {
+        uint32_t* rec = dump + (c - base_case) * kEntryDump;
+        if (lane == 0u) {
+#pragma unroll
+            for (int i = 0; i < 20; i++) rec[i] = as_u(b[i]);
+        }
+        if (lane == 20u) {
+            rec[20] = has_pre ? 1u : 0u;
+            for (int k = 0; k < 3; k++) { rec[21 + k] = as_u(pmn[k]); rec[24 + k] = as_u(pmx[k]); }
+            rec[27] = kind_ok ? 1u : 0u; rec[28] = ordered ? 1u : 0u;
+            rec[29] = static_cast<uint32_t>(am); rec[30] = static_cast<uint32_t>(am >> 32);
+            rec[31] = walk_b | (took_short ? 0x100u : 0u) | (walk_a << 16);
+        }
+#pragma unroll
+        for (int i = 0; i < 9; i++) rec[kEntryHead + i * 64 + static_cast<int>(lane)] = as_u(val[i]);
     }
 }
 
@@ -602,7 +771,7 @@
     constexpr int kTags = kLeafMaskBase - kMaskCacheHeader;
     for (int i = 0; i < kTags / 64; i++) base[kMaskCacheHeader + i * 64 + static_cast<int>(lane)] = static_cast<uint32_t>(i * 64) + lane;
     wave_lds_sync();
-    mask_cache_begin_unit(MaskCache{base}, cam.s, jitter_scale, blocks[4 * unit], blocks[4 * unit + 1], blocks[4 * unit + 2], blocks[4 * unit + 3]);
+    mask_cache_begin_unit(MaskCache{base}, cam.s, jitter_scale, blocks[4 * unit], blocks[4 * unit + 1], blocks[4 * unit + 2], blocks[4 * unit + 3], PreBox{0u, nullptr, nullptr});
     wave_lds_sync();
     uint32_t cleared = 0u;
     for (int i = 0; i < kTags / 64; i++) cleared += static_cast<uint32_t>(__popcll(__ballot(base[kMaskCacheHeader + i * 64 + static_cast<int>(lane)] == 0xFFFFFFFFu)));
@@ -758,6 +927,21 @@
     for (int i = 0; i < kCounters; i++) out[i] = acc[i];
     return static_cast<int>(ef);
 }
+int mp_mask_probe_entry_dwords() { return kEntryDump; }
+int mp_mask_probe_entry(uint64_t seed, uint64_t ncases, uint32_t* host_dump, unsigned long long* out) {
+    (void)hipGetLastError();
+    if (ncases > kCasesPerLaunch) return -1;
+    uint32_t* dev = nullptr;
+    const size_t bytes = static_cast<size_t>(ncases) * kEntryDump * sizeof(uint32_t);
+    if (host_dump && bytes) {
+        const hipError_t e = hipMalloc(&dev, bytes);
+        if (e != hipSuccess) return static_cast<int>(e);
+    }
+    int rc = run_cases(entry_kernel, seed, ncases, dev, out);
+    if (rc == 0 && dev) rc = static_cast<int>(hipMemcpy(host_dump, dev, bytes, hipMemcpyDeviceToHost));
+    const hipError_t ef = dev ? hipFree(dev) : hipSuccess;
+    return rc != 0 ? rc : static_cast<int>(ef);
+}
 int mp_mask_probe_unit(const float* sampler, float jitter_scale, const uint32_t* blocks, uint32_t n, uint32_t* out, uint32_t* ntags,
                        float* margin) {
     (void)hipGetLastError();
```

New measurement: 38980, median of 6. 1.03x the previous value.
